# ubc-vision/RefTR

Hardware: AMD Instinct MI355X
Metric: images/sec training step, RefCOCO R50 640x640 bs=8/GPU (higher is better)
Workload: dtype bf16; 1 GPU; RefCOCO-shaped REC train step, ResNet-50 + BERT-base + VL transformer 6+6, 640x640, batch 8/GPU, L=40, aux loss, dropout on, clip 0.1, AdamW (configs[1]); global_batch=8, batch_per_gpu=8, image_size=640, parallelism=dp1, launch=hipgraph

## Files before the change

include/reftr_hip.h:

```cpp
#ifndef REFTR_HIP_H
#define REFTR_HIP_H
#include <stdint.h>

#ifdef __cplusplus
extern "C" {
#endif

typedef void* rt_stream_t;

enum { RT_OK = 0, RT_ERR_BADARG = -1, RT_ERR_UNSUPPORTED = -2, RT_ERR_COMM = -3 };
enum { RT_ACT_NONE = 0, RT_ACT_RELU = 1, RT_ACT_GELU = 2, RT_ACT_TANH = 3 };

int rt_abi_version(void);
int rt_device_arch(int dev, char* buf, int buflen);

typedef struct rt_conv_gemm_desc {
    const void*  src;
    const void*  wgt;
    void*        out_bf16;
    float*       out_f32;
    const float* bias;
    const float* res_f32;
    const void*  res_bf16;
    const void*  gate;
    const void*  preact;
    int32_t B, SH, SW, SC;
    int32_t DH, DW, N;
    int32_t KH, KW, stride, pad;
    int32_t transposed;
    int32_t act;
    float    gate_scale;
    float    drop_p;
    uint32_t drop_seed;
    int32_t  tile_hint;
    void*    out_preact;
    const void* dtanh;
    int32_t  res_first;
    const uint32_t* seed_dev;
    int32_t drop_shift;
    float* acc2_f32;
    int32_t dil;
} rt_conv_gemm_desc;
int rt_conv_gemm(const rt_conv_gemm_desc* d, rt_stream_t stream);
int rt_conv_gemm_grouped(const rt_conv_gemm_desc* descs, int n, rt_stream_t stream);

typedef struct rt_conv_wgrad_desc {
    const void*  dy;
    const void*  x;
    float*       dw;
    const float* scale;
    int32_t B, SH, SW, SC;
    int32_t DH, DW, N;
    int32_t KH, KW, stride, pad;
    int32_t msplit;
    float*  dbias;
    int32_t variant;
    float*  workspace;
    int64_t workspace_bytes;
    int32_t overwrite;
    int32_t dil;
    float*  sqacc;
    void*   g16;
} rt_conv_wgrad_desc;
int rt_conv_wgrad(const rt_conv_wgrad_desc* d, rt_stream_t stream);

typedef struct rt_small_wgrad_job {
    const void* dy; const void* x; float* dw; float* dbias;
    int32_t M, N, K, overwrite;
    float* sqacc;
    void*  g16;
} rt_small_wgrad_job;
int rt_small_wgrad_grouped(const rt_small_wgrad_job* jobs, int njobs, rt_stream_t stream);

int rt_conv_wgrad_grouped(const rt_conv_wgrad_desc* descs, int n, float* workspace, int64_t workspace_bytes, rt_stream_t stream);

int rt_gconv(const rt_conv_gemm_desc* d, int groups, rt_stream_t stream);
int rt_gconv_wgrad(const rt_conv_wgrad_desc* d, int groups, rt_stream_t stream);

typedef struct rt_layernorm_desc {
    const float* x;
    const float* gamma;
    const float* beta;
    float*       y_f32;
    void*        y_bf16;
    const float* pos;
    void*        ypos_bf16;
    float*       mean;
    float*       rstd;
    int32_t M, D;
    float   eps;
    int32_t act;
    float    drop_p;
    uint32_t drop_seed;
    int32_t grp_rows, grp_stride, grp_off;
    const uint32_t* seed_dev;
} rt_layernorm_desc;
int rt_layernorm_fwd(const rt_layernorm_desc* d, rt_stream_t stream);

typedef struct rt_layernorm_bwd_desc {
    const float* dy;
    const float* dy2;
    const float* x;
    const float* gamma;
    const float* beta;
    const float* mean;
    const float* rstd;
    float*       dx_f32;
    void*        dx_bf16;
    float*       dgamma;
    float*       dbeta;
    int32_t M, D;
    int32_t act;
    float    drop_p;  uint32_t drop_seed;
    float    drop2_p; uint32_t drop2_seed;
    int32_t grp_rows, grp_stride, grp_off;
    const uint32_t* seed_dev;
    float*   partials;
    int32_t* n_blocks_out;
} rt_layernorm_bwd_desc;
int rt_layernorm_bwd(const rt_layernorm_bwd_desc* d, rt_stream_t stream);

typedef struct rt_ln_pg_job {
    const float* partials; float* dgamma; float* dbeta;
    int32_t n_blocks, D;
} rt_ln_pg_job;
int rt_ln_param_grad_grouped(const rt_ln_pg_job* jobs, int n, rt_stream_t stream);

typedef struct rt_groupnorm_desc {
    const float* x;
    const float* gamma; const float* beta;
    float*       stats;
    float*       y_f32; void* y_bf16;
    const float* pos; void* ypos_bf16;
    int32_t B, HW, C, G;
    float   eps;
    int32_t out_rows_per_img, out_row_off;
    float*  partials;
    int32_t chunks;
} rt_groupnorm_desc;
int rt_groupnorm_fwd(const rt_groupnorm_desc* d, rt_stream_t stream);

typedef struct rt_groupnorm_bwd_desc {
    const float* dy; const float* dy2;
    const float* x; const float* gamma;
    const float* stats;
    float*       bstats;
    float*       dx_f32; void* dx_bf16;
    float*       dgamma; float* dbeta;
    int32_t B, HW, C, G;
    float   eps;
    int32_t out_rows_per_img, out_row_off;
} rt_groupnorm_bwd_desc;
int rt_groupnorm_bwd(const rt_groupnorm_bwd_desc* d, rt_stream_t stream);

typedef struct rt_gn_nhwc_desc {
    const float* x; const float* gamma; const float* beta;
    float* stats; void* y_bf16;
    int32_t B, HW, C, G, ldx, ldy, act;
    float eps;
    float* partials; int32_t partial_blocks;
} rt_gn_nhwc_desc;
int rt_gn_nhwc_fwd(const rt_gn_nhwc_desc* d, rt_stream_t stream);

typedef struct rt_gn_nhwc_bwd_desc {
    const float* dy; const float* x; const float* gamma; const float* beta;
    const float* stats; float* bstats;
    void* dx_bf16; float* dgamma; float* dbeta;
    int32_t B, HW, C, G, ldx, lddy, lddx, act;
    float eps;
} rt_gn_nhwc_bwd_desc;
int rt_gn_nhwc_bwd(const rt_gn_nhwc_bwd_desc* d, rt_stream_t stream);

typedef struct rt_upsample_add_desc {
    const float* fpn; const void* a_bf16; void* out_bf16;
    int32_t B, H, W, h, w, C, ldf, lda, ldo;
} rt_upsample_add_desc;
int rt_upsample_add(const rt_upsample_add_desc* d, rt_stream_t stream);

typedef struct rt_upsample_add_bwd_desc {
    const float* dy; float* da; void* dy_bf16;
    int32_t B, H, W, h, w, C, lddy, ldda, lddyb;
} rt_upsample_add_bwd_desc;
int rt_upsample_add_bwd(const rt_upsample_add_bwd_desc* d, rt_stream_t stream);

typedef struct rt_attn_map_desc {
    const float* q; const float* k; const uint8_t* mask;
    float* P; void* concat_bf16;
    int32_t B, HW, E, nh, ldk, k_rows_per_img, k_row_off, ld_concat, concat_col;
    float norm;
} rt_attn_map_desc;
int rt_attn_map_fwd(const rt_attn_map_desc* d, rt_stream_t stream);

typedef struct rt_attn_map_bwd_desc {
    const float* q; const float* k; const float* P; const float* dconcat;
    float* dq; float* dk;
    int32_t B, HW, E, nh, ldk, k_rows_per_img, k_row_off, ld_dconcat, concat_col;
    float norm;
} rt_attn_map_bwd_desc;
int rt_attn_map_bwd(const rt_attn_map_bwd_desc* d, rt_stream_t stream);

typedef struct rt_seg_concat_desc {
    const float* src; const float* mem; void* out_bf16;
    int32_t B, HW, E, nh, ldo, mem_rows_per_img, mem_row_off, src_rows_per_img, src_row_off;
} rt_seg_concat_desc;
int rt_seg_concat(const rt_seg_concat_desc* d, rt_stream_t stream);

typedef struct rt_mask_loss_desc {
    const float* pred; const uint8_t* target;
    float* sums; float* losses;
    float* dpred; const float* g_focal; const float* g_dice;
    int32_t B, h, w, Ht, Wt, ldp, lddp;
    float inv_norm;
    float* gbuf;
} rt_mask_loss_desc;
#define RT_MASK_LOSS_PARTIALS 1024
int rt_mask_loss(const rt_mask_loss_desc* d, rt_stream_t stream);

typedef struct rt_attn_desc {
    const void* q; const void* k; const void* v;
    void*  out;
    float* lse;
    const uint8_t* kpm;
    int32_t B, H, Sq, Sk, dh;
    int32_t ldq, ldk, ldv, ldo;
    float    scale;
    float    drop_p; uint32_t drop_seed;
    const uint32_t* seed_dev;
} rt_attn_desc;
int rt_attn_fwd(const rt_attn_desc* d, rt_stream_t stream);

typedef struct rt_attn_bwd_desc {
    const void* q; const void* k; const void* v; const void* out; const void* dout;
    const float* lse;
    float* delta;
    const uint8_t* kpm;
    void* dq; void* dk; void* dv;
    int32_t B, H, Sq, Sk, dh;
    int32_t ldq, ldk, ldv, ldo, lddq, lddk, lddv;
    float    scale;
    float    drop_p; uint32_t drop_seed;
    const uint32_t* seed_dev;
} rt_attn_bwd_desc;
int rt_attn_bwd(const rt_attn_bwd_desc* d, rt_stream_t stream);

int rt_img_pack(const float* img, void* out, int B, int H, int W, int Hp, int Wp, rt_stream_t stream);
int rt_stem_conv(const void* xp, const void* w, const float* bias, void* out,
                 int B, int Hp, int Wp, int Ho, int Wo, rt_stream_t stream);
int rt_maxpool3x3s2(const void* x, void* y, int B, int H, int W, int C, int Ho, int Wo, rt_stream_t stream);
int rt_stem_pool(const void* xp, const void* w, const float* bias, void* out,
                 int B, int Hp, int Wp, int Ho, int Wo, rt_stream_t stream);
int rt_weight_prep(const float* src, const float* scale, void* dst, void* dst_t, int N, int T, int C, rt_stream_t stream);

typedef struct rt_bottleneck_desc {
    const void*  x;
    const void*  w1;
    const void*  w2;
    const void*  w3;
    const void*  wd;
    const float* b1;
    const float* b2;
    const float* b3;
    const float* bd;
    void*        out;
    int32_t B, H, W, cin, planes;
    int32_t form;
} rt_bottleneck_desc;
int rt_bottleneck_fwd(const rt_bottleneck_desc* d, rt_stream_t stream);
int rt_weight_prep_batched(const int64_t* table, int njobs, int total_tiles, rt_stream_t stream);
int rt_stem_weight_prep(const float* src, const float* scale, void* dst, rt_stream_t stream);
int rt_bn_fold(const float* w, const float* b, const float* rm, const float* rv, float eps,
               float* scale, float* shift, int n, rt_stream_t stream);

typedef struct rt_mask_posenc_desc {
    const uint8_t* mask;
    uint8_t* kpm_out;
    float*   pos_out;
    const float* add_vec;
    int32_t B, H, W, h, w, C;
    int32_t kpm_stride, kpm_off;
    int32_t pos_rows_per_img, pos_row_off;
} rt_mask_posenc_desc;
int rt_mask_posenc(const rt_mask_posenc_desc* d, rt_stream_t stream);

int rt_colsum(const void* dy, int is_bf16, float* db, int M, int N, rt_stream_t stream);

typedef struct rt_rows_add_desc {
    const float* a_f32; const void* a_bf16; const float* b_f32;
    float* out_f32; void* out_bf16;
    int32_t rows, D;
    float   alpha;
    int32_t accumulate;
    int32_t a_grp_rows, a_grp_stride, a_grp_off;
    int32_t b_grp_rows, b_grp_stride, b_grp_off;
    int32_t o_grp_rows, o_grp_stride, o_grp_off;
} rt_rows_add_desc;
int rt_rows_add(const rt_rows_add_desc* d, rt_stream_t stream);

int rt_bert_embed_fwd(const int64_t* ids, const float* word, const float* pos, const float* type0,
                      float* out, int rows, int L, int D, const int32_t* pos_ids, rt_stream_t stream);
int rt_bert_embed_bwd(const int64_t* ids, const float* de, float* dword, float* dpos, float* dtype0,
                      int rows, int L, int D, const int32_t* pos_ids, rt_stream_t stream);
int rt_roberta_pos_ids(const int64_t* ids, int32_t* pos_ids, int B, int L, int pad_idx, rt_stream_t stream);
int rt_context_mask(const uint8_t* smask, const uint8_t* phrase_mask, const int64_t* pos_l, const int64_t* pos_r,
                    uint8_t* ctx, uint8_t* qmask, int B, int L, int P, int Lp, rt_stream_t stream);
int rt_qenc_attn_fwd(const float* k, const float* qs, const float* vs, const uint8_t* ctx, float* w, float* c,
                     int B, int P, int L, int E, rt_stream_t stream);
int rt_qenc_attn_bwd(const float* k, const float* qs, const float* vs, const float* w, const float* dc,
                     float* dk, float* dqs, float* dvs, int B, int P, int L, int E, rt_stream_t stream);

typedef struct rt_box_loss_desc {
    const float*   logits;
    const uint8_t* valid;
    const float*   targets;
    const int32_t* tgt_off;
    const float*   num_boxes;
    float* losses; float* total; float* dlogits;
    int32_t NL, B, P, K;
    float   w_bbox, w_giou;
    const float* weights;
} rt_box_loss_desc;
int rt_box_loss(const rt_box_loss_desc* d, rt_stream_t stream);

int rt_small_dgrad(const float* dy, const float* w, const void* gate, void* dx, int M, int N, int K, rt_stream_t stream);
int rt_pos_grad(const float* dpos, float* d_lang_pos, float* d_type, float* d_level, int B, int S, int L, int E,
                rt_stream_t stream);

int rt_sqnorm(const float* g, int64_t n, float* out, rt_stream_t stream);
int rt_sqnorm_bf16(const void* g16, int64_t n, float* out, rt_stream_t stream);

typedef struct rt_adamw_desc {
    float* p; const float* g; float* m; float* v;
    int64_t n;
    const float* gnorm_sq;
    float* gnorm_out;
    float grad_scale, max_norm, beta1, beta2, eps;
    int32_t step, n_ranges;
    int64_t range_begin[8], range_end[8];
    float   range_lr[8], range_wd[8];
    const int32_t* step_dev;
    const int32_t* active;
    const float*   lr_dev;
    int64_t span_begin, span_end;
    const void* g16;
} rt_adamw_desc;
int rt_adamw_flat(const rt_adamw_desc* d, rt_stream_t stream);
int rt_sgd_flat(const rt_adamw_desc* d, rt_stream_t stream);
enum { RT_ACCUM_FIRST = 0, RT_ACCUM_ADD = 1, RT_ACCUM_FINISH = 2 };
// ... 327 lines not shown
```

reftr_amd/csrc/rt_gemm.hip:

```cpp
#include "rt_gemm_dma.h"
#include <stdio.h>

namespace {

#ifdef RT_LAB
template <int BM, int BN, int MODE>
__global__ __launch_bounds__(256, 2) void conv_gemm_kernel(const bf16_t* __restrict__ src,
                                                        const bf16_t* __restrict__ wgt, const GemmArgs p) {
    typedef WaveTile<BM, BN, 2> WT;
    constexpr int TM = WT::TM, TN = WT::TN;
    constexpr int AJ = BN / 32, BJ = BM / 32;
    constexpr int A_BYTES = WT::A_BYTES, BUF_BYTES = WT::BUF_BYTES;
    extern __shared__ __attribute__((aligned(16))) unsigned char smem[];

    const int t = threadIdx.x;
    const int lane = t & 63, wave = t >> 6;
    const int wn = wave & 1, wm = wave >> 1;
    const WT wt{wn, wm, lane & 15, lane >> 4};

    const int n_tiles = (p.N + BN - 1) / BN;
    const int tile_n = blockIdx.x % n_tiles, tile_m = blockIdx.x / n_tiles;
    const int n0 = tile_n * BN, m0 = tile_m * BM;

    const int chunk = t & 7, srow = t >> 3;

    int a_off[AJ]; bool a_ok[AJ];
#pragma unroll
    for (int j = 0; j < AJ; ++j) {
        const int n = n0 + srow + 32 * j;
        a_ok[j] = n < p.N;
        a_off[j] = a_ok[j] ? n * p.K + chunk * 8 : 0;
    }
    int b_off[BJ], b_y[BJ], b_x[BJ]; bool b_ok[BJ];
#pragma unroll
    for (int j = 0; j < BJ; ++j) {
        const int m = m0 + srow + 32 * j;
        b_ok[j] = m < p.M;
        const int mm = b_ok[j] ? m : 0;
        if (MODE == 0) {
            b_off[j] = mm * p.SC + chunk * 8; b_y[j] = 0; b_x[j] = 0;
        } else {
            const int dx = mm % p.DW;
            const int tmp = mm / p.DW;
            const int dy = tmp % p.DH;
            const int b = tmp / p.DH;
            if (MODE == 1) { b_y[j] = dy * p.stride - p.pad; b_x[j] = dx * p.stride - p.pad; }
            else           { b_y[j] = dy + p.pad;            b_x[j] = dx + p.pad; }
            b_off[j] = b * p.SH * p.SW * p.SC + chunk * 8;
        }
    }

    f32x4 acc[TN][TM];
#pragma unroll
    for (int a = 0; a < TN; ++a)
#pragma unroll
        for (int b = 0; b < TM; ++b) acc[a][b] = f32x4{0.f, 0.f, 0.f, 0.f};

    const int nk = p.K >> 6;
    int lk = 0, c0 = 0, kw = 0, kh = 0;

    uint4 ra0[AJ], rb0[BJ], ra1[AJ], rb1[BJ];

    const __amdgpu_buffer_rsrc_t rs_w = __builtin_amdgcn_make_buffer_rsrc(const_cast<bf16_t*>(wgt), 0, p.wgt_bytes, 0x00020000);
    const __amdgpu_buffer_rsrc_t rs_x = __builtin_amdgcn_make_buffer_rsrc(const_cast<bf16_t*>(src), 0, p.src_bytes, 0x00020000);
    constexpr int OOB = 0x7fffffff;
    auto load_tiles = [&](uint4 (&ra)[AJ], uint4 (&rb)[BJ]) __attribute__((always_inline)) {
        const int k0b = lk << 7;
#pragma unroll
        for (int j = 0; j < AJ; ++j) {
            const auto v = __builtin_amdgcn_raw_buffer_load_b128(rs_w, a_ok[j] ? a_off[j] * 2 : OOB, k0b, 0);
            ra[j] = make_uint4(v[0], v[1], v[2], v[3]);
        }
#pragma unroll
        for (int j = 0; j < BJ; ++j) {
            if (MODE == 0) {
                const auto v = __builtin_amdgcn_raw_buffer_load_b128(rs_x, b_ok[j] ? b_off[j] * 2 : OOB, k0b, 0);
                rb[j] = make_uint4(v[0], v[1], v[2], v[3]);
            } else {
                bool ok = b_ok[j];
                int sy, sx;
                if (MODE == 1) { sy = b_y[j] + kh; sx = b_x[j] + kw; }
                else {
                    const int ny = b_y[j] - kh, nx = b_x[j] - kw;
                    const int msk = p.stride - 1;
                    ok = ok && ((ny | nx) >= 0) && (((ny | nx) & msk) == 0);
                    sy = ny >> p.sshift; sx = nx >> p.sshift;
                }
                ok = ok && (unsigned)sy < (unsigned)p.SH && (unsigned)sx < (unsigned)p.SW;
                const int off = (b_off[j] + (sy * p.SW + sx) * p.SC) * 2;
                const auto v = __builtin_amdgcn_raw_buffer_load_b128(rs_x, ok ? off : OOB, c0 * 2, 0);
                rb[j] = make_uint4(v[0], v[1], v[2], v[3]);
            }
        }
        if (lk + 1 < nk) {
            ++lk;
            if (MODE != 0) {
                c0 += 64;
                if (c0 >= p.SC) { c0 = 0; ++kw; if (kw >= p.KW) { kw = 0; ++kh; } }
            }
        }
    };
    auto store_tiles = [&](int buf, const uint4 (&ra)[AJ], const uint4 (&rb)[BJ]) __attribute__((always_inline)) {
        unsigned char* bA = smem + buf * BUF_BYTES;
        unsigned char* bB = bA + A_BYTES;
#pragma unroll
        for (int j = 0; j < AJ; ++j) {
            const int row = srow + 32 * j;
            *reinterpret_cast<uint4*>(bA + row * 128 + ((chunk ^ (row & 7)) << 4)) = ra[j];
        }
#pragma unroll
        for (int j = 0; j < BJ; ++j) {
            const int row = srow + 32 * j;
            *reinterpret_cast<uint4*>(bB + row * 128 + ((chunk ^ (row & 7)) << 4)) = rb[j];
        }
    };
    auto compute = [&](int buf) __attribute__((always_inline)) { wt.compute(smem + buf * BUF_BYTES, acc); };

    load_tiles(ra0, rb0);
    load_tiles(ra1, rb1);
    store_tiles(0, ra0, rb0);
    __syncthreads();
    for (int kt = 0; kt < nk; kt += 2) {
        load_tiles(ra0, rb0);
        compute(0);
        store_tiles(1, ra1, rb1);
        __syncthreads();
        if (kt + 1 >= nk) break;
        load_tiles(ra1, rb1);
        compute(1);
        store_tiles(0, ra0, rb0);
        __syncthreads();
    }

#pragma unroll
    for (int a = 0; a < TN; ++a) {
        const int n = n0 + wn * (BN / 2) + a * 16 + wt.lg * 4;
        if (n >= p.N) continue;
#pragma unroll
        for (int b = 0; b < TM; ++b) {
            const int m = m0 + wm * (BM / 2) + b * 16 + wt.li;
            if (m >= p.M) continue;
            epilogue<4>(p, m, n, acc[a][b]);
        }
    }
}

#endif

struct GemmGroup { GemmArgs j[12]; int first[13]; int n; };
struct GroupTile { static constexpr int BM = 64, BN = 64, NS = 2, MINB = 4; };
template <int BM, int BN, int NS, int MINB>
__global__ __launch_bounds__(256, MINB) void conv_gemm_dma_grouped_kernel(const GemmGroup g) {
    int lo = 0;
    for (int i = 1; i < g.n; ++i) if (g.first[i] <= (int)blockIdx.x) lo = i;
    lo = __builtin_amdgcn_readfirstlane(lo);
    const int lin = (int)blockIdx.x - g.first[lo];
    const int gx = g.first[lo + 1] - g.first[lo];
    gemm_dma_body<BM, BN, 0, NS>(g.j[lo].src, g.j[lo].wgt, g.j[lo], lin, 0, gx);
}

template <int CH>
__global__ __launch_bounds__(256) void skinny_gemm_kernel(const bf16_t* __restrict__ src, const bf16_t* __restrict__ wgt,
                                                          const GemmArgs p) {
    __shared__ f32x4 red[4][64];
    const int lane = threadIdx.x & 63, wave = threadIdx.x >> 6;
    const int li = lane & 15, lg = lane >> 4;
    const int n0 = blockIdx.x * 16;
    const int nrow = n0 + li;
    const int n = n0 + lg * 4;
    const bool out_ok = wave == 0 && n < p.N && li < p.M;
    EpiPre<4> pre;
    if (out_ok) pre = epi_prefetch<4>(p, (size_t)li * p.N + n, n);
    constexpr int OOB = 0x7fffffff;
    const __amdgpu_buffer_rsrc_t rs_w = __builtin_amdgcn_make_buffer_rsrc(const_cast<bf16_t*>(wgt), 0, p.wgt_bytes, 0x00020000);
    const __amdgpu_buffer_rsrc_t rs_x = __builtin_amdgcn_make_buffer_rsrc(const_cast<bf16_t*>(src), 0, p.src_bytes, 0x00020000);
    const int w_off = nrow < p.N ? (nrow * p.K + lg * 8) * 2 : OOB;
    const int x_off = li < p.M ? (li * p.K + lg * 8) * 2 : OOB;
    const int ksteps = p.K >> 5;
    const int per = (ksteps + 3) >> 2;
    const int k_begin = wave * per, k_end = min(k_begin + per, ksteps);
    f32x4 acc = {0.f, 0.f, 0.f, 0.f};
    typedef __attribute__((ext_vector_type(4))) unsigned u32x4;
    for (int ks = k_begin; ks < k_end; ks += CH) {
        u32x4 wv[CH], xv[CH];
#pragma unroll
        for (int j = 0; j < CH; ++j) {
            const bool in = ks + j < k_end;
            wv[j] = __builtin_amdgcn_raw_buffer_load_b128(rs_w, in ? w_off : OOB, (ks + j) << 6, 0);
            xv[j] = __builtin_amdgcn_raw_buffer_load_b128(rs_x, in ? x_off : OOB, (ks + j) << 6, 0);
        }
#pragma unroll
        for (int j = 0; j < CH; ++j)
            acc = __builtin_amdgcn_mfma_f32_16x16x32_bf16(*reinterpret_cast<bf16x8*>(&wv[j]), *reinterpret_cast<bf16x8*>(&xv[j]), acc, 0, 0, 0);
    }
    red[wave][lane] = acc;
    __syncthreads();
    if (wave != 0) return;
    acc = red[0][lane] + red[1][lane] + red[2][lane] + red[3][lane];
    if (out_ok) epilogue<4, true>(p, li, n, acc, &pre);
}

#ifdef RT_LAB
__global__ __launch_bounds__(256) void skinny_gemm_kernel_v1(const bf16_t* __restrict__ src, const bf16_t* __restrict__ wgt,
                                                             const GemmArgs p) {
    __shared__ f32x4 red[4][64];
    const int lane = threadIdx.x & 63, wave = threadIdx.x >> 6;
    const int li = lane & 15, lg = lane >> 4;
    const int n0 = blockIdx.x * 16;
    const int nrow = n0 + li;
    const bool n_ok = nrow < p.N, m_ok = li < p.M;
    const bf16_t* wp = wgt + (size_t)(n_ok ? nrow : 0) * p.K + lg * 8;
    const bf16_t* xp = src + (size_t)(m_ok ? li : 0) * p.K + lg * 8;
    const int ksteps = p.K >> 5;
    const int per = (ksteps + 3) >> 2;
    const int k_begin = wave * per, k_end = min(k_begin + per, ksteps);
    f32x4 acc = {0.f, 0.f, 0.f, 0.f};
    const uint4 z = make_uint4(0, 0, 0, 0);
#pragma unroll 4
    for (int ks = k_begin; ks < k_end; ++ks) {
        uint4 wv = *reinterpret_cast<const uint4*>(wp + ks * 32);
        uint4 xv = *reinterpret_cast<const uint4*>(xp + ks * 32);
        if (!n_ok) wv = z;
        if (!m_ok) xv = z;
        acc = __builtin_amdgcn_mfma_f32_16x16x32_bf16(*reinterpret_cast<bf16x8*>(&wv), *reinterpret_cast<bf16x8*>(&xv), acc, 0, 0, 0);
    }
    red[wave][lane] = acc;
    __syncthreads();
    if (wave != 0) return;
    acc = red[0][lane] + red[1][lane] + red[2][lane] + red[3][lane];
    const int n = n0 + lg * 4;
    if (n < p.N && li < p.M) epilogue<4>(p, li, n, acc);
}

template <int BM, int BN>
int launch_gemm(const GemmArgs& a, hipStream_t s) {
    const int mt = (a.M + BM - 1) / BM, nt = (a.N + BN - 1) / BN;
    const size_t smem = 2 * (size_t)(BM + BN) * 128;
    const dim3 grid((unsigned)(mt * nt)), block(256);
    if (gemm_dense(a))
        hipLaunchKernelGGL((conv_gemm_kernel<BM, BN, 0>), grid, block, smem, s, a.src, a.wgt, a);
    else if (!a.transposed)
        hipLaunchKernelGGL((conv_gemm_kernel<BM, BN, 1>), grid, block, smem, s, a.src, a.wgt, a);
    else
        hipLaunchKernelGGL((conv_gemm_kernel<BM, BN, 2>), grid, block, smem, s, a.src, a.wgt, a);
    RT_CHECK_LAUNCH();
    return RT_OK;
}

#endif

}

static int fill_gemm_args(const rt_conv_gemm_desc* d, GemmArgs& a) {
    if (!d || !d->src || !d->wgt || (!d->out_bf16 && !d->out_f32)) return RT_ERR_BADARG;
    if (d->SC <= 0 || (d->SC & 63) || (d->N & 3) || d->N <= 0) return RT_ERR_UNSUPPORTED;
    if (d->stride != 1 && d->stride != 2) return RT_ERR_UNSUPPORTED;
    if (d->KH <= 0 || d->KW <= 0 || d->B <= 0 || d->DH <= 0 || d->DW <= 0) return RT_ERR_BADARG;
    a.src = (const bf16_t*)d->src; a.wgt = (const bf16_t*)d->wgt;
    a.out_bf16 = (bf16_t*)d->out_bf16; a.out_f32 = d->out_f32; a.out_preact = (bf16_t*)d->out_preact;
    a.bias = d->bias; a.res_f32 = d->res_f32; a.res_bf16 = (const bf16_t*)d->res_bf16;
    a.gate = (const bf16_t*)d->gate; a.preact = (const bf16_t*)d->preact; a.dtanh = (const bf16_t*)d->dtanh;
    a.B = d->B; a.SH = d->SH; a.SW = d->SW; a.SC = d->SC; a.DH = d->DH; a.DW = d->DW; a.N = d->N;
    a.KH = d->KH; a.KW = d->KW; a.stride = d->stride; a.pad = d->pad; a.transposed = d->transposed;
    a.act = d->act; a.res_first = d->res_first; a.gate_scale = d->gate_scale; a.drop_p = d->drop_p; a.drop_seed = d->drop_seed; a.seed_dev = d->seed_dev;
    a.drop_shift = d->drop_shift;
    a.acc2_f32 = d->acc2_f32;
    a.dil = d->dil > 1 ? d->dil : 1;
    if (a.dil > 1 && d->stride != 1) return RT_ERR_UNSUPPORTED;
    if (a.drop_shift < 0 || a.drop_shift > 16) return RT_ERR_BADARG;
    const long long M = (long long)d->B * d->DH * d->DW;
    if (M > 0x7fffffffLL / 4) return RT_ERR_UNSUPPORTED;
    if ((long long)d->B * d->SH * d->SW * d->SC >= 0x3fffffffLL || (long long)d->N * d->KH * d->KW * d->SC >= 0x3fffffffLL) return RT_ERR_UNSUPPORTED;
    a.M = (int)M; a.K = d->KH * d->KW * d->SC; a.sshift = d->stride == 2 ? 1 : 0;
    static const int xcd_env = RT_TUNE("REFTR_XCD", 1);
    a.xcd = xcd_env;
    static const int early_env = RT_TUNE("REFTR_EARLY", 3);
    a.early = early_env & 1;
    static const int epi_env = RT_TUNE("REFTR_EPI", 3);
    a.epi_lds = epi_env & 1;
#ifdef RT_LAB
    static const int abl_env = RT_TUNE("REFTR_GEMM_ABL", 0);
    a.abl = abl_env;
#else
    a.abl = 0;
#endif
    static const int pre_env = RT_TUNE("REFTR_EPI_PREFETCH", 1);
    a.prefetch = pre_env;
    a.mfast = 0;
    a.src_bytes = (unsigned)((long long)d->B * d->SH * d->SW * d->SC * 2);
    a.wgt_bytes = (unsigned)((long long)d->N * d->KH * d->KW * d->SC * 2);
    return RT_OK;
}

static bool gemm_skinny(const GemmArgs& a) { return gemm_dense(a) && a.M <= 16; }
enum { GEMM_ROUTE_SKINNY = -1 };

static int gemm_route(const GemmArgs& a, int tile_hint) {
    if (tile_hint != 0) return tile_hint;
    if (gemm_skinny(a)) return GEMM_ROUTE_SKINNY;
    const bool dense = gemm_dense(a);
    int hint;
    const long long t128 = (long long)((a.M + 127) / 128) * ((a.N + 127) / 128);
    const long long t12864 = (long long)((a.M + 127) / 128) * ((a.N + 63) / 64);
    static const int smallt = RT_TUNE("REFTR_SMALLT", 1);
    static const int pipe = RT_TUNE("REFTR_PIPE", 3);
    const long long t64 = (long long)((a.M + 63) / 64) * ((a.N + 63) / 64);
    const long long t256 = (long long)((a.M + 255) / 256) * ((a.N + 127) / 128);
    static const int deep = RT_TUNE("REFTR_DEEP", 1);
    static const int k1024 = RT_TUNE("REFTR_K1024", 1);
    if (dense && smallt && a.M <= 1024 && t64 < 256 && (a.N & 7) == 0) hint = t64 <= 96 ? ((deep && a.K >= 512) ? 285 : 281) : 33;
    else if (a.K < 1024) hint = (a.N >= 128 && t128 >= 384 && t128 <= 512) ? 51 : 31;
    else if (dense && a.K >= 2048 && a.N >= 128 && t256 >= 512) hint = 262;
    else if (a.N > 64 && (t128 >= 384 || (a.K >= 2048 && t128 >= 192))) hint = (!dense && (pipe & 1) && a.K >= 2048 && t128 <= 256) ? 252 : 51;
    else if (k1024 && dense && a.N > 64 && a.K >= 1024 && t128 >= 192) hint = 51;
    else if (t12864 >= 256) hint = 21;
    else hint = (!dense && (pipe & 2)) ? 233 : 33;
#ifdef RT_LAB
    static const int pp = RT_TUNE("REFTR_PP", 0);
    if ((a.N & 7) == 0 && a.epi_lds && a.N >= 128) {
        if ((pp & 1) && hint == 252) hint = (pp & 4) ? 351 : 352;
        else if ((pp & 2) && dense && a.K >= 1024 && t128 >= 128 && t128 <= 256) hint = (pp & 4) ? 351 : 352;
    }
    static const int astat = RT_TUNE("REFTR_ASTAT", 0);
    if (astat && rt_gemm_astat_ok(a) && a.M >= 1024 && a.N >= 2 * a.K && a.N >= 256) hint = 501;
    {
        const char* ov = getenv("REFTR_HINT_OVERRIDE");
        while (ov && *ov) {
            int t_, kh_, s_, m_, k_, n_, h_, used = 0;
            if (sscanf(ov, "%d,%d,%d,%d,%d,%d=%d%n", &t_, &kh_, &s_, &m_, &k_, &n_, &h_, &used) == 7) {
                if (t_ == (a.transposed ? 1 : 0) && kh_ == a.KH && s_ == a.stride && m_ == a.M && k_ == a.K && n_ == a.N) { hint = h_; break; }
                ov += used;
            }
            while (*ov && *ov != ';') ++ov;
            if (*ov == ';') ++ov;
        }
    }
#endif
    return hint;
}

static int launch_skinny(const GemmArgs& a, hipStream_t s) {
    const dim3 grid((unsigned)((a.N + 15) / 16));
    const int per = ((a.K >> 5) + 3) >> 2;
#ifdef RT_LAB
    static const int skinny_v = RT_TUNE("REFTR_SKINNY_V", 2);
    if (skinny_v == 1) { hipLaunchKernelGGL(skinny_gemm_kernel_v1, grid, dim3(256), 0, s, a.src, a.wgt, a); RT_CHECK_LAUNCH(); return RT_OK; }
#endif
    if (per <= 2) hipLaunchKernelGGL(skinny_gemm_kernel<2>, grid, dim3(256), 0, s, a.src, a.wgt, a);
    else if (per <= 4) hipLaunchKernelGGL(skinny_gemm_kernel<4>, grid, dim3(256), 0, s, a.src, a.wgt, a);
    else hipLaunchKernelGGL(skinny_gemm_kernel<8>, grid, dim3(256), 0, s, a.src, a.wgt, a);
    RT_CHECK_LAUNCH();
    return RT_OK;
}

extern "C" int rt_conv_gemm(const rt_conv_gemm_desc* d, rt_stream_t stream) {
    GemmArgs a;
    const int frc = fill_gemm_args(d, a);
    if (frc != RT_OK) return frc;
    hipStream_t s = (hipStream_t)stream;
    const int hint = gemm_route(a, d->tile_hint);
    if (a.dil > 1 && hint >= 1 && hint <= 3) return RT_ERR_UNSUPPORTED;
    switch (hint) {
        case GEMM_ROUTE_SKINNY: return launch_skinny(a, s);
        case 21: return launch_gemm_dma<128, 64, 2, 2>(a, s);
        case 31: return launch_gemm_dma<GroupTile::BM, GroupTile::BN, GroupTile::NS, GroupTile::MINB>(a, s);
        case 33: return launch_gemm_dma<64, 64, 3, 3>(a, s);
        case 51: return launch_gemm_dma<128, 128, 2, 2, 8>(a, s);
        case 233: case 252: case 262: case 281: case 285: return rt_launch_gemm_pipe(a, hint, s);
#ifdef RT_LAB
        case 501: return rt_launch_gemm_astat(a, s);
        case 1: return launch_gemm<128, 128>(a, s);
        case 2: return launch_gemm<128, 64>(a, s);
        case 3: return launch_gemm<64, 64>(a, s);
        case 11: return launch_gemm_dma<128, 128, 2, 2>(a, s);
        case 12: return launch_gemm_dma<128, 128, 3, 2>(a, s);
        case 13: return launch_gemm_dma<128, 128, 4, 2>(a, s);
        case 22: return launch_gemm_dma<128, 64, 3, 2>(a, s);
        case 32: return launch_gemm_dma<64, 64, 4, 2>(a, s);
        case 52: return launch_gemm_dma<128, 128, 3, 1, 8>(a, s);
        case 53: return launch_gemm_dma<128, 64, 2, 2, 8>(a, s);
        case 54: return launch_gemm_dma<128, 64, 3, 2, 8>(a, s);
        case 61: return launch_gemm_dma<256, 128, 2, 1, 8>(a, s);
        case 62: return launch_gemm_dma<256, 128, 3, 1, 8>(a, s);
        case 63: return launch_gemm_dma<128, 256, 2, 1, 8>(a, s);
        case 211: case 221: case 231: case 251: case 261:
        case 81: case 282: case 283: case 284: case 286: case 287: case 288: case 234: case 236: return rt_launch_gemm_pipe(a, hint, s);
        case 351: case 321: case 323: case 331: case 352: case 322: case 332: return rt_launch_gemm_pp(a, hint, s);
#endif
        default: return RT_ERR_BADARG;
    }
}

extern "C" int rt_conv_gemm_grouped(const rt_conv_gemm_desc* descs, int n, rt_stream_t stream) {
    if (!descs || n <= 0) return RT_ERR_BADARG;
    hipStream_t s = (hipStream_t)stream;
    static const int grp_env = RT_TUNE("REFTR_GEMM_GROUP", 1);
    bool ok = grp_env && n >= 2 && n <= 12;
    GemmGroup g;
    int blocks = 0;
    for (int i = 0; i < n && ok; ++i) {
        const rt_conv_gemm_desc& d = descs[i];
        GemmArgs a;
        const int rc = fill_gemm_args(&d, a);
        if (rc != RT_OK) return rc;
        if (d.tile_hint != 0 || !gemm_dense(a) || gemm_skinny(a) || a.K >= 1024) { ok = false; break; }
        g.j[i] = a; g.first[i] = blocks;
        blocks += ((a.M + GroupTile::BM - 1) / GroupTile::BM) * ((a.N + GroupTile::BN - 1) / GroupTile::BN);
    }
    if (!ok) {
        for (int i = 0; i < n; ++i) { const int rc = rt_conv_gemm(descs + i, stream); if (rc != RT_OK) return rc; }
        return RT_OK;
    }
    g.first[n] = blocks; g.n = n;
    for (int i = n + 1; i < 13; ++i) g.first[i] = blocks;
    hipLaunchKernelGGL((conv_gemm_dma_grouped_kernel<GroupTile::BM, GroupTile::BN, GroupTile::NS, GroupTile::MINB>), dim3((unsigned)blocks), dim3(256),
                       gemm_dma_lds_bytes(GroupTile::BM, GroupTile::BN, GroupTile::NS), s, g);
    RT_CHECK_LAUNCH();
    return RT_OK;
}

extern "C" int rt_abi_version(void) { return 39; }

extern "C" int rt_device_arch(int dev, char* buf, int buflen) {
    hipDeviceProp_t prop;
    hipError_t e = hipGetDeviceProperties(&prop, dev);
    if (e != hipSuccess) return (int)e;
    if (!buf || buflen <= 0) return RT_ERR_BADARG;
    int i = 0;
    for (; i < buflen - 1 && prop.gcnArchName[i]; ++i) buf[i] = prop.gcnArchName[i];
    buf[i] = 0;
    return RT_OK;
}
```

reftr_amd/hip.py:

```python
import contextlib
import ctypes
import os
from ctypes import POINTER, Structure, c_char_p, c_float, c_int, c_int32, c_int64, c_uint32, c_void_p

import torch

_HERE = os.path.dirname(os.path.abspath(__file__))
LIB_PATH = os.path.join(_HERE, "libreftr_hip_lab.so" if os.environ.get("REFTR_LAB", "0") == "1" else "libreftr_hip.so")
ABI_VERSION = 39

CONSTANTS = {
    "RT_ACT_NONE": 0, "RT_ACT_RELU": 1, "RT_ACT_GELU": 2, "RT_ACT_TANH": 3,
    "RT_ACCUM_FIRST": 0, "RT_ACCUM_ADD": 1, "RT_ACCUM_FINISH": 2, "RT_GRAD_ACCUM_SLOTS": 2048,
    "RT_SQ_SLOTS": 256, "RT_SQ_STRIDE": 32,
    "RT_MASK_LOSS_PARTIALS": 1024, "RT_STATS_MAX": 40,
    "RT_BATCH_STAGE_MAX_B": 64,
    "RT_RAW_STAGE_MAX_SCALE": 4, "RT_RAW_STAGE_TILE_H": 32, "RT_RAW_STAGE_TILE_W": 64,
    "RT_EVAL_DET_N": 0, "RT_EVAL_DET_HIT": 1, "RT_EVAL_SEG_N": 6, "RT_EVAL_SEG_HIT": 7, "RT_EVAL_SEG_I": 12, "RT_EVAL_SEG_U": 13,
    "RT_EVAL_DET_SUM": 14, "RT_EVAL_SEG_SUM": 15, "RT_EVAL_SLOTS": 16, "RT_EVAL_CHUNK": 16384,
    "RT_EVAL_ORIG_N": 0, "RT_EVAL_ORIG_HIT": 1, "RT_EVAL_ORIG_I": 6, "RT_EVAL_ORIG_U": 7, "RT_EVAL_ORIG_SUM": 8, "RT_EVAL_ORIG_SLOTS": 9,
    "RT_PREDICT_FACTS_WORDS": 8,
    "RT_DEC_MAX_LAYERS": 8, "RT_DEC_HANDOFF_BYTES": 256 + 16 * 256 * 36 + 16 * 2048 * 4,
}
globals().update({name[3:]: value for name, value in CONSTANTS.items()})

STRUCTS = {}


class _Abi(Structure):

    def __init_subclass__(cls, c):
        cls.C_NAME = c
        STRUCTS[c] = cls


class ConvGemmDesc(_Abi, c="rt_conv_gemm_desc"):
    _fields_ = [("src", c_void_p), ("wgt", c_void_p), ("out_bf16", c_void_p), ("out_f32", c_void_p),
                ("bias", c_void_p), ("res_f32", c_void_p), ("res_bf16", c_void_p), ("gate", c_void_p),
                ("preact", c_void_p),
                ("B", c_int32), ("SH", c_int32), ("SW", c_int32), ("SC", c_int32),
                ("DH", c_int32), ("DW", c_int32), ("N", c_int32),
                ("KH", c_int32), ("KW", c_int32), ("stride", c_int32), ("pad", c_int32),
                ("transposed", c_int32), ("act", c_int32),
                ("gate_scale", c_float), ("drop_p", c_float), ("drop_seed", c_uint32), ("tile_hint", c_int32),
                ("out_preact", c_void_p), ("dtanh", c_void_p), ("res_first", c_int32), ("seed_dev", c_void_p),
                ("drop_shift", c_int32), ("acc2_f32", c_void_p), ("dil", c_int32)]


class ConvWgradDesc(_Abi, c="rt_conv_wgrad_desc"):
    _fields_ = [("dy", c_void_p), ("x", c_void_p), ("dw", c_void_p), ("scale", c_void_p),
                ("B", c_int32), ("SH", c_int32), ("SW", c_int32), ("SC", c_int32),
                ("DH", c_int32), ("DW", c_int32), ("N", c_int32),
                ("KH", c_int32), ("KW", c_int32), ("stride", c_int32), ("pad", c_int32),
                ("msplit", c_int32), ("dbias", c_void_p), ("variant", c_int32),
                ("workspace", c_void_p), ("workspace_bytes", c_int64), ("overwrite", c_int32), ("dil", c_int32),
                ("sqacc", c_void_p), ("g16", c_void_p)]


class LayerNormDesc(_Abi, c="rt_layernorm_desc"):
    _fields_ = [("x", c_void_p), ("gamma", c_void_p), ("beta", c_void_p), ("y_f32", c_void_p), ("y_bf16", c_void_p),
                ("pos", c_void_p), ("ypos_bf16", c_void_p), ("mean", c_void_p), ("rstd", c_void_p),
                ("M", c_int32), ("D", c_int32), ("eps", c_float), ("act", c_int32),
                ("drop_p", c_float), ("drop_seed", c_uint32),
                ("grp_rows", c_int32), ("grp_stride", c_int32), ("grp_off", c_int32), ("seed_dev", c_void_p)]


class LayerNormBwdDesc(_Abi, c="rt_layernorm_bwd_desc"):
    _fields_ = [("dy", c_void_p), ("dy2", c_void_p), ("x", c_void_p), ("gamma", c_void_p), ("beta", c_void_p),
                ("mean", c_void_p), ("rstd", c_void_p), ("dx_f32", c_void_p), ("dx_bf16", c_void_p),
                ("dgamma", c_void_p), ("dbeta", c_void_p),
                ("M", c_int32), ("D", c_int32), ("act", c_int32),
                ("drop_p", c_float), ("drop_seed", c_uint32), ("drop2_p", c_float), ("drop2_seed", c_uint32),
                ("grp_rows", c_int32), ("grp_stride", c_int32), ("grp_off", c_int32), ("seed_dev", c_void_p),
                ("partials", c_void_p), ("n_blocks_out", POINTER(c_int32))]


class LnPgJob(_Abi, c="rt_ln_pg_job"):
    _fields_ = [("partials", c_void_p), ("dgamma", c_void_p), ("dbeta", c_void_p), ("n_blocks", c_int32), ("D", c_int32)]


class GroupNormDesc(_Abi, c="rt_groupnorm_desc"):
    _fields_ = [("x", c_void_p), ("gamma", c_void_p), ("beta", c_void_p), ("stats", c_void_p),
                ("y_f32", c_void_p), ("y_bf16", c_void_p), ("pos", c_void_p), ("ypos_bf16", c_void_p),
                ("B", c_int32), ("HW", c_int32), ("C", c_int32), ("G", c_int32), ("eps", c_float),
                ("out_rows_per_img", c_int32), ("out_row_off", c_int32), ("partials", c_void_p), ("chunks", c_int32)]


class GroupNormBwdDesc(_Abi, c="rt_groupnorm_bwd_desc"):
    _fields_ = [("dy", c_void_p), ("dy2", c_void_p), ("x", c_void_p), ("gamma", c_void_p), ("stats", c_void_p),
                ("bstats", c_void_p), ("dx_f32", c_void_p), ("dx_bf16", c_void_p), ("dgamma", c_void_p), ("dbeta", c_void_p),
                ("B", c_int32), ("HW", c_int32), ("C", c_int32), ("G", c_int32), ("eps", c_float),
                ("out_rows_per_img", c_int32), ("out_row_off", c_int32)]


class AttnDesc(_Abi, c="rt_attn_desc"):
    _fields_ = [("q", c_void_p), ("k", c_void_p), ("v", c_void_p), ("out", c_void_p), ("lse", c_void_p), ("kpm", c_void_p),
                ("B", c_int32), ("H", c_int32), ("Sq", c_int32), ("Sk", c_int32), ("dh", c_int32),
                ("ldq", c_int32), ("ldk", c_int32), ("ldv", c_int32), ("ldo", c_int32),
                ("scale", c_float), ("drop_p", c_float), ("drop_seed", c_uint32), ("seed_dev", c_void_p)]


class AttnBwdDesc(_Abi, c="rt_attn_bwd_desc"):
    _fields_ = [("q", c_void_p), ("k", c_void_p), ("v", c_void_p), ("out", c_void_p), ("dout", c_void_p),
                ("lse", c_void_p), ("delta", c_void_p), ("kpm", c_void_p), ("dq", c_void_p), ("dk", c_void_p), ("dv", c_void_p),
                ("B", c_int32), ("H", c_int32), ("Sq", c_int32), ("Sk", c_int32), ("dh", c_int32),
                ("ldq", c_int32), ("ldk", c_int32), ("ldv", c_int32), ("ldo", c_int32),
                ("lddq", c_int32), ("lddk", c_int32), ("lddv", c_int32),
                ("scale", c_float), ("drop_p", c_float), ("drop_seed", c_uint32), ("seed_dev", c_void_p)]


class MaskPosencDesc(_Abi, c="rt_mask_posenc_desc"):
    _fields_ = [("mask", c_void_p), ("kpm_out", c_void_p), ("pos_out", c_void_p), ("add_vec", c_void_p),
                ("B", c_int32), ("H", c_int32), ("W", c_int32), ("h", c_int32), ("w", c_int32), ("C", c_int32),
                ("kpm_stride", c_int32), ("kpm_off", c_int32), ("pos_rows_per_img", c_int32), ("pos_row_off", c_int32)]


class BottleneckDesc(_Abi, c="rt_bottleneck_desc"):
    _fields_ = [("x", c_void_p), ("w1", c_void_p), ("w2", c_void_p), ("w3", c_void_p), ("wd", c_void_p),
                ("b1", c_void_p), ("b2", c_void_p), ("b3", c_void_p), ("bd", c_void_p), ("out", c_void_p),
                ("B", c_int32), ("H", c_int32), ("W", c_int32), ("cin", c_int32), ("planes", c_int32), ("form", c_int32)]


class RowsAddDesc(_Abi, c="rt_rows_add_desc"):
    _fields_ = [("a_f32", c_void_p), ("a_bf16", c_void_p), ("b_f32", c_void_p), ("out_f32", c_void_p), ("out_bf16", c_void_p),
                ("rows", c_int32), ("D", c_int32), ("alpha", c_float), ("accumulate", c_int32),
                ("a_grp_rows", c_int32), ("a_grp_stride", c_int32), ("a_grp_off", c_int32),
                ("b_grp_rows", c_int32), ("b_grp_stride", c_int32), ("b_grp_off", c_int32),
                ("o_grp_rows", c_int32), ("o_grp_stride", c_int32), ("o_grp_off", c_int32)]


class BoxLossDesc(_Abi, c="rt_box_loss_desc"):
    _fields_ = [("logits", c_void_p), ("valid", c_void_p), ("targets", c_void_p), ("tgt_off", c_void_p),
                ("num_boxes", c_void_p), ("losses", c_void_p), ("total", c_void_p), ("dlogits", c_void_p),
                ("NL", c_int32), ("B", c_int32), ("P", c_int32), ("K", c_int32), ("w_bbox", c_float), ("w_giou", c_float),
                ("weights", c_void_p)]


class MaskPostDesc(_Abi, c="rt_mask_post_desc"):
    _fields_ = [("pred", c_void_p), ("sizes", c_void_p), ("orig", c_void_p), ("origin_off", c_void_p),
                ("masks", c_void_p), ("masks_origin", c_void_p),
                ("B", c_int32), ("Q", c_int32), ("h", c_int32), ("w", c_int32), ("max_h", c_int32), ("max_w", c_int32),
                ("max_origin", c_int64), ("threshold", c_float)]


class BoxPostDesc(_Abi, c="rt_box_post_desc"):
    _fields_ = [("boxes", c_void_p), ("valid", c_void_p), ("sizes", c_void_p), ("out", c_void_p), ("counts", c_void_p),
                ("B", c_int32), ("P", c_int32), ("K", c_int32)]


class CemDesc(_Abi, c="rt_cem_desc"):
    _fields_ = [("hs", c_void_p), ("w3", c_void_p), ("b3", c_void_p), ("res", c_void_p), ("w2", c_void_p), ("b2", c_void_p),
                ("u", c_void_p), ("energy", c_void_p), ("stats", c_void_p), ("loss", c_void_p), ("g", c_void_p),
                ("dres", c_void_p), ("dhs", c_void_p), ("dw3", c_void_p), ("db3", c_void_p), ("dw2", c_void_p),
                ("B", c_int32), ("HW", c_int32), ("ld", c_int32), ("lddr", c_int32), ("E", c_int32), ("reserved", c_int32)]


class AdamWDesc(_Abi, c="rt_adamw_desc"):
    _fields_ = [("p", c_void_p), ("g", c_void_p), ("m", c_void_p), ("v", c_void_p), ("n", c_int64),
                ("gnorm_sq", c_void_p), ("gnorm_out", c_void_p),
                ("grad_scale", c_float), ("max_norm", c_float), ("beta1", c_float), ("beta2", c_float), ("eps", c_float),
                ("step", c_int32), ("n_ranges", c_int32),
                ("range_begin", c_int64 * 8), ("range_end", c_int64 * 8), ("range_lr", c_float * 8), ("range_wd", c_float * 8),
                ("step_dev", c_void_p), ("active", c_void_p), ("lr_dev", c_void_p), ("span_begin", c_int64), ("span_end", c_int64),
                ("g16", c_void_p)]


class FinishDesc(_Abi, c="rt_finish_desc"):
    _fields_ = [("step", c_void_p), ("active", c_void_p), ("cond", c_void_p), ("loss", c_void_p),
                ("sq", c_void_p), ("norm_scale", c_float), ("grad_norm", c_void_p),
                ("src", c_void_p * STATS_MAX), ("n_src", c_int), ("cond_in_stats", c_int), ("stats", c_void_p)]


class SmallWgradJob(_Abi, c="rt_small_wgrad_job"):
    _fields_ = [("dy", c_void_p), ("x", c_void_p), ("dw", c_void_p), ("dbias", c_void_p),
                ("M", c_int32), ("N", c_int32), ("K", c_int32), ("overwrite", c_int32), ("sqacc", c_void_p), ("g16", c_void_p)]


class GnNhwcDesc(_Abi, c="rt_gn_nhwc_desc"):
    _fields_ = [("x", c_void_p), ("gamma", c_void_p), ("beta", c_void_p), ("stats", c_void_p), ("y_bf16", c_void_p),
                ("B", c_int32), ("HW", c_int32), ("C", c_int32), ("G", c_int32), ("ldx", c_int32), ("ldy", c_int32),
                ("act", c_int32), ("eps", c_float), ("partials", c_void_p), ("partial_blocks", c_int32)]


class GnNhwcBwdDesc(_Abi, c="rt_gn_nhwc_bwd_desc"):
    _fields_ = [("dy", c_void_p), ("x", c_void_p), ("gamma", c_void_p), ("beta", c_void_p), ("stats", c_void_p),
                ("bstats", c_void_p), ("dx_bf16", c_void_p), ("dgamma", c_void_p), ("dbeta", c_void_p),
                ("B", c_int32), ("HW", c_int32), ("C", c_int32), ("G", c_int32), ("ldx", c_int32), ("lddy", c_int32),
                ("lddx", c_int32), ("act", c_int32), ("eps", c_float)]


class UpsampleAddDesc(_Abi, c="rt_upsample_add_desc"):
    _fields_ = [("fpn", c_void_p), ("a_bf16", c_void_p), ("out_bf16", c_void_p),
                ("B", c_int32), ("H", c_int32), ("W", c_int32), ("h", c_int32), ("w", c_int32), ("C", c_int32),
                ("ldf", c_int32), ("lda", c_int32), ("ldo", c_int32)]


class UpsampleAddBwdDesc(_Abi, c="rt_upsample_add_bwd_desc"):
    _fields_ = [("dy", c_void_p), ("da", c_void_p), ("dy_bf16", c_void_p),
                ("B", c_int32), ("H", c_int32), ("W", c_int32), ("h", c_int32), ("w", c_int32), ("C", c_int32),
                ("lddy", c_int32), ("ldda", c_int32), ("lddyb", c_int32)]


class AttnMapDesc(_Abi, c="rt_attn_map_desc"):
    _fields_ = [("q", c_void_p), ("k", c_void_p), ("mask", c_void_p), ("P", c_void_p), ("concat_bf16", c_void_p),
                ("B", c_int32), ("HW", c_int32), ("E", c_int32), ("nh", c_int32), ("ldk", c_int32),
                ("k_rows_per_img", c_int32), ("k_row_off", c_int32), ("ld_concat", c_int32), ("concat_col", c_int32),
                ("norm", c_float)]


class AttnMapBwdDesc(_Abi, c="rt_attn_map_bwd_desc"):
    _fields_ = [("q", c_void_p), ("k", c_void_p), ("P", c_void_p), ("dconcat", c_void_p), ("dq", c_void_p), ("dk", c_void_p),
                ("B", c_int32), ("HW", c_int32), ("E", c_int32), ("nh", c_int32), ("ldk", c_int32),
                ("k_rows_per_img", c_int32), ("k_row_off", c_int32), ("ld_dconcat", c_int32), ("concat_col", c_int32),
                ("norm", c_float)]


class SegConcatDesc(_Abi, c="rt_seg_concat_desc"):
    _fields_ = [("src", c_void_p), ("mem", c_void_p), ("out_bf16", c_void_p),
                ("B", c_int32), ("HW", c_int32), ("E", c_int32), ("nh", c_int32), ("ldo", c_int32),
                ("mem_rows_per_img", c_int32), ("mem_row_off", c_int32), ("src_rows_per_img", c_int32), ("src_row_off", c_int32)]


class MaskLossDesc(_Abi, c="rt_mask_loss_desc"):
    _fields_ = [("pred", c_void_p), ("target", c_void_p), ("sums", c_void_p), ("losses", c_void_p),
                ("dpred", c_void_p), ("g_focal", c_void_p), ("g_dice", c_void_p),
                ("B", c_int32), ("h", c_int32), ("w", c_int32), ("Ht", c_int32), ("Wt", c_int32), ("ldp", c_int32),
                ("lddp", c_int32), ("inv_norm", c_float), ("gbuf", c_void_p)]


class EvalMetricsArgs(_Abi, c="rt_eval_metrics_args"):
    _fields_ = [("pred_boxes", c_void_p), ("valid", c_void_p), ("table", c_void_p), ("masks", c_void_p), ("sizes", c_void_p),
                ("partials", c_void_p), ("iou_det", c_void_p), ("iou_seg", c_void_p), ("iu", c_void_p), ("acc", c_void_p),
                ("B", c_int32), ("P", c_int32), ("K", c_int32), ("Q", c_int32), ("max_h", c_int32), ("max_w", c_int32),
                ("reset", c_int32)]


class EvalCanvasArgs(_Abi, c="rt_eval_canvas_args"):
    _fields_ = [("pred_boxes", c_void_p), ("valid", c_void_p), ("tgt_boxes", c_void_p), ("tgt_off", c_void_p), ("facts", c_void_p),
                ("image_ids", c_void_p), ("pred_masks", c_void_p), ("tgt_masks", c_void_p), ("partials", c_void_p),
                ("iou_det", c_void_p), ("iou_seg", c_void_p), ("iu", c_void_p), ("acc", c_void_p), ("ring_boxes", c_void_p),
                ("ring_counts", c_void_p), ("ring_ids", c_void_p), ("cursor", c_void_p), ("veto", c_void_p),
                ("B", c_int32), ("P", c_int32), ("K", c_int32), ("Q", c_int32), ("h", c_int32), ("w", c_int32), ("Hc", c_int32),
                ("Wc", c_int32), ("tgt_rows", c_int32), ("slots", c_int32), ("threshold", c_float)]


class EvalRawFactsArgs(_Abi, c="rt_eval_raw_facts_args"):
    _N = CONSTANTS["RT_BATCH_STAGE_MAX_B"]
    _fields_ = [("facts", c_void_p), ("image_ids", c_void_p), ("mask_table", c_void_p), ("max_pixels", c_int64),
                ("B", c_int32), ("Hc", c_int32), ("Wc", c_int32), ("has_ids", c_int32),
                ("img_h", c_int32 * _N), ("img_w", c_int32 * _N), ("orig_h", c_int32 * _N), ("orig_w", c_int32 * _N),
                ("image_id", c_int64 * _N), ("tm_ptr", c_void_p * _N)]


class EvalOrigArgs(_Abi, c="rt_eval_orig_args"):
    _fields_ = [("pred_masks", c_void_p), ("facts", c_void_p), ("mask_table", c_void_p), ("partials", c_void_p), ("iou_seg", c_void_p),
                ("iu", c_void_p), ("acc", c_void_p), ("veto", c_void_p), ("max_pixels", c_int64),
                ("B", c_int32), ("Q", c_int32), ("h", c_int32), ("w", c_int32), ("Hc", c_int32), ("Wc", c_int32), ("threshold", c_float)]


class PredictFactsArgs(_Abi, c="rt_predict_facts_args"):
    _N = CONSTANTS["RT_BATCH_STAGE_MAX_B"]
    _fields_ = [("facts", c_void_p), ("capacity", c_int64), ("B", c_int32), ("Q", c_int32), ("Hc", c_int32), ("Wc", c_int32),
                ("img_h", c_int32 * _N), ("img_w", c_int32 * _N), ("orig_h", c_int32 * _N), ("orig_w", c_int32 * _N)]


class PredictCanvasArgs(_Abi, c="rt_predict_canvas_args"):
    _fields_ = [("pred_boxes", c_void_p), ("valid", c_void_p), ("facts", c_void_p), ("pred_masks", c_void_p), ("out_boxes", c_void_p),
                ("out_counts", c_void_p), ("out_masks", c_void_p), ("capacity", c_int64),
                ("B", c_int32), ("P", c_int32), ("K", c_int32), ("Q", c_int32), ("h", c_int32), ("w", c_int32), ("Hc", c_int32),
                ("Wc", c_int32), ("threshold", c_float)]


class RawStageArgs(_Abi, c="rt_raw_stage_args"):
    _N = CONSTANTS["RT_BATCH_STAGE_MAX_B"]
    _fields_ = [("img", c_void_p), ("mask", c_void_p), ("tgt_masks", c_void_p), ("boxes", c_void_p), ("tgt_off", c_void_p),
                ("num_boxes", c_void_p), ("B", c_int32), ("Hc", c_int32), ("Wc", c_int32), ("boxes_per_image", c_int32),
                ("mean", c_float * 3), ("std", c_float * 3),
                ("src", c_void_p * _N), ("box_ptr", c_void_p * _N), ("tm_ptr", c_void_p * _N),
                ("h", c_int32 * _N), ("w", c_int32 * _N), ("oh", c_int32 * _N), ("ow", c_int32 * _N), ("box_n", c_int32 * _N),
                ("rw", c_float * _N), ("rh", c_float * _N)]


class HsvJitterArgs(_Abi, c="rt_hsv_jitter_args"):
    _N = CONSTANTS["RT_BATCH_STAGE_MAX_B"]
    _fields_ = [("B", c_int32), ("src", c_void_p * _N), ("dst", c_void_p * _N), ("h", c_int32 * _N), ("w", c_int32 * _N),
                ("s_gain", c_float * _N), ("v_gain", c_float * _N)]


class DecoderLayerFwd(_Abi, c="rt_decoder_layer_fwd"):
    _PTRS = ("Wv", "Wo", "Wq", "Wo2", "W1", "W2", "bv", "bo", "bq", "bo2", "b1", "b2", "g1", "be1", "g2", "be2", "g3", "be3",
             "k2", "v2", "o", "t1q16", "q2", "o2", "t2_16", "hdn", "t3_16", "u", "u2", "u3",
             "mean1", "rstd1", "mean2", "rstd2", "mean3", "rstd3", "lse2", "t3_f32")
    _SEEDS = ("seed_ad", "seed_d1", "seed_ad2", "seed_d2", "seed_dh", "seed_d3")
    _fields_ = [(n, c_void_p) for n in _PTRS] + [(n, c_uint32) for n in _SEEDS]


class DecoderLayerBwd(_Abi, c="rt_decoder_layer_bwd"):
    _PTRS = ("WT2", "WT1", "WTo2", "WTq", "WTo", "WTv", "g1", "g2", "g3", "u", "u2", "u3",
             "mean1", "rstd1", "mean2", "rstd2", "mean3", "rstd3", "hdn", "q2", "k2", "v2", "o2", "lse2", "dnorm",
             "du3b", "dhdn", "du2b", "dq2", "dub", "dv", "dk2", "dv2", "dk2p", "dv2p", "part1", "part2", "part3")
    _SEEDS = ("seed_ad", "seed_d1", "seed_ad2", "seed_d2", "seed_d3", "reserved")
    _fields_ = [(n, c_void_p) for n in _PTRS] + [(n, c_uint32) for n in _SEEDS]


class DecoderBwdDesc(_Abi, c="rt_decoder_bwd_desc"):
    _fields_ = [("layer", DecoderLayerBwd * DEC_MAX_LAYERS),
                ("dta", c_void_p), ("dqpos", c_void_p), ("kpm", c_void_p), ("handoff", c_void_p), ("seed_dev", c_void_p),
                ("n_layers", c_int32), ("M", c_int32), ("H", c_int32), ("S", c_int32), ("F", c_int32), ("ldkv", c_int32),
                ("drop_p", c_float), ("scale", c_float), ("gate_scale", c_float), ("ldkvp", c_int32)]


class DecoderFwdDesc(_Abi, c="rt_decoder_fwd_desc"):
    _fields_ = [("layer", DecoderLayerFwd * DEC_MAX_LAYERS),
                ("t32", c_void_p), ("t16", c_void_p), ("qpos", c_void_p), ("kpm", c_void_p), ("handoff", c_void_p),
                ("seed_dev", c_void_p),
                ("n_layers", c_int32), ("M", c_int32), ("H", c_int32), ("S", c_int32), ("F", c_int32), ("ldkv", c_int32),
                ("drop_p", c_float), ("eps", c_float), ("scale", c_float)]


class QencFwdDesc(_Abi, c="rt_qenc_fwd_desc"):
    _PTRS = ("mem16", "mem32", "ctx", "W1", "W2", "W3", "Wc", "Wf0", "Wf4", "b1", "b2", "b3", "bc", "bf0", "bf4",
             "gc", "betc", "g1", "bet1", "g5", "bet5", "qembed", "seed_dev",
             "cls16", "lang16", "kq", "qs", "vs", "qw", "c16", "co", "cmean", "crstd", "cat16",
             "t1", "m1", "r1", "a16", "t2", "m2", "r2", "tgt32", "tgt16", "qpos", "tgtq16")
    _fields_ = [(n, c_void_p) for n in _PTRS] + [("B", c_int32), ("S", c_int32), ("L", c_int32), ("P", c_int32), ("nq", c_int32),
                                                 ("E", c_int32), ("eps", c_float), ("drop_p", c_float), ("drop_seed", c_uint32),
                                                 ("reserved", c_int32)]


class HeadLossDesc(_Abi, c="rt_head_loss_desc"):
    _PTRS = ("t3", "gn", "betn", "W0", "W1", "W2", "W0T", "W1T", "b0", "b1", "b2", "w2_f32",
             "valid", "targets", "tgt_off", "num_boxes", "weights",
             "hs16", "y1", "y2", "hmean", "hrstd", "logits", "losses", "dlogits", "dl16", "dy2", "dy1", "dhs", "dnorm", "db2_part", "part_n", "total", "ticket")
    _fields_ = [(n, c_void_p) for n in _PTRS] + [("NL", c_int32), ("B", c_int32), ("P", c_int32), ("K", c_int32), ("E", c_int32),
                                                 ("eps", c_float), ("invert_valid", c_int32), ("reserved", c_int32)]


class QencBwdDesc(_Abi, c="rt_qenc_bwd_desc"):
    _PTRS = ("ga", "gb", "dqpos", "t2", "m2", "r2", "g5", "bet5", "t1", "m1", "r1", "g1", "bet1", "co", "cmean", "crstd", "gc", "betc",
             "kq", "qs", "vs", "qw", "Wf4T", "Wf0T", "WcT", "W1T", "W2T", "W3T", "seed_dev",
             "dt2b", "dt1b", "dcob", "dk16", "dqs16", "dvs16", "da", "dcat", "dc", "dmem", "dqembed", "part5", "part1", "partc")
    _fields_ = [(n, c_void_p) for n in _PTRS] + [("B", c_int32), ("S", c_int32), ("L", c_int32), ("P", c_int32), ("E", c_int32),
                                                 ("drop_p", c_float), ("drop_seed", c_uint32), ("reserved", c_int32)]


_SIGNATURES = {
    "rt_abi_version": (c_int, []),
    "rt_device_arch": (c_int, [c_int, c_char_p, c_int]),
    "rt_conv_gemm": (c_int, [POINTER(ConvGemmDesc), c_void_p]),
    "rt_conv_gemm_grouped": (c_int, [c_void_p, c_int, c_void_p]),
    "rt_conv_wgrad": (c_int, [POINTER(ConvWgradDesc), c_void_p]),
    "rt_gconv": (c_int, [POINTER(ConvGemmDesc), c_int, c_void_p]),
    "rt_gconv_wgrad": (c_int, [POINTER(ConvWgradDesc), c_int, c_void_p]),
    "rt_layernorm_fwd": (c_int, [POINTER(LayerNormDesc), c_void_p]),
    "rt_layernorm_bwd": (c_int, [POINTER(LayerNormBwdDesc), c_void_p]),
    "rt_groupnorm_fwd": (c_int, [POINTER(GroupNormDesc), c_void_p]),
    "rt_groupnorm_bwd": (c_int, [POINTER(GroupNormBwdDesc), c_void_p]),
    "rt_attn_fwd": (c_int, [POINTER(AttnDesc), c_void_p]),
    "rt_attn_bwd": (c_int, [POINTER(AttnBwdDesc), c_void_p]),
    "rt_img_pack": (c_int, [c_void_p, c_void_p, c_int, c_int, c_int, c_int, c_int, c_void_p]),
    "rt_stem_conv": (c_int, [c_void_p, c_void_p, c_void_p, c_void_p, c_int, c_int, c_int, c_int, c_int, c_void_p]),
    "rt_maxpool3x3s2": (c_int, [c_void_p, c_void_p, c_int, c_int, c_int, c_int, c_int, c_int, c_void_p]),
    "rt_stem_pool": (c_int, [c_void_p, c_void_p, c_void_p, c_void_p, c_int, c_int, c_int, c_int, c_int, c_void_p]),
    "rt_bottleneck_fwd": (c_int, [POINTER(BottleneckDesc), c_void_p]),
    "rt_weight_prep": (c_int, [c_void_p, c_void_p, c_void_p, c_void_p, c_int, c_int, c_int, c_void_p]),
    "rt_weight_prep_batched": (c_int, [c_void_p, c_int, c_int, c_void_p]),
    "rt_stem_weight_prep": (c_int, [c_void_p, c_void_p, c_void_p, c_void_p]),
    "rt_bn_fold": (c_int, [c_void_p, c_void_p, c_void_p, c_void_p, c_float, c_void_p, c_void_p, c_int, c_void_p]),
    "rt_mask_posenc": (c_int, [POINTER(MaskPosencDesc), c_void_p]),
    "rt_colsum": (c_int, [c_void_p, c_int, c_void_p, c_int, c_int, c_void_p]),
    "rt_rows_add": (c_int, [POINTER(RowsAddDesc), c_void_p]),
    "rt_bert_embed_fwd": (c_int, [c_void_p, c_void_p, c_void_p, c_void_p, c_void_p, c_int, c_int, c_int, c_void_p, c_void_p]),
    "rt_bert_embed_bwd": (c_int, [c_void_p, c_void_p, c_void_p, c_void_p, c_void_p, c_int, c_int, c_int, c_void_p, c_void_p]),
    "rt_roberta_pos_ids": (c_int, [c_void_p, c_void_p, c_int, c_int, c_int, c_void_p]),
    "rt_context_mask": (c_int, [c_void_p, c_void_p, c_void_p, c_void_p, c_void_p, c_void_p, c_int, c_int, c_int, c_int, c_void_p]),
    "rt_qenc_attn_fwd": (c_int, [c_void_p, c_void_p, c_void_p, c_void_p, c_void_p, c_void_p, c_int, c_int, c_int, c_int, c_void_p]),
    "rt_qenc_attn_bwd": (c_int, [c_void_p, c_void_p, c_void_p, c_void_p, c_void_p, c_void_p, c_void_p, c_void_p, c_int, c_int, c_int, c_int, c_void_p]),
    "rt_box_loss": (c_int, [POINTER(BoxLossDesc), c_void_p]),
    "rt_cem_fwd": (c_int, [POINTER(CemDesc), c_void_p]),
    "rt_cem_bwd": (c_int, [POINTER(CemDesc), c_void_p]),
    "rt_mask_postprocess": (c_int, [POINTER(MaskPostDesc), c_void_p]),
    "rt_box_postprocess": (c_int, [POINTER(BoxPostDesc), c_void_p]),
    "rt_eval_metrics": (c_int, [POINTER(EvalMetricsArgs), c_void_p]),
    "rt_eval_facts": (c_int, [POINTER(c_void_p), POINTER(c_void_p), POINTER(c_void_p), POINTER(c_int32), c_int, c_void_p,
                              c_void_p, c_void_p]),
    "rt_eval_canvas": (c_int, [POINTER(EvalCanvasArgs), c_void_p]),
    "rt_eval_raw_facts": (c_int, [POINTER(EvalRawFactsArgs), c_void_p]),
    "rt_eval_orig": (c_int, [POINTER(EvalOrigArgs), c_void_p]),
    "rt_predict_facts": (c_int, [POINTER(PredictFactsArgs), c_void_p]),
    "rt_predict_canvas": (c_int, [POINTER(PredictCanvasArgs), c_void_p]),
    "rt_small_dgrad": (c_int, [c_void_p, c_void_p, c_void_p, c_void_p, c_int, c_int, c_int, c_void_p]),
    "rt_pos_grad": (c_int, [c_void_p, c_void_p, c_void_p, c_void_p, c_int, c_int, c_int, c_int, c_void_p]),
    "rt_sqnorm": (c_int, [c_void_p, c_int64, c_void_p, c_void_p]),
    "rt_sqnorm_bf16": (c_int, [c_void_p, c_int64, c_void_p, c_void_p]),
    "rt_sqnorm_finish": (c_int, [c_void_p, c_void_p, c_int, c_void_p, c_void_p, c_void_p, c_void_p]),
    "rt_round_chunks": (c_int, [c_void_p, c_void_p, c_void_p, c_int, c_void_p]),
    "rt_adamw_flat": (c_int, [POINTER(AdamWDesc), c_void_p]),
    "rt_sgd_flat": (c_int, [POINTER(AdamWDesc), c_void_p]),
    "rt_grad_accum": (c_int, [c_int, c_void_p, c_void_p, c_int64, c_float, c_void_p, c_void_p, c_void_p, c_void_p]),
    "rt_zero_chunks": (c_int, [c_void_p, c_void_p, c_int, c_void_p]),
    "rt_counter_add": (c_int, [c_void_p, c_int32, c_void_p]),
    "rt_ln_param_grad_grouped": (c_int, [POINTER(LnPgJob), c_int, c_void_p]),
    "rt_conv_wgrad_grouped": (c_int, [POINTER(ConvWgradDesc), c_int, c_void_p, c_int64, c_void_p]),
    "rt_small_wgrad_grouped": (c_int, [POINTER(SmallWgradJob), c_int, c_void_p]),
    "rt_resample_u8": (c_int, [c_void_p, c_void_p, c_void_p, c_void_p, c_int, c_int, c_int, c_int, c_int, c_int, c_void_p]),
    "rt_img_collate_norm": (c_int, [c_void_p, c_void_p, c_void_p, c_int, c_int, c_int, POINTER(c_float), POINTER(c_float), c_void_p]),
    "rt_batch_stage": (c_int, [c_void_p, c_void_p, c_int, c_int, c_int, c_void_p, c_void_p, c_int, c_int, POINTER(c_void_p),
                               POINTER(c_int32), c_int, c_void_p, c_void_p, c_void_p, POINTER(c_void_p), POINTER(c_int32),
                               c_void_p, c_void_p]),
    "rt_raw_stage": (c_int, [POINTER(RawStageArgs), c_void_p]),
    "rt_resample_taps": (c_int, [c_int, c_int, c_void_p, c_void_p, c_int, c_void_p]),
    "rt_hsv_jitter": (c_int, [POINTER(HsvJitterArgs), c_void_p]),
    "rt_gn_nhwc_fwd": (c_int, [POINTER(GnNhwcDesc), c_void_p]),
    "rt_gn_nhwc_bwd": (c_int, [POINTER(GnNhwcBwdDesc), c_void_p]),
    "rt_upsample_add": (c_int, [POINTER(UpsampleAddDesc), c_void_p]),
    "rt_upsample_add_bwd": (c_int, [POINTER(UpsampleAddBwdDesc), c_void_p]),
    "rt_attn_map_fwd": (c_int, [POINTER(AttnMapDesc), c_void_p]),
    "rt_attn_map_bwd": (c_int, [POINTER(AttnMapBwdDesc), c_void_p]),
    "rt_seg_concat": (c_int, [POINTER(SegConcatDesc), c_void_p]),
    "rt_mask_loss": (c_int, [POINTER(MaskLossDesc), c_void_p]),
    "rt_comm_unique_id": (c_int, [c_void_p]),
    "rt_comm_init": (c_int, [c_void_p, c_int, c_int, POINTER(c_void_p)]),
    "rt_comm_allreduce": (c_int, [c_void_p, POINTER(c_void_p), POINTER(c_int64), c_int, c_int, c_void_p]),
    "rt_comm_destroy": (c_int, [c_void_p]),
    "rt_decoder_fwd": (c_int, [POINTER(DecoderFwdDesc), c_void_p]),
    "rt_decoder_bwd": (c_int, [POINTER(DecoderBwdDesc), c_void_p]),
    "rt_decoder_trace": (c_int, [c_void_p]),
    "rt_decoder_supported": (c_int, [c_int]),
    "rt_decoder_set_spin": (c_int, [c_int]),
    "rt_counter_add_if_zero": (c_int, [c_void_p, c_int32, c_void_p, c_int, c_void_p]),
    "rt_stamp": (c_int, [c_void_p, c_int, c_void_p]),
    "rt_finish_step": (c_int, [c_void_p, c_void_p, c_void_p, c_void_p, c_void_p]),
    "rt_finish_stats": (c_int, [c_void_p, c_void_p]),
    "rt_adamw_mat": (c_int, [POINTER(AdamWDesc), c_void_p, c_int, c_int, c_void_p]),
    "rt_adamw_chunks": (c_int, [POINTER(AdamWDesc), c_void_p, c_int, c_void_p]),
    "rt_qenc_fwd": (c_int, [POINTER(QencFwdDesc), c_void_p]),
    "rt_head_loss": (c_int, [POINTER(HeadLossDesc), c_void_p]),
    "rt_qenc_bwd": (c_int, [POINTER(QencBwdDesc), c_void_p]),
    "rt_qregion_trace": (c_int, [c_void_p]),
}

_lib = None
LAB_LIB_PATH = os.path.join(_HERE, "libreftr_hip_lab.so")
PRODUCT_TILE_HINTS = frozenset({0, 21, 31, 33, 51, 233, 252, 262, 281, 285})


def _load(path):
    if not os.path.exists(path):
        raise RuntimeError(
            f"{path} not found: the HIP kernel library is not built. Run "
            "`python -c 'import __graft_entry__ as g; g.build()'` (needs hipcc; no CPU fallback exists).")
    L = ctypes.CDLL(path)
    for name, (res, args) in _SIGNATURES.items():
        fn = getattr(L, name)
        fn.restype = res
        fn.argtypes = args
    v = L.rt_abi_version()
    if v != ABI_VERSION:
        raise RuntimeError(f"{os.path.basename(path)} ABI {v} != binding ABI {ABI_VERSION}; rebuild")
    return L


def lib():
    global _lib
    if _lib is None:
        _lib = _load(LIB_PATH)
    return _lib


_lab_lib = None


@contextlib.contextmanager
def lab_library():
    global _lib, _lab_lib
    if _lab_lib is None:
        _lab_lib = _load(LAB_LIB_PATH)
    prev = lib()
    _lib = _lab_lib
    try:
        yield
    finally:
        _lib = prev


def exported_symbols():
    return sorted(_SIGNATURES)


def _p(t):
    return None if t is None else t.data_ptr()


def _stream():
    return torch.cuda.current_stream().cuda_stream


_PLAIN = frozenset({int, float, bool, type(None), POINTER(c_int32)})


def _val(v):
    if isinstance(v, torch.Tensor):
        return v.data_ptr()
    return tuple(_val(e) for e in v) if isinstance(v, (list, tuple)) else v


def _fill(d, fields, Tensor=torch.Tensor, plain=_PLAIN):
    for k, v in fields.items():
        if v.__class__ is Tensor:
            fields[k] = v.data_ptr()
        elif v.__class__ not in plain:
            fields[k] = _val(v)
    d.__init__(**fields)
    if d.__dict__:
        raise TypeError(f"{type(d).__name__} ({d.C_NAME}): no field {sorted(d.__dict__)}")
    return d


def _set(d, **fields):
    return _fill(d, fields)


def _desc(cls, **fields):
    return _fill(cls(), fields)


def _call(name, *args, stream=True, Tensor=torch.Tensor, plain=_PLAIN, byref=ctypes.byref):
    args = [a if a.__class__ in plain else a.data_ptr() if a.__class__ is Tensor
            else byref(a) if isinstance(a, Structure) else _val(a) for a in args]
    if stream:
        args.append(_stream())
    rc = getattr(lib(), name)(*args)
    if rc != 0:
        raise RuntimeError(f"{name} failed with code {rc} ({'RT_ERR' if rc < 0 else 'hipError'})")


_TIMER = None
_SEED_DEV = None


def set_seed_dev(t):
    global _SEED_DEV
    _SEED_DEV = t


def _seedp(drop_p):
    return _p(_SEED_DEV) if (drop_p > 0 and _SEED_DEV is not None) else None


def set_launch_timer(records):
    global _TIMER
    _TIMER = records


def _algo_bytes(tag):
    kind, B, SH, SW, SC, DH, DW, N, KH, KW = tag[:10]
    M = B * DH * DW
    if kind == "W":
        return 2.0 * (M * N + B * SH * SW * SC) + 4.0 * N * KH * KW * SC
    return 2.0 * (B * SH * SW * SC + N * KH * KW * SC + M * N)


def _timed(kind, flops, fn, tag=None, nbytes=None, epi_bytes=0.0):
    if _TIMER is None:
        return fn()
    e0 = torch.cuda.Event(enable_timing=True); e1 = torch.cuda.Event(enable_timing=True)
    e0.record()
    r = fn()
    e1.record()
    _TIMER.append({"kind": kind, "flops": float(flops), "start": e0, "end": e1, "tag": tag,
                   "bytes": nbytes if nbytes is not None else (_algo_bytes(tag) if tag is not None else 0.0),
                   "epi_bytes": float(epi_bytes)})
    return r


def as_u8(t):
    t = t.contiguous()
    if t.dtype == torch.bool:
        return t.view(torch.uint8)
    return t if t.dtype == torch.uint8 else t.to(torch.uint8)


def _req(t, dtype, name):
    if t is None:
        return
    if not t.is_cuda:
        raise RuntimeError(f"{name}: HIP kernels need a device tensor (got {t.device}); no CPU path exists")
    if t.dtype != dtype:
        raise RuntimeError(f"{name}: expected {dtype}, got {t.dtype}")
    if not t.is_contiguous():
        raise RuntimeError(f"{name}: tensor must be contiguous")


_GEOM = ("B", "SH", "SW", "SC", "DH", "DW", "N", "KH", "KW", "stride", "pad")


def _gemm_desc(src, wgt, geom, **fields):
    fields.update(src=src, wgt=wgt)
    return _fill(ConvGemmDesc(**dict(zip(_GEOM, geom, strict=True))), fields)


def _wgrad_desc(dy, x, dw, geom, **fields):
    fields.update(dy=dy, x=x, dw=dw, sqacc=_sqacc(dw), g16=_g16(dw))
    return _fill(ConvWgradDesc(**dict(zip(_GEOM, geom, strict=True))), fields)


def _out_buffer(o, dtype, name, M, N, dev):
    o = o if torch.is_tensor(o) else (torch.empty((M, N), dtype=dtype, device=dev) if o else None)
    _req(o, dtype, name)
    assert o is None or o.numel() == M * N
    return o


def conv_gemm(src, wgt, *, geom, bias=None, res_f32=None, res_bf16=None, gate=None, gate_scale=1.0,
              preact=None, dtanh=None, res_first=False, act=ACT_NONE, drop_p=0.0, drop_seed=0, transposed=False,
              out_bf16=True, out_f32=False, out_preact=False, tile_hint=0, group=None, drop_shift=0, acc2_f32=None, dil=1):
    B, SH, SW, SC, DH, DW, N, KH, KW, stride, pad = geom
    _req(src, torch.bfloat16, "src"); _req(wgt, torch.bfloat16, "wgt")
    _req(bias, torch.float32, "bias"); _req(res_f32, torch.float32, "res_f32")
    _req(res_bf16, torch.bfloat16, "res_bf16"); _req(gate, torch.bfloat16, "gate")
    _req(preact, torch.bfloat16, "preact")
    assert src.numel() == B * SH * SW * SC, (src.shape, geom)
    assert wgt.numel() == N * KH * KW * SC, (wgt.shape, geom)
    M = B * DH * DW
    _req(dtanh, torch.bfloat16, "dtanh")
    ob = _out_buffer(out_bf16, torch.bfloat16, "out_bf16", M, N, src.device)
    of = _out_buffer(out_f32, torch.float32, "out_f32", M, N, src.device)
    _req(acc2_f32, torch.float32, "acc2_f32")
    assert acc2_f32 is None or acc2_f32.numel() == M * N
    d = _gemm_desc(src, wgt, geom, out_bf16=ob, out_f32=of, bias=bias, res_f32=res_f32, res_bf16=res_bf16, gate=gate, preact=preact,
                   transposed=int(bool(transposed)), act=act, gate_scale=gate_scale, drop_p=drop_p, drop_seed=drop_seed & 0xFFFFFFFF,
                   tile_hint=tile_hint, dtanh=dtanh, res_first=int(bool(res_first)), seed_dev=_seedp(drop_p), drop_shift=drop_shift,
                   acc2_f32=acc2_f32, dil=int(dil))
    op = _out_buffer(out_preact, torch.bfloat16, "out_preact", M, N, src.device)
    if op is not None:
        _set(d, out_preact=op)
    if transposed:
        flops = 2.0 * B * SH * SW * SC * N * KH * KW
    else:
        flops = 2.0 * M * N * KH * KW * SC
    epi = M * N * (2.0 * sum(t is not None for t in (res_bf16, gate, preact, dtanh)) + 4.0 * (res_f32 is not None)
                   + 8.0 * (acc2_f32 is not None) + (4.0 if of is not None else 0.0) + (2.0 if ob is not None else 0.0) - 2.0
                   + (2.0 if op is not None else 0.0))
    if group is not None:
        group.add(d, flops, ("T" if transposed else "F",) + tuple(geom), (src, wgt, ob, of, op, bias, res_f32, res_bf16, gate, preact, dtanh), epi)
    else:
        _timed("conv_gemm", flops, lambda: _call("rt_conv_gemm", d), tag=("T" if transposed else "F",) + tuple(geom), epi_bytes=epi)
    if op is not None:
        return ob, of, op
    return ob, of


class GemmGroup:

    def __init__(self):
        self.descs, self.keep, self.flops, self.nbytes, self.epi = [], [], 0.0, 0.0, 0.0

    def add(self, d, flops, tag, keep, epi=0.0):
        self.descs.append(d); self.keep.append(keep); self.flops += flops; self.nbytes += _algo_bytes(tag); self.epi += epi

    def run(self):
        if not self.descs:
            return
        n = len(self.descs)
        for i in range(0, n, 12):
            chunk = self.descs[i:i + 12]
            arr = (ConvGemmDesc * len(chunk))(*chunk)
            share = len(chunk) / n
            _timed("conv_gemm", self.flops * share, lambda arr=arr, m=len(chunk): _call("rt_conv_gemm_grouped", arr, m),
                   nbytes=self.nbytes * share, epi_bytes=self.epi * share)
        self.descs, self.keep, self.flops, self.nbytes, self.epi = [], [], 0.0, 0.0, 0.0


def linear(x, w, bias=None, **kw):
    M, K = x.shape
    N = w.shape[0]
    return conv_gemm(x, w, geom=(M, 1, 1, K, 1, 1, N, 1, 1, 1, 0), bias=bias, **kw)


_WGRAD_WS = {}
WGRAD_WS_BYTES = 64 << 20


def _wgrad_workspace(dev):
    key = (dev.index, torch.cuda.current_stream().cuda_stream)
    ws = _WGRAD_WS.get(key)
    if ws is None:
        ws = _WGRAD_WS[key] = torch.empty(WGRAD_WS_BYTES // 4, dtype=torch.float32, device=dev)
    return ws


_SQACC_MAP = {}


def _owned(table, dw):
    ent = table.get(dw.data_ptr())
    if ent is None:
        return None
    if ent[0]() is None:
        del table[dw.data_ptr()]
        return None
    return ent[1]


def _sqacc(dw):
    t = _owned(_SQACC_MAP, dw)
    return t.data_ptr() if t is not None else None


_G16_MAP = {}


def _g16(dw):
    return _owned(_G16_MAP, dw)


def round_chunks(base, twin, table, n):
    _req(base, torch.float32, "base"); _req(twin, torch.bfloat16, "twin"); _req(table, torch.int64, "table")
    if n > 0:
        _call("rt_round_chunks", base, twin, table, int(n))


def sqnorm_finish(flat_g, table, nchunks, slots, out, extra=None):
    _req(flat_g, torch.float32, "flat_g"); _req(slots, torch.float32, "slots"); _req(out, torch.float32, "out")
    assert slots.numel() == SQ_SLOTS * SQ_STRIDE
    _call("rt_sqnorm_finish", flat_g, table, int(nchunks), slots, extra, out)


def conv_wgrad(dy, x, dw, *, geom, scale=None, msplit=0, dbias=None, variant=0, workspace=True, overwrite=False, dil=1):
    B, SH, SW, SC, DH, DW, N, KH, KW, stride, pad = geom
    _req(dy, torch.bfloat16, "dy"); _req(x, torch.bfloat16, "x"); _req(dw, torch.float32, "dw")
    _req(scale, torch.float32, "scale")
    assert dy.numel() == B * DH * DW * N and x.numel() == B * SH * SW * SC and dw.numel() == N * KH * KW * SC
    _req(dbias, torch.float32, "dbias")
    ws = _wgrad_workspace(dy.device) if workspace else None
    d = _wgrad_desc(dy, x, dw, geom, scale=scale, msplit=msplit, dbias=dbias, variant=variant, workspace=ws,
                    workspace_bytes=WGRAD_WS_BYTES if ws is not None else 0, overwrite=int(bool(overwrite)), dil=int(dil))
    _timed("conv_wgrad", 2.0 * B * DH * DW * N * KH * KW * SC, lambda: _call("rt_conv_wgrad", d), tag=("W",) + tuple(geom))
    return dw


def gconv(src, wgt, *, geom, groups, bias=None, gate=None, gate_scale=1.0, act=ACT_NONE, transposed=False,
          out_bf16=True, out_f32=False, dil=1, **unsupported):
    B, SH, SW, SC, DH, DW, N, KH, KW, stride, pad = geom
    _req(src, torch.bfloat16, "src"); _req(wgt, torch.bfloat16, "wgt"); _req(bias, torch.float32, "bias"); _req(gate, torch.bfloat16, "gate")
    assert src.numel() == B * SH * SW * SC, (src.shape, geom)
    cg = SC // groups if groups > 0 else 0
    assert wgt.numel() == SC * KH * KW * cg, (wgt.shape, geom, groups)
    M = B * DH * DW
    ob = _out_buffer(out_bf16, torch.bfloat16, "out_bf16", M, N, src.device)
    of = _out_buffer(out_f32, torch.float32, "out_f32", M, N, src.device)
    d = _gemm_desc(src, wgt, geom, out_bf16=ob, out_f32=of, bias=bias, gate=gate, transposed=int(bool(transposed)), act=act,
                   gate_scale=gate_scale, dil=int(dil), **unsupported)
    spatial = B * (SH * SW if transposed else DH * DW)
    flops = 2.0 * spatial * SC * KH * KW * cg
    _timed("gconv", flops, lambda: _call("rt_gconv", d, int(groups)), nbytes=2.0 * (B * SH * SW * SC + M * N) + 2.0 * wgt.numel())
    return ob, of


def gconv_wgrad(dy, x, dw, *, geom, groups, scale=None, msplit=0, overwrite=False, dil=1, dbias=None, variant=0):
    B, SH, SW, SC, DH, DW, N, KH, KW, stride, pad = geom
    _req(dy, torch.bfloat16, "dy"); _req(x, torch.bfloat16, "x"); _req(dw, torch.float32, "dw"); _req(scale, torch.float32, "scale")
    _req(dbias, torch.float32, "dbias")
    cg = SC // groups if groups > 0 else 0
    assert dy.numel() == B * DH * DW * N and x.numel() == B * SH * SW * SC and dw.numel() == N * KH * KW * cg
    ws = _wgrad_workspace(dy.device)
    d = _wgrad_desc(dy, x, dw, geom, scale=scale, msplit=msplit, dbias=dbias, variant=variant, workspace=ws,
                    workspace_bytes=WGRAD_WS_BYTES, overwrite=int(bool(overwrite)), dil=int(dil))
    _timed("gconv_wgrad", 2.0 * B * DH * DW * N * KH * KW * cg, lambda: _call("rt_gconv_wgrad", d, int(groups)),
           nbytes=2.0 * (B * DH * DW * N + B * SH * SW * SC) + 4.0 * dw.numel())
    return dw


def linear_wgrad(dy, x, dw, **kw):
    M, N = dy.shape
    K = x.shape[1]
    return conv_wgrad(dy, x, dw, geom=(M, 1, 1, K, 1, 1, N, 1, 1, 1, 0), **kw)


def _new(shape, dtype, like):
    return torch.empty(shape, dtype=dtype, device=like.device)


def layernorm_fwd(x, gamma, beta, eps=1e-5, *, act=ACT_NONE, drop_p=0.0, drop_seed=0, pos=None,
                  y_f32=None, y_bf16=None, ypos_bf16=None, want_f32=True, want_bf16=True,
                  rowmap=(0, 0, 0), save_stats=True):
    M, D = x.shape
    _req(x, torch.float32, "x"); _req(gamma, torch.float32, "gamma"); _req(beta, torch.float32, "beta")
    _req(pos, torch.float32, "pos")
    if y_f32 is None and want_f32:
        y_f32 = _new((M, D), torch.float32, x)
    if y_bf16 is None and want_bf16:
        y_bf16 = _new((M, D), torch.bfloat16, x)
    if pos is not None and ypos_bf16 is None:
        ypos_bf16 = _new((M, D), torch.bfloat16, x)
    mean = _new((M,), torch.float32, x) if save_stats else None
    rstd = _new((M,), torch.float32, x) if save_stats else None
    grp_rows, grp_stride, grp_off = rowmap
    _call("rt_layernorm_fwd", _desc(
        LayerNormDesc, x=x, gamma=gamma, beta=beta, y_f32=y_f32, y_bf16=y_bf16, pos=pos, ypos_bf16=ypos_bf16, mean=mean, rstd=rstd,
        M=M, D=D, eps=eps, act=act, drop_p=drop_p, drop_seed=drop_seed & 0xFFFFFFFF, grp_rows=grp_rows, grp_stride=grp_stride,
        grp_off=grp_off, seed_dev=_seedp(drop_p)))
    return y_f32, y_bf16, ypos_bf16, mean, rstd


class LnGradBatch:

    def __init__(self):
        self.jobs, self.keep = [], []

    def run(self):
        if not self.jobs:
            return
        arr = (LnPgJob * len(self.jobs))(*self.jobs)
        _call("rt_ln_param_grad_grouped", arr, len(self.jobs))
        self.jobs, self.keep = [], []


def layernorm_bwd(dy, x, gamma, beta, mean, rstd, dgamma, dbeta, *, dy2=None, act=ACT_NONE, drop_p=0.0,
                  drop_seed=0, drop2_p=0.0, drop2_seed=0, rowmap=(0, 0, 0), want_f32=True, want_bf16=True, pg_batch=None):
    M, D = x.shape
    _req(dy, torch.float32, "dy"); _req(dy2, torch.float32, "dy2"); _req(x, torch.float32, "x")
    dx_f32 = _new((M, D), torch.float32, x) if want_f32 else None
    dx_bf16 = _new((M, D), torch.bfloat16, x) if want_bf16 else None
    part, nb = None, c_int32(0)
    if pg_batch is not None and (dgamma is not None or dbeta is not None):
        part = _new((min((M + 3) // 4, 1024), 2, D), torch.float32, x)
    grp_rows, grp_stride, grp_off = rowmap
    _call("rt_layernorm_bwd", _desc(
        LayerNormBwdDesc, dy=dy, dy2=dy2, x=x, gamma=gamma, beta=beta, mean=mean, rstd=rstd, dx_f32=dx_f32, dx_bf16=dx_bf16,
        dgamma=dgamma, dbeta=dbeta, M=M, D=D, act=act, drop_p=drop_p, drop_seed=drop_seed & 0xFFFFFFFF, drop2_p=drop2_p,
        drop2_seed=drop2_seed & 0xFFFFFFFF, grp_rows=grp_rows, grp_stride=grp_stride, grp_off=grp_off,
        seed_dev=_seedp(max(drop_p, drop2_p)), partials=part, n_blocks_out=ctypes.pointer(nb)))
    if part is not None:
        pg_batch.jobs.append(_desc(LnPgJob, partials=part, dgamma=dgamma, dbeta=dbeta, n_blocks=nb.value, D=D))
        pg_batch.keep.append(part)
    return dx_f32, dx_bf16


def groupnorm_fwd(x, gamma, beta, G, eps, *, y_f32=None, y_bf16=None, pos=None, ypos_bf16=None,
                  rows_per_img=None, row_off=0):
    B, HW, C = x.shape
    _req(x, torch.float32, "x")
    rows_per_img = HW if rows_per_img is None else rows_per_img
    stats = _new((B, G, 2), torch.float32, x)
    chunks = min(64, (HW + 7) // 8)
    partials = _new((B, chunks, G, 2), torch.float32, x)
    _call("rt_groupnorm_fwd", _desc(
        GroupNormDesc, x=x, gamma=gamma, beta=beta, stats=stats, y_f32=y_f32, y_bf16=y_bf16, pos=pos, ypos_bf16=ypos_bf16,
        B=B, HW=HW, C=C, G=G, eps=eps, out_rows_per_img=rows_per_img, out_row_off=row_off, partials=partials, chunks=chunks))
    return stats


def groupnorm_bwd(dy, x, gamma, stats, dgamma, dbeta, G, eps, *, dy2=None, rows_per_img=None, row_off=0,
                  want_f32=False, want_bf16=True):
    B, HW, C = x.shape
    rows_per_img = HW if rows_per_img is None else rows_per_img
    bstats = _new((B, G, 2), torch.float32, x)
    dx_f32 = _new((B, HW, C), torch.float32, x) if want_f32 else None
    dx_bf16 = _new((B, HW, C), torch.bfloat16, x) if want_bf16 else None
    _call("rt_groupnorm_bwd", _desc(
        GroupNormBwdDesc, dy=dy, dy2=dy2, x=x, gamma=gamma, stats=stats, bstats=bstats, dx_f32=dx_f32, dx_bf16=dx_bf16,
        dgamma=dgamma, dbeta=dbeta, B=B, HW=HW, C=C, G=G, eps=eps, out_rows_per_img=rows_per_img, out_row_off=row_off))
    return dx_f32, dx_bf16


def _ld(t):
    assert t.dim() == 2 and t.stride(1) == 1, "attention operands are 2-D row views with unit inner stride"
    return t.stride(0)


def attn_fwd(q, k, v, kpm, *, B, H, Sq, Sk, dh, scale, drop_p=0.0, drop_seed=0, out=None):
    if out is None:
        out = _new((B * Sq, H * dh), torch.bfloat16, q)
    lse = _new((B, H, Sq), torch.float32, q)
    _call("rt_attn_fwd", _desc(
        AttnDesc, q=q, k=k, v=v, out=out, lse=lse, kpm=kpm, B=B, H=H, Sq=Sq, Sk=Sk, dh=dh, ldq=_ld(q), ldk=_ld(k), ldv=_ld(v),
        ldo=_ld(out), scale=scale, drop_p=drop_p, drop_seed=drop_seed & 0xFFFFFFFF, seed_dev=_seedp(drop_p)))
    return out, lse


def attn_bwd(q, k, v, out, dout, lse, kpm, *, B, H, Sq, Sk, dh, scale, drop_p=0.0, drop_seed=0,
             dq=None, dk=None, dv=None):
    if dq is None:
        dq = _new((B * Sq, H * dh), torch.bfloat16, q)
    if dk is None:
        dk = _new((B * Sk, H * dh), torch.bfloat16, q)
    if dv is None:
        dv = _new((B * Sk, H * dh), torch.bfloat16, q)
    delta = _new((B, H, Sq), torch.float32, q)
    d = _desc(AttnBwdDesc, q=q, k=k, v=v, out=out, dout=dout, lse=lse, delta=delta, kpm=kpm, dq=dq, dk=dk, dv=dv,
              B=B, H=H, Sq=Sq, Sk=Sk, dh=dh, ldq=_ld(q), ldk=_ld(k), ldv=_ld(v), ldo=_ld(out), lddq=_ld(dq), lddk=_ld(dk), lddv=_ld(dv),
              scale=scale, drop_p=drop_p, drop_seed=drop_seed & 0xFFFFFFFF, seed_dev=_seedp(drop_p))
    assert _ld(dout) == _ld(out)
    _call("rt_attn_bwd", d)
    return dq, dk, dv


def decoder_handoff(dev):
    return torch.zeros(DEC_HANDOFF_BYTES // 4, dtype=torch.int32, device=dev)


def decoder_fwd(layers, t32, t16, qpos, kpm, *, H, S, F, drop_p, scale, handoff, eps=1e-5):
    M = t32.shape[0]
    assert 1 <= len(layers) <= DEC_MAX_LAYERS
    d = _desc(DecoderFwdDesc, t32=t32, t16=t16, qpos=qpos, kpm=kpm, handoff=handoff, seed_dev=_seedp(drop_p), n_layers=len(layers),
              M=M, H=H, S=S, F=F, ldkv=_ld(layers[0]["k2"]), drop_p=drop_p, eps=eps, scale=scale)
    for i, lay in enumerate(layers):
        _set(d.layer[i], **{n: lay[n] for n in DecoderLayerFwd._PTRS}, **{n: lay[n] & 0xFFFFFFFF for n in DecoderLayerFwd._SEEDS})
    _call("rt_decoder_fwd", d)
    return handoff[:2]


def decoder_bwd(layers, dta, dqpos, kpm, *, H, S, F, drop_p, scale, gate_scale, handoff, ldkvp=0):
    M = dta.shape[0]
    assert 1 <= len(layers) <= DEC_MAX_LAYERS
    d = _desc(DecoderBwdDesc, dta=dta, dqpos=dqpos, kpm=kpm, handoff=handoff, seed_dev=_seedp(drop_p), n_layers=len(layers),
              M=M, H=H, S=S, F=F, ldkv=_ld(layers[0]["k2"]), drop_p=drop_p, scale=scale, gate_scale=gate_scale, ldkvp=ldkvp)
    for i, lay in enumerate(layers):
        _set(d.layer[i], **{n: lay.get(n) for n in DecoderLayerBwd._PTRS},
             **{n: lay[n] & 0xFFFFFFFF for n in DecoderLayerBwd._SEEDS[:-1]})
    _call("rt_decoder_bwd", d)
    return handoff[:2]


def decoder_trace(readback=True):
    buf = (c_uint32 * 1024)()
    _call("rt_decoder_trace", ctypes.cast(buf, c_void_p) if readback else None, stream=False)
    if not readback:
        return None
    a = list(buf)
    return a[:512], a[512:]


def stem_geometry(H, W):
    Ho, Wo = (H - 1) // 2 + 1, (W - 1) // 2 + 1
    Hp = max(H + 6, 2 * Ho + 5)
    Wp = max(W + 6, 32 * ((Wo + 15) // 16) + 6)
    return Ho, Wo, Hp, Wp


def img_pack(img):
    B, C, H, W = img.shape
    assert C == 3
    _req(img, torch.float32, "img")
    _, _, Hp, Wp = stem_geometry(H, W)
    out = _new((B, Hp, Wp, 4), torch.bfloat16, img)
    _call("rt_img_pack", img, out, B, H, W, Hp, Wp)
    return out


def stem_conv(xp, w, bias, Ho, Wo):
    B, Hp, Wp, _ = xp.shape
    out = _new((B, Ho, Wo, 64), torch.bfloat16, xp)
    _call("rt_stem_conv", xp, w, bias, out, B, Hp, Wp, Ho, Wo)
    return out


def maxpool3x3s2(x):
    B, H, W, C = x.shape
    Ho, Wo = (H - 1) // 2 + 1, (W - 1) // 2 + 1
    y = _new((B, Ho, Wo, C), torch.bfloat16, x)
    _call("rt_maxpool3x3s2", x, y, B, H, W, C, Ho, Wo)
    return y


def stem_pool(xp, w, bias, Ho, Wo):
    B, Hp, Wp, _ = xp.shape
    out = _new((B, (Ho - 1) // 2 + 1, (Wo - 1) // 2 + 1, 64), torch.bfloat16, xp)
    _call("rt_stem_pool", xp, w, bias, out, B, Hp, Wp, Ho, Wo)
    return out


def bottleneck_fwd(x, w1, b1, w2, b2, w3, b3, wd=None, bd=None, out=None, form=0):
    _req(x, torch.bfloat16, "x")
    B, Hh, Ww, cin = x.shape
    if out is None:
        out = _new((B, Hh, Ww, 256), torch.bfloat16, x)
    d = _desc(BottleneckDesc, x=x, w1=w1, w2=w2, w3=w3, wd=wd, b1=b1, b2=b2, b3=b3, bd=bd, out=out, B=B, H=Hh, W=Ww, cin=cin,
              planes=w1.shape[0], form=form)
    M = B * Hh * Ww
    macs = cin * 64 + 576 * 64 + 64 * 256 + (cin * 256 if wd is not None else 0)
    nbytes = 2.0 * (M * (cin + 256) + macs)
    _timed("bottleneck_fwd", 2.0 * M * macs, lambda: _call("rt_bottleneck_fwd", d), tag=("BNK", B, Hh, Ww, cin, Hh, Ww, 256, 3, 3, 1, 1),
           nbytes=nbytes)
    return out


def weight_prep(src, N, T, C, *, scale=None, dst=None, dst_t=None):
    _req(src, torch.float32, "src")
    _call("rt_weight_prep", src, scale, dst, dst_t, N, T, C)


def stem_weight_prep(src, scale, dst):
    _call("rt_stem_weight_prep", src, scale, dst)


def bn_fold(w, b, rm, rv, eps, scale, shift):
    _call("rt_bn_fold", w, b, rm, rv, eps, scale, shift, w.numel())


def mask_posenc(mask_u8, h, w, C, add_vec, kpm_out, kpm_off, pos_out, rows_per_img, row_off):
    B, H, W = mask_u8.shape
    _call("rt_mask_posenc", _desc(
        MaskPosencDesc, mask=mask_u8, kpm_out=kpm_out, pos_out=pos_out, add_vec=add_vec, B=B, H=H, W=W, h=h, w=w, C=C,
        kpm_stride=kpm_out.shape[1], kpm_off=kpm_off, pos_rows_per_img=rows_per_img, pos_row_off=row_off))


def colsum(dy, db):
    M, N = dy.shape
    _call("rt_colsum", dy, 1 if dy.dtype == torch.bfloat16 else 0, db, M, N)


def rows_add(rows, D, *, a_f32=None, a_bf16=None, b_f32=None, out_f32=None, out_bf16=None, alpha=1.0,
             accumulate=False, a_map=(0, 0, 0), b_map=(0, 0, 0), o_map=(0, 0, 0)):
    (a_rows, a_stride, a_off), (b_rows, b_stride, b_off), (o_rows, o_stride, o_off) = a_map, b_map, o_map
    _call("rt_rows_add", _desc(
        RowsAddDesc, a_f32=a_f32, a_bf16=a_bf16, b_f32=b_f32, out_f32=out_f32, out_bf16=out_bf16, rows=rows, D=D, alpha=alpha,
        accumulate=int(accumulate), a_grp_rows=a_rows, a_grp_stride=a_stride, a_grp_off=a_off, b_grp_rows=b_rows, b_grp_stride=b_stride,
        b_grp_off=b_off, o_grp_rows=o_rows, o_grp_stride=o_stride, o_grp_off=o_off))


def roberta_pos_ids(ids, pad_idx):
    B, L = ids.shape
    out = torch.empty((B, L), dtype=torch.int32, device=ids.device)
    _call("rt_roberta_pos_ids", ids, out, B, L, pad_idx)
    return out


def bert_embed_fwd(ids, word, pos, type_emb, L, pos_ids=None):
    rows = ids.numel()
    D = word.shape[1]
    out = _new((rows, D), torch.float32, word)
    _call("rt_bert_embed_fwd", ids, word, pos, type_emb, out, rows, L, D, pos_ids)
    return out


def bert_embed_bwd(ids, de, dword, dpos, dtype_emb, L, pos_ids=None):
    rows, D = de.shape
    _call("rt_bert_embed_bwd", ids, de, dword, dpos, dtype_emb, rows, L, D, pos_ids)


def context_mask(smask_u8, phrase_mask_u8=None, pos_l=None, pos_r=None):
    B, L = smask_u8.shape
    if phrase_mask_u8 is None:
        P, Lp = 1, 0
    else:
        _, P, Lp = phrase_mask_u8.shape
    ctx = _new((B, P, L), torch.uint8, smask_u8)
    qmask = _new((B, P), torch.uint8, smask_u8)
    _call("rt_context_mask", smask_u8, phrase_mask_u8, pos_l, pos_r, ctx, qmask, B, L, P, Lp)
    return ctx, qmask


def qenc_attn_fwd(k, qs, vs, ctx):
    B, L, E = qs.shape
    P = ctx.shape[1]
    w = _new((B, P, L), torch.float32, qs)
    c = _new((B, P, E), torch.float32, qs)
    _call("rt_qenc_attn_fwd", k, qs, vs, ctx, w, c, B, P, L, E)
    return w, c


def qenc_attn_bwd(k, qs, vs, w, dc):
    B, L, E = qs.shape
    P = w.shape[1]
    zz = torch.zeros(B * E + 2 * B * L * E, dtype=torch.float32, device=qs.device)
    dk, dqs, dvs = zz[:B * E].view(B, E), zz[B * E:B * E + B * L * E].view(B, L, E), zz[B * E + B * L * E:].view(B, L, E)
    _call("rt_qenc_attn_bwd", k, qs, vs, w, dc, dk, dqs, dvs, B, P, L, E)
    return dk, dqs, dvs


def qenc_fwd(*, B, S, L, P, nq, E, eps=1e-5, drop_p=0.0, drop_seed=0, **t):
    _call("rt_qenc_fwd", _desc(QencFwdDesc, **dict(t, seed_dev=_SEED_DEV if drop_p > 0 else None), B=B, S=S, L=L, P=P, nq=nq, E=E,
                               eps=eps, drop_p=drop_p, drop_seed=drop_seed & 0xFFFFFFFF))


def head_loss(*, NL, B, P, K, E, eps=1e-5, invert_valid=False, **t):
    _call("rt_head_loss", _desc(HeadLossDesc, **t, NL=NL, B=B, P=P, K=K, E=E, eps=eps, invert_valid=int(bool(invert_valid))))


def qenc_bwd(*, B, S, L, P, E, drop_p=0.0, drop_seed=0, **t):
    _call("rt_qenc_bwd", _desc(QencBwdDesc, **dict(t, seed_dev=_SEED_DEV if drop_p > 0 else None), B=B, S=S, L=L, P=P, E=E,
                               drop_p=drop_p, drop_seed=drop_seed & 0xFFFFFFFF))


def qregion_trace():
    buf = (ctypes.c_uint64 * 72)()
    _call("rt_qregion_trace", ctypes.cast(buf, c_void_p), stream=False)
    return [list(buf[i * 24:(i + 1) * 24]) for i in range(3)]


def box_loss(logits, valid_u8, targets, tgt_off, num_boxes, w_bbox=1.0, w_giou=1.0, want_grad=True, weights=None):
    NL, B, P, K, _ = logits.shape
    buf = _new((NL * 2 + 1,), torch.float32, logits)
    losses, total = buf[:NL * 2].view(NL, 2), buf[NL * 2:]
    dl = _new(tuple(logits.shape), torch.float32, logits) if want_grad else None
    _call("rt_box_loss", _desc(BoxLossDesc, logits=logits, valid=valid_u8, targets=targets, tgt_off=tgt_off, num_boxes=num_boxes,
                               losses=losses, total=total, dlogits=dl, NL=NL, B=B, P=P, K=K, w_bbox=w_bbox, w_giou=w_giou, weights=weights))
    return losses, total, dl


def cem_fwd(hs16, w3, b3, res16, w2, b2, B, HW):
    _req(hs16, torch.bfloat16, "hs"); _req(res16, torch.bfloat16, "res")
    for t, n in ((w3, "w3"), (b3, "b3"), (w2, "w2"), (b2, "b2")):
        _req(t, torch.float32, n)
# ... 684 lines not shown
```

reftr_amd/models/net.py:

```python
import math
import os

import torch

from .. import hip as H

RELU, GELU, TANH, NONE = H.ACT_RELU, H.ACT_GELU, H.ACT_TANH, H.ACT_NONE


class Lin:
    __slots__ = ("w32", "b32", "gw", "gb", "W", "WT", "N", "K")

    def __init__(self, w32, b32, gw, gb, device):
        self.w32, self.b32, self.gw, self.gb = w32, b32, gw, gb
        self.N, self.K = w32.shape
        self.W = torch.empty(self.N, self.K, dtype=torch.bfloat16, device=device)
        self.WT = torch.empty(self.K, self.N, dtype=torch.bfloat16, device=device)

    def refresh(self):
        H.weight_prep(self.w32, self.N, 1, self.K, dst=self.W, dst_t=self.WT)


class Net:
    def __init__(self, store, cfg):
        self.store, self.cfg = store, cfg
        self.lins = {}
        self.training = True
        self._seed_base = 0x1234567
        self._site = 0
        import os
        on = int(os.environ.get("REFTR_STREAMS", "1")) if str(store.device).startswith("cuda") else 0
        self.wg = H.SideStream(bool(on & 2), defer=True)
        self.side = H.SideStream(bool(on & 1))
        self.small_wg = H.SmallWgradBatch()
        self.trivial_sa = True
        self.fold_sa = os.environ.get("REFTR_FOLD_SA", "1") != "0"
        self.dec_coop = os.environ.get("REFTR_DEC_COOP", "1") != "0"
        self.dec_coop_bwd = os.environ.get("REFTR_DEC_COOP_BWD", "1") != "0"
        self.dec_kv_pack = os.environ.get("REFTR_DEC_KV_PACK", "1") != "0"
        self._kv_cat = None
        self._dec_cus = None
        self._dec_handoff = H.decoder_handoff(store.device) if str(store.device).startswith("cuda") else None
        self.ln_batch = H.LnGradBatch() if str(store.device).startswith("cuda") else None
        self.big_wg = H.WgradBatch() if str(store.device).startswith("cuda") else None
        self._build_lins()

    def _lin(self, key, wname, bname, rows=None):
        P, G = self.store.P, self.store.G
        w, gw, b, gb = P[wname], G[wname], P[bname], G[bname]
        if rows is not None:
            a, e = rows
            w, gw, b, gb = w[a:e], gw[a:e], b[a:e], gb[a:e]
        self.lins[key] = Lin(w, b, gw, gb, self.store.device)

    def _build_lins(self):
        cfg, st = self.cfg, self.store
        E = cfg.hidden
        for i in range(cfg.bert.layers):
            lp = f"lang_backbone.encoder.layer.{i}."
            q = lp + "attention.self.query."
            self.lins[lp + "qkv"] = Lin(st.packed(q + "weight", 3), st.packed(q + "bias", 3),
                                        st.packed(q + "weight", 3, grad=True), st.packed(q + "bias", 3, grad=True), st.device)
            for n in ("attention.output.dense.", "intermediate.dense.", "output.dense."):
                self._lin(lp + n, lp + n + "weight", lp + n + "bias")
        self._lin("lang_backbone.pooler.dense.", "lang_backbone.pooler.dense.weight", "lang_backbone.pooler.dense.bias")
        for m in ("map_sentence.", "map_phrase.", "query_encoder.fuse_encoder_query."):
            for j in ("0.", "4."):
                self._lin(m + j, m + j + "weight", m + j + "bias")
        for n in ("linear1.", "linear2.", "linear3.", "context_out.0."):
            self._lin("query_encoder." + n, "query_encoder." + n + "weight", "query_encoder." + n + "bias")
        vt = "vl_transformer."
        for i in range(cfg.enc_layers):
            p = f"{vt}encoder.layers.{i}."
            self._mha(p + "self_attn.", split_qk=False)
            self._lin(p + "linear1.", p + "linear1.weight", p + "linear1.bias")
            self._lin(p + "linear2.", p + "linear2.weight", p + "linear2.bias")
        for i in range(cfg.dec_layers):
            p = f"{vt}decoder.layers.{i}."
            self._mha(p + "self_attn.", split_qk=False)
            self._mha(p + "multihead_attn.", split_qk=True)
            self._lin(p + "linear1.", p + "linear1.weight", p + "linear1.bias")
            self._lin(p + "linear2.", p + "linear2.weight", p + "linear2.bias")
        for i in range(3):
            p = f"bbox_embed.layers.{i}."
            self._lin(p, p + "weight", p + "bias")
        if cfg.masks:
            for n in ("q_linear.", "k_linear."):
                self._lin("bbox_attention." + n, "bbox_attention." + n + "weight", "bbox_attention." + n + "bias")
        w = st.phys("input_proj.0.0.weight").view(E, 2048)
        gw = st.phys("input_proj.0.0.weight", grad=True).view(E, 2048)
        self.lins["input_proj.0.0."] = Lin(w, st.P["input_proj.0.0.bias"], gw, st.G["input_proj.0.0.bias"], st.device)
        for l in self.lins.values():
            st.register_overwritable(l.gw)

    def _mha(self, p, split_qk):
        E = self.cfg.hidden
        wn, bn = p + "in_proj_weight", p + "in_proj_bias"
        if split_qk:
            self._lin(p + "q", wn, bn, rows=(0, E)); self._lin(p + "k", wn, bn, rows=(E, 2 * E))
        else:
            self._lin(p + "qk", wn, bn, rows=(0, 2 * E))
        self._lin(p + "v", wn, bn, rows=(2 * E, 3 * E))
        self._lin(p + "out_proj.", p + "out_proj.weight", p + "out_proj.bias")

    def refresh(self):
        if getattr(self, "_prep", None) is None:
            self._prep = H.WeightPrepBatch(self.store.device)
            for l in self.lins.values():
                self._prep.add(l.w32, l.N, 1, l.K, dst=l.W, dst_t=l.WT)
        self._prep.run()
        self._refresh_kv_cat()

    def begin_step(self, training):
        self.training, self._site = training, 0

    def _drop(self, p):
        self._site += 1
        if not self.training or p <= 0:
            return 0.0, 0
        return float(p), (self._site * 40503 + 977) & 0xFFFFFFFF

    def lin_fwd(self, key, x, **kw):
        l = self.lins[key]
        return H.linear(x, l.W, bias=l.b32, **kw)

    def lin_bwd(self, key, dy, x, need_dx=True, **kw):
        l = self.lins[key]
        ow = self.store.claim(l.gw)
        if self.small_wg is not None and dy.shape[0] <= 16:
            self.small_wg.add(dy, x, l.gw, l.gb, overwrite=ow)
        elif self.big_wg is not None and dy.shape[0] > 16:
            self.big_wg.add(dy, x, l.gw, l.gb, overwrite=ow)
        else:
            self.wg.run(lambda: H.linear_wgrad(dy, x, l.gw, dbias=l.gb, overwrite=ow), dy, x)
        if need_dx:
            return H.linear(dy, l.WT, **kw)
        return None

    def flush_wgrads(self):
        if self.small_wg is not None:
            self.small_wg.run()
        if self.big_wg is not None:
            self.big_wg.run()
        if self.ln_batch is not None:
            self.ln_batch.run()

    def flush_wgrads_side(self):
        if not self.side.enabled:
            return self.flush_wgrads()
        keep = []
        for b in (self.small_wg, self.big_wg, self.ln_batch):
            for tup in getattr(b, "keep", []) if b is not None else []:
                keep.extend(t for t in tup if torch.is_tensor(t))
        if keep:
            self.side.run(self.flush_wgrads, *keep)

    def P(self, name):
        return self.store.P[name]

    def G(self, name):
        return self.store.G[name]

    def ln_fwd(self, x, pfx, eps=1e-5, **kw):
        return H.layernorm_fwd(x, self.P(pfx + "weight"), self.P(pfx + "bias"), eps, **kw)

    def ln_bwd(self, dy, x, pfx, mean, rstd, **kw):
        return H.layernorm_bwd(dy, x, self.P(pfx + "weight"), self.P(pfx + "bias"), mean, rstd,
                               self.G(pfx + "weight"), self.G(pfx + "bias"), pg_batch=self.ln_batch, **kw)

    def bert_fwd(self, ids, mask_u8):
        bc = self.cfg.bert
        B, L = ids.shape
        M, Hd = B * L, bc.hidden
        pfx = "lang_backbone."
        e = pfx + "embeddings."
        kpm = (mask_u8 == 0).view(torch.uint8)
        pos_ids = H.roberta_pos_ids(ids, bc.pad_idx) if bc.pad_idx >= 0 else None
        emb = H.bert_embed_fwd(ids, self.P(e + "word_embeddings.weight"), self.P(e + "position_embeddings.weight"),
                               self.P(e + "token_type_embeddings.weight"), L, pos_ids=pos_ids)
        dp, ds = self._drop(bc.dropout)
        h32, h16, _, mean, rstd = self.ln_fwd(emb, e + "LayerNorm.", bc.eps, drop_p=dp, drop_seed=ds)
        ctx = {"ids": ids, "pos_ids": pos_ids, "kpm": kpm, "B": B, "L": L, "emb": emb, "emb_stats": (mean, rstd, dp, ds), "layers": []}
        dh = Hd // bc.heads
        scale = 1.0 / math.sqrt(dh)
        for i in range(bc.layers):
            lp = f"{pfx}encoder.layer.{i}."
            r = {"h16": h16}
            qkv, _ = self.lin_fwd(lp + "qkv", h16)
            r["qkv"] = qkv
            r["adrop"] = self._drop(bc.dropout)
            o, lse = H.attn_fwd(qkv[:, :Hd], qkv[:, Hd:2 * Hd], qkv[:, 2 * Hd:], kpm, B=B, H=bc.heads, Sq=L, Sk=L, dh=dh,
                                scale=scale, drop_p=r["adrop"][0], drop_seed=r["adrop"][1])
            r["o"], r["lse"] = o, lse
            r["d1"] = self._drop(bc.dropout)
            _, t = self.lin_fwd(lp + "attention.output.dense.", o, drop_p=r["d1"][0], drop_seed=r["d1"][1], res_f32=h32,
                                out_bf16=False, out_f32=True)
            h32, h16, _, m1, r1 = self.ln_fwd(t, lp + "attention.output.LayerNorm.", bc.eps)
            r["t"], r["st1"], r["h1_16"] = t, (m1, r1), h16
            g, _, u = self.lin_fwd(lp + "intermediate.dense.", h16, act=GELU, out_preact=True)
            r["g"], r["u"] = g, u
            r["d2"] = self._drop(bc.dropout)
            _, t2 = self.lin_fwd(lp + "output.dense.", g, drop_p=r["d2"][0], drop_seed=r["d2"][1], res_f32=h32,
                                 out_bf16=False, out_f32=True)
            h32, h16, _, m2, r2 = self.ln_fwd(t2, lp + "output.LayerNorm.", bc.eps)
            r["t2"], r["st2"] = t2, (m2, r2)
            ctx["layers"].append(r)
        cls = torch.empty(B, Hd, dtype=torch.bfloat16, device=h16.device)
        H.rows_add(B, Hd, a_bf16=h16, a_map=(1, L, 0), out_bf16=cls)
        pooled, _ = self.lin_fwd(pfx + "pooler.dense.", cls, act=TANH)
        ctx["cls"], ctx["pooled"] = cls, pooled
        return h16, pooled, ctx

    def bert_bwd(self, ctx, d_seq, d_pooled_bf16):
        for _ in self.bert_bwd_layers(ctx, d_seq, d_pooled_bf16):
            pass

    def bert_bwd_layers(self, ctx, d_seq, d_pooled_bf16, stops=()):
        bc = self.cfg.bert
        B, L, Hd = ctx["B"], ctx["L"], bc.hidden
        pfx = "lang_backbone."
        dev = ctx["emb"].device
        if d_seq is None:
            d_seq = torch.zeros(B * L, Hd, dtype=torch.float32, device=dev)
        if d_pooled_bf16 is not None:
            _, dcls = self.lin_bwd(pfx + "pooler.dense.", d_pooled_bf16, ctx["cls"], out_bf16=False, out_f32=True)
            H.rows_add(B, Hd, a_f32=dcls, out_f32=d_seq, accumulate=True, o_map=(1, L, 0))
        dh = Hd // bc.heads
        scale = 1.0 / math.sqrt(dh)
        dh32 = d_seq
        for i in reversed(range(bc.layers)):
            lp = f"{pfx}encoder.layer.{i}."
            r = ctx["layers"][i]
            dt2, dt2b = self.ln_bwd(dh32, r["t2"], lp + "output.LayerNorm.", *r["st2"], drop2_p=r["d2"][0], drop2_seed=r["d2"][1])
            du, _ = self.lin_bwd(lp + "output.dense.", dt2b, r["g"], preact=r["u"])
            _, dh1 = self.lin_bwd(lp + "intermediate.dense.", du, r["h1_16"], res_f32=dt2, out_bf16=False, out_f32=True)
            dt, dtb = self.ln_bwd(dh1, r["t"], lp + "attention.output.LayerNorm.", *r["st1"], drop2_p=r["d1"][0], drop2_seed=r["d1"][1])
            do, _ = self.lin_bwd(lp + "attention.output.dense.", dtb, r["o"])
            qkv = r["qkv"]
            dqkv = torch.empty_like(qkv)
            H.attn_bwd(qkv[:, :Hd], qkv[:, Hd:2 * Hd], qkv[:, 2 * Hd:], r["o"], do, r["lse"], ctx["kpm"], B=B, H=bc.heads,
                       Sq=L, Sk=L, dh=dh, scale=scale, drop_p=r["adrop"][0], drop_seed=r["adrop"][1],
                       dq=dqkv[:, :Hd], dk=dqkv[:, Hd:2 * Hd], dv=dqkv[:, 2 * Hd:])
            _, dh32 = self.lin_bwd(lp + "qkv", dqkv, r["h16"], res_f32=dt, out_bf16=False, out_f32=True)
            if i in stops:
                self.flush_wgrads()
                yield i
        e = pfx + "embeddings."
        mean, rstd, dp, ds = ctx["emb_stats"]
        de, _ = self.ln_bwd(dh32, ctx["emb"], e + "LayerNorm.", mean, rstd, drop_p=dp, drop_seed=ds, want_bf16=False)
        H.bert_embed_bwd(ctx["ids"], de, self.G(e + "word_embeddings.weight"), self.G(e + "position_embeddings.weight"),
                         self.G(e + "token_type_embeddings.weight"), L, pos_ids=ctx["pos_ids"])
        self.flush_wgrads()

    def mlp_fwd(self, x16, pfx, **out_kw):
        _, t1 = self.lin_fwd(pfx + "0.", x16, out_bf16=False, out_f32=True)
        dp, ds = self._drop(0.1)
        _, a16, _, m1, r1 = self.ln_fwd(t1, pfx + "1.", act=RELU, drop_p=dp, drop_seed=ds, want_f32=False)
        _, t2 = self.lin_fwd(pfx + "4.", a16, out_bf16=False, out_f32=True)
        outs = self.ln_fwd(t2, pfx + "5.", act=RELU, **out_kw)
        ctx = {"x16": x16, "t1": t1, "st1": (m1, r1, dp, ds), "a16": a16, "t2": t2, "st2": (outs[3], outs[4])}
        return outs, ctx

    def mlp_bwd(self, ctx, dy, pfx, dy_rowmap=(0, 0, 0), dy2=None, need_dx=True, dx_f32=True, **dx_kw):
        _, dt2b = self.ln_bwd(dy, ctx["t2"], pfx + "5.", *ctx["st2"], act=RELU, rowmap=dy_rowmap, dy2=dy2, want_f32=False)
        _, da = self.lin_bwd(pfx + "4.", dt2b, ctx["a16"], out_bf16=False, out_f32=True)
        m1, r1, dp, ds = ctx["st1"]
        _, dt1b = self.ln_bwd(da, ctx["t1"], pfx + "1.", m1, r1, act=RELU, drop_p=dp, drop_seed=ds, want_f32=False)
        if not need_dx:
            self.lin_bwd(pfx + "0.", dt1b, ctx["x16"], need_dx=False)
            return None
        ob, of = self.lin_bwd(pfx + "0.", dt1b, ctx["x16"], out_bf16=not dx_f32, out_f32=dx_f32, **dx_kw)
        return of if dx_f32 else ob

    def enc_layer_fwd(self, p, x32, x16, xp16, pos, kpm, B, S, qkv=None, next_p=None):
        cfg = self.cfg
        E, Hh = cfg.hidden, cfg.nheads
        dh = E // Hh
        r = {"x16": x16, "xp16": xp16}
        if qkv is None:
            grp = H.GemmGroup()
            qk, _ = self.lin_fwd(p + "self_attn.qk", xp16, group=grp)
            v, _ = self.lin_fwd(p + "self_attn.v", x16, group=grp)
            grp.run()
        else:
            qk, v = qkv
        r["ad"] = self._drop(cfg.dropout)
        o, lse = H.attn_fwd(qk[:, :E], qk[:, E:], v, kpm, B=B, H=Hh, Sq=S, Sk=S, dh=dh, scale=dh ** -0.5,
                            drop_p=r["ad"][0], drop_seed=r["ad"][1])
        r.update(qk=qk, v=v, o=o, lse=lse)
        r["d1"] = self._drop(cfg.dropout)
        _, t = self.lin_fwd(p + "self_attn.out_proj.", o, drop_p=r["d1"][0], drop_seed=r["d1"][1], res_f32=x32,
                            out_bf16=False, out_f32=True)
        x1_32, x1_16, _, m1, r1 = self.ln_fwd(t, p + "norm1.")
        r.update(t=t, st1=(m1, r1), x1_16=x1_16)
        r["dh"] = self._drop(cfg.dropout)
        hdn, _ = self.lin_fwd(p + "linear1.", x1_16, act=RELU, drop_p=r["dh"][0], drop_seed=r["dh"][1])
        r["hdn"] = hdn
        r["d2"] = self._drop(cfg.dropout)
        _, t2 = self.lin_fwd(p + "linear2.", hdn, drop_p=r["d2"][0], drop_seed=r["d2"][1], res_f32=x1_32,
                             out_bf16=False, out_f32=True)
        x2_32, x2_16, x2p16, m2, r2 = self.ln_fwd(t2, p + "norm2.", pos=pos)
        r.update(t2=t2, st2=(m2, r2))
        return x2_32, x2_16, x2p16, r, None

    def enc_layer_bwd(self, p, r, dx2, dx2b, kpm, B, S, dpos_acc):
        cfg = self.cfg
        E, Hh = cfg.hidden, cfg.nheads
        dh = E // Hh
        M = B * S
        gs = 1.0 / (1.0 - r["dh"][0]) if r["dh"][0] > 0 else 1.0
        if getattr(self, "_dbg_enc", None) is not None:
            self._dbg_enc.append((dx2 if dx2b is None else dx2 + dx2b).detach().clone())
        dt2, dt2b = self.ln_bwd(dx2, r["t2"], p + "norm2.", *r["st2"], dy2=dx2b, drop2_p=r["d2"][0], drop2_seed=r["d2"][1])
        dhdn, _ = self.lin_bwd(p + "linear2.", dt2b, r["hdn"], gate=r["hdn"], gate_scale=gs)
        _, dx1 = self.lin_bwd(p + "linear1.", dhdn, r["x1_16"], res_f32=dt2, out_bf16=False, out_f32=True)
        dt, dtb = self.ln_bwd(dx1, r["t"], p + "norm1.", *r["st1"], drop2_p=r["d1"][0], drop2_seed=r["d1"][1])
        do, _ = self.lin_bwd(p + "self_attn.out_proj.", dtb, r["o"])
        qk, v = r["qk"], r["v"]
        dqk = torch.empty_like(qk)
        _, _, dv = H.attn_bwd(qk[:, :E], qk[:, E:], v, r["o"], do, r["lse"], kpm, B=B, H=Hh, Sq=S, Sk=S, dh=dh,
                              scale=dh ** -0.5, drop_p=r["ad"][0], drop_seed=r["ad"][1], dq=dqk[:, :E], dk=dqk[:, E:])
        grp = H.GemmGroup()
        _, dxa = self.lin_bwd(p + "self_attn.v", dv, r["x16"], res_f32=dt, out_bf16=False, out_f32=True, group=grp)
        _, dxp = self.lin_bwd(p + "self_attn.qk", dqk, r["xp16"], out_bf16=False, out_f32=True, group=grp, acc2_f32=dpos_acc)
        grp.run()
        if getattr(self, "_dbg_enc", None) is not None:
            self._dbg_enc.append((dxa + dxp).detach().clone())
        return dxa, dxp

    def dec_kv_all(self, prefixes, mem16, memp16):
        grp = H.GemmGroup()
        out = []
        for p in prefixes:
            k2, _ = self.lin_fwd(p + "multihead_attn.k", memp16, group=grp)
            v2, _ = self.lin_fwd(p + "multihead_attn.v", mem16, group=grp)
            out.append((k2, v2))
        grp.run()
        return out

    def dec_layer_fwd(self, p, t32, t16, tq16, qpos, mem16, memp16, qmask, kpm, B, T, S, kv=None, t3_out=None, fold_sa=False):
        cfg = self.cfg
        E, Hh = cfg.hidden, cfg.nheads
        dh = E // Hh
        sc = dh ** -0.5
        r = {"t16": t16, "tq16": tq16}
        trivial = T == 1 and self.trivial_sa
        fold = trivial and fold_sa and self.fold_sa and (dh & (dh - 1)) == 0
        r["trivial"], r["fold"] = trivial, fold
        lse = None
        if fold:
            r["ad"] = self._drop(cfg.dropout)
            qk = v = None
            o, _ = self.lin_fwd(p + "self_attn.v", t16, drop_p=r["ad"][0], drop_seed=r["ad"][1], drop_shift=dh.bit_length() - 1)
        else:
            v, _ = self.lin_fwd(p + "self_attn.v", t16)
            r["ad"] = self._drop(cfg.dropout)
            if trivial:
                qk = None
                o, lse = H.attn_fwd(v, v, v, qmask, B=B, H=Hh, Sq=1, Sk=1, dh=dh, scale=sc, drop_p=r["ad"][0], drop_seed=r["ad"][1])
            else:
                qk, _ = self.lin_fwd(p + "self_attn.qk", tq16)
                o, lse = H.attn_fwd(qk[:, :E], qk[:, E:], v, qmask, B=B, H=Hh, Sq=T, Sk=T, dh=dh, scale=sc,
                                    drop_p=r["ad"][0], drop_seed=r["ad"][1])
        r.update(qk=qk, v=v, o=o, lse=lse)
        r["d1"] = self._drop(cfg.dropout)
        _, u = self.lin_fwd(p + "self_attn.out_proj.", o, drop_p=r["d1"][0], drop_seed=r["d1"][1], res_f32=t32,
                            out_bf16=False, out_f32=True)
        t1_32, t1_16, t1q16, m1, r1 = self.ln_fwd(u, p + "norm1.", pos=qpos)
        r.update(u=u, st1=(m1, r1), t1q16=t1q16)
        q2, _ = self.lin_fwd(p + "multihead_attn.q", t1q16)
        if kv is not None:
            k2, v2 = kv
        else:
            k2, _ = self.lin_fwd(p + "multihead_attn.k", memp16)
            v2, _ = self.lin_fwd(p + "multihead_attn.v", mem16)
        r["ad2"] = self._drop(cfg.dropout)
        o2, lse2 = H.attn_fwd(q2, k2, v2, kpm, B=B, H=Hh, Sq=T, Sk=S, dh=dh, scale=sc, drop_p=r["ad2"][0], drop_seed=r["ad2"][1])
        r.update(q2=q2, k2=k2, v2=v2, o2=o2, lse2=lse2)
        r["d2"] = self._drop(cfg.dropout)
        _, u2 = self.lin_fwd(p + "multihead_attn.out_proj.", o2, drop_p=r["d2"][0], drop_seed=r["d2"][1], res_f32=t1_32,
                             out_bf16=False, out_f32=True)
        t2_32, t2_16, _, m2, r2 = self.ln_fwd(u2, p + "norm2.")
        r.update(u2=u2, st2=(m2, r2), t2_16=t2_16)
        r["dh"] = self._drop(cfg.dropout)
        hdn, _ = self.lin_fwd(p + "linear1.", t2_16, act=RELU, drop_p=r["dh"][0], drop_seed=r["dh"][1])
        r["hdn"] = hdn
        r["d3"] = self._drop(cfg.dropout)
        _, u3 = self.lin_fwd(p + "linear2.", hdn, drop_p=r["d3"][0], drop_seed=r["d3"][1], res_f32=t2_32,
                             out_bf16=False, out_f32=True)
        t3_32, t3_16, t3q16, m3, r3 = self.ln_fwd(u3, p + "norm3.", pos=qpos, y_f32=t3_out)
        r.update(u3=u3, st3=(m3, r3))
        return t3_32, t3_16, t3q16, r

    def _dec_handoff_buf(self, dev):
        if self._dec_handoff is None or self._dec_handoff.device != dev:
            self._dec_handoff = H.decoder_handoff(dev)
        return self._dec_handoff

    def dec_stack_coop_ok(self, N, T, S, n_layers, fold_sa):
        cfg = self.cfg
        if self._dec_cus is None:
            dev = self.store.device
            ok = False
            if str(dev).startswith("cuda"):
                with torch.cuda.device(dev):
                    ok = H.decoder_supported(cfg.ffn)
            self._dec_cus = 1 << 20 if ok else 0
        return (self.dec_coop and self._dec_cus >= 160 and T == 1 and fold_sa and self.trivial_sa and self.fold_sa and cfg.hidden == 256 and cfg.nheads == 8
                and cfg.ffn == 2048 and N <= 16 and S <= 768 and 1 <= n_layers <= H.DEC_MAX_LAYERS)

    def dec_stack_fwd_coop(self, prefixes, t32, t16, tq16, qpos, kvs, kpm, B, S, t3_all):
        cfg = self.cfg
        E, F, N = cfg.hidden, cfg.ffn, t32.shape[0]
        dev = t32.device
        bf, f32 = torch.bfloat16, torch.float32
        layers, saved = [], []
        t16_in = t16
        for i, p in enumerate(prefixes):
            r = {"t16": t16_in, "tq16": tq16 if i == 0 else None, "trivial": True, "fold": True, "qk": None, "v": None, "lse": None,
                 "coop": True}
            for k in ("ad", "d1", "ad2", "d2", "dh", "d3"):
                r[k] = self._drop(cfg.dropout)
            sm = torch.empty(6, N, dtype=f32, device=dev)
            act = torch.empty(5, N, E, dtype=bf, device=dev)
            pre = torch.empty(3, N, E, dtype=f32, device=dev)
            t3_16 = torch.empty(N, E, dtype=bf, device=dev)
            hdn = torch.empty(N, F, dtype=bf, device=dev)
            lse2 = torch.empty(B, cfg.nheads, 1, dtype=f32, device=dev)
            k2, v2 = kvs[i]
            r.update(o=act[0], t1q16=act[1], q2=act[2], o2=act[3], t2_16=act[4], u=pre[0], u2=pre[1], u3=pre[2], hdn=hdn,
                     st1=(sm[0], sm[1]), st2=(sm[2], sm[3]), st3=(sm[4], sm[5]), k2=k2, v2=v2, lse2=lse2)
            L = self.lins
            lay = dict(Wv=L[p + "self_attn.v"].W, Wo=L[p + "self_attn.out_proj."].W, Wq=L[p + "multihead_attn.q"].W,
                       Wo2=L[p + "multihead_attn.out_proj."].W, W1=L[p + "linear1."].W, W2=L[p + "linear2."].W,
                       bv=L[p + "self_attn.v"].b32, bo=L[p + "self_attn.out_proj."].b32, bq=L[p + "multihead_attn.q"].b32,
                       bo2=L[p + "multihead_attn.out_proj."].b32, b1=L[p + "linear1."].b32, b2=L[p + "linear2."].b32,
                       g1=self.P(p + "norm1.weight"), be1=self.P(p + "norm1.bias"), g2=self.P(p + "norm2.weight"),
                       be2=self.P(p + "norm2.bias"), g3=self.P(p + "norm3.weight"), be3=self.P(p + "norm3.bias"),
                       k2=k2, v2=v2, o=act[0], t1q16=act[1], q2=act[2], o2=act[3], t2_16=act[4], hdn=hdn, t3_16=t3_16,
                       u=pre[0], u2=pre[1], u3=pre[2], mean1=sm[0], rstd1=sm[1], mean2=sm[2], rstd2=sm[3], mean3=sm[4], rstd3=sm[5],
                       lse2=lse2, t3_f32=t3_all[i * N:(i + 1) * N],
                       seed_ad=r["ad"][1], seed_d1=r["d1"][1], seed_ad2=r["ad2"][1], seed_d2=r["d2"][1], seed_dh=r["dh"][1],
                       seed_d3=r["d3"][1])
            layers.append(lay); saved.append(r)
            t16_in = t3_16
        dh = E // cfg.nheads
        drop_p = saved[0]["ad"][0]
        self.dec_counters = H.decoder_fwd(layers, t32, t16, qpos, kpm, H=cfg.nheads, S=S, F=F, drop_p=drop_p, scale=dh ** -0.5,
                                          handoff=self._dec_handoff_buf(dev))
        return saved

    def _wgrad_only(self, key, dy, x):
        l = self.lins[key]
        ow = self.store.claim(l.gw)
        if self.small_wg is not None and dy.shape[0] <= 16:
            self.small_wg.add(dy, x, l.gw, l.gb, overwrite=ow)
        elif self.big_wg is not None and dy.shape[0] > 16:
            self.big_wg.add(dy, x, l.gw, l.gb, overwrite=ow)
        else:
            self.wg.run(lambda: H.linear_wgrad(dy, x, l.gw, dbias=l.gb, overwrite=ow), dy, x)

    def _dec_kv_wt_cat(self, prefixes):
        if self._kv_cat is None or self._kv_cat[0] != tuple(prefixes):
            E = self.cfg.hidden
            dev = self.store.device
            bufs = {n: torch.empty(E, len(prefixes) * E, dtype=torch.bfloat16, device=dev) for n in ("k", "v")}
            self._kv_cat = (tuple(prefixes), bufs)
            self._refresh_kv_cat()
        return self._kv_cat[1]

    def _refresh_kv_cat(self):
        if self._kv_cat is not None:
            prefixes, bufs = self._kv_cat
            for n in ("k", "v"):
                torch.cat([self.lins[p + "multihead_attn." + n].WT for p in prefixes], dim=1, out=bufs[n])

    def dec_stack_bwd_coop(self, prefixes, saved, dnorm_all, mem16, memp16, kpm, B, S, dmem_acc, dmemp_acc, dqpos_acc):
        cfg = self.cfg
        E, F, N = cfg.hidden, cfg.ffn, B
        dev = dnorm_all.device
        bf, f32 = torch.bfloat16, torch.float32
        nb = (N + 3) // 4
        layers, outs = [], []
        NLd = len(prefixes)
        pack = self.dec_kv_pack and NLd > 1
        dkv_all = torch.empty(2, B * S, NLd * E, dtype=bf, device=dev) if pack else None
        for i, p in enumerate(prefixes):
            r = saved[i]
            d16 = torch.empty(5, N, E, dtype=bf, device=dev)
            dhdn = torch.empty(N, F, dtype=bf, device=dev)
            dkv = torch.empty(2, B * S, E, dtype=bf, device=dev)
            parts = torch.empty(3, nb, 2, E, dtype=f32, device=dev)
            L = self.lins
            lay = dict(WT2=L[p + "linear2."].WT, WT1=L[p + "linear1."].WT, WTo2=L[p + "multihead_attn.out_proj."].WT,
                       WTq=L[p + "multihead_attn.q"].WT, WTo=L[p + "self_attn.out_proj."].WT, WTv=L[p + "self_attn.v"].WT,
                       g1=self.P(p + "norm1.weight"), g2=self.P(p + "norm2.weight"), g3=self.P(p + "norm3.weight"),
                       u=r["u"], u2=r["u2"], u3=r["u3"], mean1=r["st1"][0], rstd1=r["st1"][1], mean2=r["st2"][0], rstd2=r["st2"][1],
                       mean3=r["st3"][0], rstd3=r["st3"][1], hdn=r["hdn"], q2=r["q2"], k2=r["k2"], v2=r["v2"], o2=r["o2"],
                       lse2=r["lse2"], dnorm=dnorm_all[i * N:(i + 1) * N], du3b=d16[0], dhdn=dhdn, du2b=d16[1], dq2=d16[2],
                       dub=d16[3], dv=d16[4], dk2=dkv[0], dv2=dkv[1], part1=parts[0], part2=parts[1], part3=parts[2],
                       seed_ad=r["ad"][1], seed_d1=r["d1"][1], seed_ad2=r["ad2"][1], seed_d2=r["d2"][1], seed_d3=r["d3"][1])
            if pack:
                lay.update(dk2p=dkv_all[0][:, i * E:(i + 1) * E], dv2p=dkv_all[1][:, i * E:(i + 1) * E])
            layers.append(lay); outs.append((d16, dhdn, dkv, parts))
        drop_p = saved[0]["d3"][0]
        p_dh = saved[0]["dh"][0]
        dta = torch.empty(N, E, dtype=f32, device=dev)
        dh = E // cfg.nheads
        self.dec_counters = H.decoder_bwd(layers, dta, dqpos_acc, kpm, H=cfg.nheads, S=S, F=F, drop_p=drop_p, scale=dh ** -0.5,
                                          gate_scale=1.0 / (1.0 - p_dh) if p_dh > 0 else 1.0, ldkvp=NLd * E if pack else 0,
                                          handoff=self._dec_handoff_buf(dev))
        for i in reversed(range(len(prefixes))):
            p, r = prefixes[i], saved[i]
            d16, dhdn, dkv, parts = outs[i]
            self._wgrad_only(p + "linear2.", d16[0], r["hdn"])
            self._wgrad_only(p + "linear1.", dhdn, r["t2_16"])
            self._wgrad_only(p + "multihead_attn.out_proj.", d16[1], r["o2"])
            if pack:
                self._wgrad_only(p + "multihead_attn.v", dkv[1], mem16)
                self._wgrad_only(p + "multihead_attn.k", dkv[0], memp16)
            else:
                grp = H.GemmGroup()
                self.lin_bwd(p + "multihead_attn.v", dkv[1], mem16, res_f32=dmem_acc, out_bf16=False, out_f32=dmem_acc, group=grp)
                self.lin_bwd(p + "multihead_attn.k", dkv[0], memp16, res_f32=dmemp_acc, out_bf16=False, out_f32=dmemp_acc, group=grp)
                grp.run()
            self._wgrad_only(p + "multihead_attn.q", d16[2], r["t1q16"])
            self._wgrad_only(p + "self_attn.out_proj.", d16[3], r["o"])
            self._wgrad_only(p + "self_attn.v", d16[4], r["t16"])
            for j, nm in ((2, "norm3."), (1, "norm2."), (0, "norm1.")):
                self.ln_batch.jobs.append(H._desc(H.LnPgJob, partials=parts[j], dgamma=self.G(p + nm + "weight"),
                                                  dbeta=self.G(p + nm + "bias"), n_blocks=nb, D=E))
                self.ln_batch.keep.append(parts[j])
        if pack:
            cat = self._dec_kv_wt_cat(prefixes)
            grp = H.GemmGroup()
            H.linear(dkv_all[1], cat["v"], res_f32=dmem_acc, out_bf16=False, out_f32=dmem_acc, group=grp)
            H.linear(dkv_all[0], cat["k"], res_f32=dmemp_acc, out_bf16=False, out_f32=dmemp_acc, group=grp)
            grp.run()
        return dta

    def dec_layer_bwd(self, p, r, g_a, g_b, mem16, memp16, qmask, kpm, B, T, S, dmem_acc, dmemp_acc, dqpos_acc):
        cfg = self.cfg
        E, Hh = cfg.hidden, cfg.nheads
        dh = E // Hh
        sc = dh ** -0.5
        N = B * T
        du3, du3b = self.ln_bwd(g_a, r["u3"], p + "norm3.", *r["st3"], dy2=g_b, drop2_p=r["d3"][0], drop2_seed=r["d3"][1])
        gs = 1.0 / (1.0 - r["dh"][0]) if r["dh"][0] > 0 else 1.0
        dhdn, _ = self.lin_bwd(p + "linear2.", du3b, r["hdn"], gate=r["hdn"], gate_scale=gs)
        _, dt2 = self.lin_bwd(p + "linear1.", dhdn, r["t2_16"], res_f32=du3, out_bf16=False, out_f32=True)
        du2, du2b = self.ln_bwd(dt2, r["u2"], p + "norm2.", *r["st2"], drop2_p=r["d2"][0], drop2_seed=r["d2"][1])
        do2, _ = self.lin_bwd(p + "multihead_attn.out_proj.", du2b, r["o2"])
        dq2, dk2, dv2 = H.attn_bwd(r["q2"], r["k2"], r["v2"], r["o2"], do2, r["lse2"], kpm, B=B, H=Hh, Sq=T, Sk=S, dh=dh,
                                   scale=sc, drop_p=r["ad2"][0], drop_seed=r["ad2"][1])
        grp = H.GemmGroup()
        self.lin_bwd(p + "multihead_attn.v", dv2, mem16, res_f32=dmem_acc, out_bf16=False, out_f32=dmem_acc, group=grp)
        self.lin_bwd(p + "multihead_attn.k", dk2, memp16, res_f32=dmemp_acc, out_bf16=False, out_f32=dmemp_acc, group=grp)
        grp.run()
        _, dt1q = self.lin_bwd(p + "multihead_attn.q", dq2, r["t1q16"], out_bf16=False, out_f32=True, acc2_f32=dqpos_acc)
        du, dub = self.ln_bwd(du2, r["u"], p + "norm1.", *r["st1"], dy2=dt1q, drop2_p=r["d1"][0], drop2_seed=r["d1"][1])
        if r["fold"]:
            dv, _ = self.lin_bwd(p + "self_attn.out_proj.", dub, r["o"], drop_p=r["ad"][0], drop_seed=r["ad"][1],
                                 drop_shift=dh.bit_length() - 1)
            _, dta = self.lin_bwd(p + "self_attn.v", dv, r["t16"], res_f32=du, out_bf16=False, out_f32=True)
            return dta, None
        do, _ = self.lin_bwd(p + "self_attn.out_proj.", dub, r["o"])
        qk, v = r["qk"], r["v"]
        if r["trivial"]:
            _, _, dv = H.attn_bwd(v, v, v, r["o"], do, r["lse"], qmask, B=B, H=Hh, Sq=1, Sk=1, dh=dh,
                                  scale=sc, drop_p=r["ad"][0], drop_seed=r["ad"][1])
            _, dta = self.lin_bwd(p + "self_attn.v", dv, r["t16"], res_f32=du, out_bf16=False, out_f32=True)
            return dta, None
        dqk = torch.empty_like(qk)
        _, _, dv = H.attn_bwd(qk[:, :E], qk[:, E:], v, r["o"], do, r["lse"], qmask, B=B, H=Hh, Sq=T, Sk=T, dh=dh,
                              scale=sc, drop_p=r["ad"][0], drop_seed=r["ad"][1], dq=dqk[:, :E], dk=dqk[:, E:])
        _, dta = self.lin_bwd(p + "self_attn.v", dv, r["t16"], res_f32=du, out_bf16=False, out_f32=True)
        _, dtq = self.lin_bwd(p + "self_attn.qk", dqk, r["tq16"], out_bf16=False, out_f32=True, acc2_f32=dqpos_acc)
        return dta, dtq
```

Baseline: 1269 images/s.

## Fuse LayerNorm forward and backward as GEMM prologues in encoder and BERT layers

Adds GEMM kernels that compute LayerNorm (forward) or LayerNorm backward directly into the LDS A-operand tile, with one column-tile writing the side outputs (normalized activations, stats, dgamma/dbeta partials). Encoder and BERT layers use these prologues to feed linear1, qk/v of the next layer, output.dense and out_proj instead of running separate LN kernels. This removes standalone LN launches and a round trip of the normalized activation through global memory. The cost is that every N-tile recomputes the row LN, and the prologue adds register and LDS pressure to the GEMM.

```diff
diff --git a/include/reftr_hip.h b/include/reftr_hip.h
--- a/include/reftr_hip.h
+++ b/include/reftr_hip.h
@@ -43,6 +43,41 @@
 } rt_conv_gemm_desc;
 int rt_conv_gemm(const rt_conv_gemm_desc* d, rt_stream_t stream);
 int rt_conv_gemm_grouped(const rt_conv_gemm_desc* descs, int n, rt_stream_t stream);
+
+typedef struct rt_ln_prologue_desc {
+    const float* x;
+    const float* gamma;
+    const float* beta;
+    const float* pos;
+    float*       y_f32;
+    void*        y_bf16;
+    void*        ypos_bf16;
+    float*       mean;
+    float*       rstd;
+    int32_t M, D;
+    float   eps;
+    int32_t operand_pos;
+    int32_t no_outputs;
+} rt_ln_prologue_desc;
+int rt_conv_gemm_ln(const rt_conv_gemm_desc* d, const rt_ln_prologue_desc* ln, rt_stream_t stream);
+int rt_conv_gemm_ln_grouped(const rt_conv_gemm_desc* descs, const rt_ln_prologue_desc* lns, int n, rt_stream_t stream);
+typedef struct rt_ln_bwd_prologue_desc {
+    const float* dy;
+    const float* dy2;
+    const float* x;
+    const float* gamma;
+    const float* mean;
+    const float* rstd;
+    float*       dx_f32;
+    void*        dx_bf16;
+    float*       partials;
+    int32_t*     n_blocks_out;
+    int32_t M, D;
+    float    drop2_p;
+    uint32_t drop2_seed;
+    const uint32_t* seed_dev;
+} rt_ln_bwd_prologue_desc;
+int rt_conv_gemm_lnbwd(const rt_conv_gemm_desc* d, const rt_ln_bwd_prologue_desc* ln, rt_stream_t stream);
 
 typedef struct rt_conv_wgrad_desc {
     const void*  dy;
diff --git a/reftr_amd/csrc/rt_gemm.hip b/reftr_amd/csrc/rt_gemm.hip
--- a/reftr_amd/csrc/rt_gemm.hip
+++ b/reftr_amd/csrc/rt_gemm.hip
@@ -1,4 +1,5 @@
 #include "rt_gemm_dma.h"
+#include "rt_gemm_ln.h"
 #include <stdio.h>
 
 namespace {
@@ -419,6 +420,83 @@
     return RT_OK;
 }
 
+struct LnTileWide   { static constexpr int BM = 64, BN = 128, NS = 2, V = 1; };
+struct LnTileNarrow { static constexpr int BM = 64, BN = 64,  NS = 2, V = 1; };
+struct LnTileBert   { static constexpr int BM = 32, BN = 64,  NS = 3, V = 3; };
+
+static int fill_ln_args(const rt_conv_gemm_desc* d, const rt_ln_prologue_desc* l, GemmArgs& a, LnPro& q) {
+    if (!l || !l->x || !l->gamma || !l->beta) return RT_ERR_BADARG;
+    const int rc = fill_gemm_args(d, a);
+    if (rc != RT_OK) return rc;
+    if (d->tile_hint != 0) return RT_ERR_BADARG;
+    if ((l->operand_pos || (l->ypos_bf16 && !l->no_outputs)) && !l->pos) return RT_ERR_BADARG;
+    if (!gemm_dense(a) || a.K != l->D || (l->D != 256 && l->D != 768) || l->M != a.M) return RT_ERR_UNSUPPORTED;
+    q.x = l->x; q.gamma = l->gamma; q.beta = l->beta; q.pos = l->pos;
+    q.y_f32 = l->y_f32; q.y_bf16 = (bf16_t*)l->y_bf16; q.ypos_bf16 = (bf16_t*)l->ypos_bf16; q.mean = l->mean; q.rstd = l->rstd;
+    q.eps = l->eps; q.a_pos = l->operand_pos ? 1 : 0; q.write = l->no_outputs ? 0 : 1;
+    return RT_OK;
+}
+
+template <class T, class Pro>
+static int launch_gemm_ln(const GemmArgs& a, const Pro& q, hipStream_t s) {
+    const int mt = (a.M + T::BM - 1) / T::BM, nt = (a.N + T::BN - 1) / T::BN;
+    const size_t smem = gemm_ln_lds_bytes(T::BM, T::BN, T::NS, T::V);
+    const auto kern = conv_gemm_ln_kernel<T::BM, T::BN, T::NS, T::V, Pro>;
+    if (smem > 65536) (void)hipFuncSetAttribute((const void*)kern, hipFuncAttributeMaxDynamicSharedMemorySize, (int)smem);
+    hipLaunchKernelGGL(kern, dim3((unsigned)(mt * nt)), dim3(256), smem, s, a, q);
+    RT_CHECK_LAUNCH();
+    return RT_OK;
+}
+
+extern "C" int rt_conv_gemm_ln(const rt_conv_gemm_desc* d, const rt_ln_prologue_desc* ln, rt_stream_t stream) {
+    GemmArgs a;
+    LnPro q;
+    const int rc = fill_ln_args(d, ln, a, q);
+    if (rc != RT_OK) return rc;
+    hipStream_t s = (hipStream_t)stream;
+    if (ln->D == 768) return launch_gemm_ln<LnTileBert>(a, q, s);
+    return a.N >= 1024 ? launch_gemm_ln<LnTileWide>(a, q, s) : launch_gemm_ln<LnTileNarrow>(a, q, s);
+}
+
+extern "C" int rt_conv_gemm_lnbwd(const rt_conv_gemm_desc* d, const rt_ln_bwd_prologue_desc* l, rt_stream_t stream) {
+    if (!l || !l->dy || !l->x || !l->gamma || !l->mean || !l->rstd) return RT_ERR_BADARG;
+    GemmArgs a;
+    const int rc = fill_gemm_args(d, a);
+    if (rc != RT_OK) return rc;
+    if (d->tile_hint != 0) return RT_ERR_BADARG;
+    if (!gemm_dense(a) || a.K != l->D || (l->D != 256 && l->D != 768) || l->M != a.M) return RT_ERR_UNSUPPORTED;
+    LnBwdPro q;
+    q.dy = l->dy; q.dy2 = l->dy2; q.x = l->x; q.gamma = l->gamma; q.mean = l->mean; q.rstd = l->rstd;
+    q.dx_f32 = l->dx_f32; q.dx_bf16 = (bf16_t*)l->dx_bf16; q.partials = l->partials;
+    q.drop2_p = l->drop2_p; q.drop2_seed = l->drop2_seed; q.seed_dev = l->seed_dev; q.write = 1;
+    hipStream_t s = (hipStream_t)stream;
+    const int bm = l->D == 768 ? LnTileBert::BM : LnTileWide::BM;
+    if (l->n_blocks_out) *l->n_blocks_out = (a.M + bm - 1) / bm;
+    if (l->D == 768) return launch_gemm_ln<LnTileBert>(a, q, s);
+    return a.N >= 1024 ? launch_gemm_ln<LnTileWide>(a, q, s) : launch_gemm_ln<LnTileNarrow>(a, q, s);
+}
+
+extern "C" int rt_conv_gemm_ln_grouped(const rt_conv_gemm_desc* descs, const rt_ln_prologue_desc* lns, int n, rt_stream_t stream) {
+    if (!descs || !lns || n < 2 || n > 4) return RT_ERR_BADARG;
+    typedef LnTileNarrow T;
+    GemmLnGroup g;
+    int blocks = 0;
+    for (int i = 0; i < n; ++i) {
+        const int rc = fill_ln_args(descs + i, lns + i, g.j[i], g.q[i]);
+        if (rc != RT_OK) return rc;
+        if (lns[i].D != 256) return RT_ERR_UNSUPPORTED;
+        g.first[i] = blocks;
+        blocks += ((g.j[i].M + T::BM - 1) / T::BM) * ((g.j[i].N + T::BN - 1) / T::BN);
+    }
+    for (int i = n; i < 5; ++i) g.first[i] = blocks;
+    for (int i = n; i < 4; ++i) { g.j[i] = g.j[0]; g.q[i] = g.q[0]; }
+    g.n = n;
+    hipLaunchKernelGGL((conv_gemm_ln_grouped_kernel<T::BM, T::BN, T::NS, T::V>), dim3((unsigned)blocks), dim3(256),
+                       gemm_ln_lds_bytes(T::BM, T::BN, T::NS, T::V), (hipStream_t)stream, g);
+    RT_CHECK_LAUNCH();
+    return RT_OK;
+}
+
 extern "C" int rt_abi_version(void) { return 39; }
 
 extern "C" int rt_device_arch(int dev, char* buf, int buflen) {
diff --git a/reftr_amd/csrc/rt_gemm_ln.h b/reftr_amd/csrc/rt_gemm_ln.h
--- /dev/null
+++ b/reftr_amd/csrc/rt_gemm_ln.h
@@ -0,0 +1,324 @@
+#pragma once
+#include "rt_gemm_dma.h"
+#include "rt_ln_row.h"
+
+namespace {
+
+template <int BM>
+__device__ __forceinline__ void ln_put(unsigned char* xs, int r, int i, int lane, f32x4 a) {
+    unsigned char* dst = xs + (4 * i + (lane >> 4)) * (BM * 128) + r * 128 + ((((lane & 15) >> 1) ^ (r & 7)) << 4) + ((lane & 1) << 3);
+    *reinterpret_cast<bf16x4*>(dst) = bf16x4{(bf16_t)a[0], (bf16_t)a[1], (bf16_t)a[2], (bf16_t)a[3]};
+}
+
+template <int V>
+__device__ __forceinline__ void ln_row_fwd(const f32x4 (&v)[V], const float eps, const f32x4 (&gam)[V], const f32x4 (&bet)[V],
+                                           float& mean, float& rstd, f32x4 (&y)[V]) {
+    if constexpr (V != 3) {
+        rt_ln_stats<V>(v, eps, mean, rstd);
+#pragma unroll
+        for (int i = 0; i < V; ++i) y[i] = rt_ln_affine(v[i], mean, rstd, gam[i], bet[i], false);
+    } else {
+#pragma clang fp contract(off)
+        constexpr float c = 1.f / 768;
+        float s = 0.f;
+#pragma unroll
+        for (int i = 0; i < 3; ++i) s += (v[i][0] + v[i][1]) + (v[i][2] + v[i][3]);
+        const float S = rt_wave_sum(s);
+        mean = S * c;
+        f32x4 d[3];
+#pragma unroll
+        for (int e = 0; e < 4; ++e) { d[0][e] = __builtin_fmaf(S, -c, v[0][e]); d[1][e] = __builtin_fmaf(S, -c, v[1][e]); d[2][e] = v[2][e] - mean; }
+        float ss = d[0][1] * d[0][1];
+        ss = __builtin_fmaf(d[0][0], d[0][0], ss); ss = __builtin_fmaf(d[0][2], d[0][2], ss); ss = __builtin_fmaf(d[0][3], d[0][3], ss);
+#pragma unroll
+        for (int e = 0; e < 4; ++e) ss = __builtin_fmaf(d[1][e], d[1][e], ss);
+#pragma unroll
+        for (int e = 0; e < 4; ++e) ss = d[2][e] * d[2][e] + ss;
+        rstd = rsqrtf(__builtin_fmaf(rt_wave_sum(ss), c, eps));
+#pragma unroll
+        for (int i = 0; i < 3; ++i)
+#pragma unroll
+            for (int e = 0; e < 4; ++e) y[i][e] = __builtin_fmaf(gam[i][e], d[i][e] * rstd, bet[i][e]);
+    }
+}
+
+struct LnPro {
+    const float* x; const float* gamma; const float* beta; const float* pos;
+    float* y_f32; bf16_t* y_bf16; bf16_t* ypos_bf16; float* mean; float* rstd;
+    float eps;
+    int a_pos;
+    int write;
+    template <int V> struct State {};
+    template <int BM, int V>
+    __device__ __forceinline__ void rows(const int M, const int m0, const bool side, unsigned char* xs, State<V>&) const {
+        constexpr int D = 256 * V, RPW = BM / 4, RB = V == 1 ? 8 : 4;
+        static_assert(RPW % RB == 0, "rows per wave");
+        const int lane = threadIdx.x & 63, wave = threadIdx.x >> 6;
+        f32x4 gam[V], bet[V];
+#pragma unroll
+        for (int i = 0; i < V; ++i) {
+            const int c = (i * 64 + lane) * 4;
+            gam[i] = *reinterpret_cast<const f32x4*>(gamma + c); bet[i] = *reinterpret_cast<const f32x4*>(beta + c);
+        }
+        const bool want_pos = pos && (a_pos || (side && ypos_bf16));
+        for (int r0 = 0; r0 < RPW; r0 += RB) {
+            f32x4 v[RB][V], ps[RB][V];
+#pragma unroll
+            for (int j = 0; j < RB; ++j) {
+                const int m = m0 + (r0 + j) * 4 + wave;
+                const size_t o = (size_t)(m < M ? m : 0) * D;
+#pragma unroll
+                for (int i = 0; i < V; ++i) {
+                    v[j][i] = *reinterpret_cast<const f32x4*>(x + o + (i * 64 + lane) * 4);
+                    ps[j][i] = want_pos ? *reinterpret_cast<const f32x4*>(pos + o + (i * 64 + lane) * 4) : f32x4{0.f, 0.f, 0.f, 0.f};
+                }
+            }
+#pragma unroll
+            for (int j = 0; j < RB; ++j) {
+                const int r = (r0 + j) * 4 + wave, m = m0 + r;
+                const bool ok = m < M;
+                float mu, rs;
+                f32x4 yv[V];
+                ln_row_fwd<V>(v[j], eps, gam, bet, mu, rs, yv);
+                if (side && ok && lane == 0) { if (mean) mean[m] = mu; if (rstd) rstd[m] = rs; }
+#pragma unroll
+                for (int i = 0; i < V; ++i) {
+                    const f32x4 y = yv[i];
+                    const f32x4 yp = y + ps[j][i];
+                    if (side && ok) {
+                        const size_t o = (size_t)m * D + (i * 64 + lane) * 4;
+                        if (y_f32) *reinterpret_cast<f32x4*>(y_f32 + o) = y;
+                        if (y_bf16) rt_store_bf16(y_bf16 + o, y);
+                        if (ypos_bf16) rt_store_bf16(ypos_bf16 + o, yp);
+                    }
+                    ln_put<BM>(xs, r, i, lane, ok ? (a_pos ? yp : y) : f32x4{0.f, 0.f, 0.f, 0.f});
+                }
+            }
+        }
+    }
+    template <int V>
+    __device__ __forceinline__ void finish(bool, int, unsigned char*, const State<V>&) const {}
+};
+
+struct LnBwdPro {
+    const float* dy; const float* dy2; const float* x; const float* gamma; const float* mean; const float* rstd;
+    float* dx_f32; bf16_t* dx_bf16; float* partials;
+    float drop2_p; uint32_t drop2_seed; const uint32_t* seed_dev;
+    int write;
+    template <int V> struct State { f32x4 dg[V], db[V]; };
+    template <int BM, int V>
+    __device__ __forceinline__ void rows(const int M, const int m0, const bool side, unsigned char* xs, State<V>& st) const {
+        constexpr int D = 256 * V, RPW = BM / 4, RB = V == 1 ? 8 : 4;
+        static_assert(RPW % RB == 0, "rows per wave");
+        const int lane = threadIdx.x & 63, wave = threadIdx.x >> 6;
+        const f32x4 zero = {0.f, 0.f, 0.f, 0.f};
+        f32x4 gam[V];
+#pragma unroll
+        for (int i = 0; i < V; ++i) { gam[i] = *reinterpret_cast<const f32x4*>(gamma + (i * 64 + lane) * 4); st.dg[i] = zero; st.db[i] = zero; }
+        const rt_drop drop2 = rt_drop::site(drop2_p, seed_dev, drop2_seed);
+        for (int r0 = 0; r0 < RPW; r0 += RB) {
+            f32x4 d[RB][V], xv[RB][V];
+            float mu[RB], rs[RB];
+#pragma unroll
+            for (int j = 0; j < RB; ++j) {
+                const int m = m0 + (r0 + j) * 4 + wave;
+                const int mm = m < M ? m : 0;
+                const size_t o = (size_t)mm * D;
+                mu[j] = mean[mm]; rs[j] = rstd[mm];
+#pragma unroll
+                for (int i = 0; i < V; ++i) {
+                    d[j][i] = *reinterpret_cast<const f32x4*>(dy + o + (i * 64 + lane) * 4);
+                    if (dy2) d[j][i] += *reinterpret_cast<const f32x4*>(dy2 + o + (i * 64 + lane) * 4);
+                    xv[j][i] = *reinterpret_cast<const f32x4*>(x + o + (i * 64 + lane) * 4);
+                }
+            }
+#pragma unroll
+            for (int j = 0; j < RB; ++j) {
+                const int r = (r0 + j) * 4 + wave, m = m0 + r;
+                if (m >= M) {
+#pragma unroll
+                    for (int i = 0; i < V; ++i) ln_put<BM>(xs, r, i, lane, zero);
+                    continue;
+                }
+                f32x4 xh[V], g[V];
+                float s1 = 0.f, s2 = 0.f;
+#pragma unroll
+                for (int i = 0; i < V; ++i) rt_ln_bwd_group(d[j][i], xv[j][i], mu[j], rs[j], gam[i], zero, false, xh[i], g[i], s1, s2, st.dg[i], st.db[i]);
+                rt_ln_bwd_means<V>(s1, s2);
+#pragma unroll
+                for (int i = 0; i < V; ++i) {
+                    const size_t o = (size_t)m * D + (i * 64 + lane) * 4;
+                    const f32x4 dx = rt_ln_bwd_dx(g[i], xh[i], rs[j], s1, s2);
+                    const f32x4 dxd = drop2.apply(dx, (uint32_t)o);
+                    if (side) {
+                        if (dx_f32) *reinterpret_cast<f32x4*>(dx_f32 + o) = dx;
+                        if (dx_bf16) rt_store_bf16(dx_bf16 + o, dxd);
+                    }
+                    ln_put<BM>(xs, r, i, lane, dxd);
+                }
+            }
+        }
+    }
+    template <int V>
+    __device__ __forceinline__ void finish(const bool side, const int tile_m, unsigned char* smem, const State<V>& st) const {
+        constexpr int D = 256 * V;
+        if (!side || !partials) return;
+        const int lane = threadIdx.x & 63, wave = threadIdx.x >> 6;
+        float* sm_g = reinterpret_cast<float*>(smem);
+        float* sm_b = sm_g + 4 * D;
+        __syncthreads();
+#pragma unroll
+        for (int i = 0; i < V; ++i) {
+            *reinterpret_cast<f32x4*>(sm_g + wave * D + (i * 64 + lane) * 4) = st.dg[i];
+            *reinterpret_cast<f32x4*>(sm_b + wave * D + (i * 64 + lane) * 4) = st.db[i];
+        }
+        __syncthreads();
+        for (int c = threadIdx.x; c < D; c += 256) {
+            partials[((size_t)tile_m * 2) * D + c] = sm_g[c] + sm_g[D + c] + sm_g[2 * D + c] + sm_g[3 * D + c];
+            partials[((size_t)tile_m * 2 + 1) * D + c] = sm_b[c] + sm_b[D + c] + sm_b[2 * D + c] + sm_b[3 * D + c];
+        }
+    }
+};
+
+constexpr size_t gemm_ln_lds_bytes(int BM, int BN, int NS, int V) { return (size_t)BM * 512 * V + (size_t)NS * BN * 128; }
+
+template <int BM, int BN, int NS, int V, class Pro>
+__device__ __forceinline__ void gemm_ln_body(const GemmArgs& p, const Pro& q, const int bx, const int gx) {
+    constexpr int NT = 256, WM = 2, RPP = 32, AJ = BN / RPP, KT = 4 * V;
+    typedef WaveTile<BM, BN, WM> WT;
+    constexpr int TM = WT::TM, TN = WT::TN;
+    constexpr int X_TILE = BM * 128, X_BYTES = KT * X_TILE, W_STAGE = BN * 128;
+    static_assert(AJ >= 1 && TM >= 1 && NS >= 2, "tile too small");
+    static_assert((size_t)8 * 256 * V * 4 <= (size_t)X_BYTES, "the d gamma / d beta rows of four waves fit the block");
+    extern __shared__ __attribute__((aligned(16))) unsigned char smem[];
+    typedef __attribute__((address_space(3))) void* lds_ptr;
+    unsigned char* const xs = smem;
+    const unsigned char* const ws = smem + X_BYTES;
+
+    const int t = threadIdx.x;
+    const int lane = t & 63, wave = t >> 6;
+    const int wn = wave & 1, wm = wave >> 1;
+    const int li = lane & 15, lg = lane >> 4;
+    const WT wt{wn, wm, li, lg};
+
+    const int n_tiles = (p.N + BN - 1) / BN;
+    const int bid = rt_xcd_remap(bx, gx, p.xcd);
+    const int tile_n = bid % n_tiles, tile_m = bid / n_tiles;
+    const int n0 = tile_n * BN, m0 = tile_m * BM;
+
+    const int srow = t >> 3, chunk = (t & 7) ^ (srow & 7);
+    constexpr int OOB = 0x7fffffff;
+    int a_off[AJ];
+#pragma unroll
+    for (int j = 0; j < AJ; ++j) {
+        const int n = n0 + srow + RPP * j;
+        a_off[j] = n < p.N ? (n * p.K + chunk * 8) * 2 : OOB;
+    }
+    const i32x4 rs_w = rt_make_rsrc(p.wgt, p.wgt_bytes);
+    const unsigned lds_w = (unsigned)(uintptr_t)(lds_ptr)smem + (unsigned)X_BYTES + (unsigned)__builtin_amdgcn_readfirstlane(wave) * 1024u;
+    int lk = 0;
+    auto issue_tile = [&](int buf) __attribute__((always_inline)) {
+#pragma unroll
+        for (int j = 0; j < AJ; ++j) rt_dma16(rs_w, lds_w + buf * W_STAGE + j * (RPP * 128), a_off[j], lk << 7);
+        if (lk + 1 < KT) ++lk;
+    };
+#pragma unroll
+    for (int s = 0; s < NS - 1; ++s) issue_tile(s);
+
+    const bool side = q.write && tile_n == 0;
+    typename Pro::template State<V> st;
+    q.template rows<BM, V>(p.M, m0, side, xs, st);
+    rt_wait_vmcnt<0>();
+
+    f32x4 acc[TN][TM], tot[TN][TM];
+#pragma unroll
+    for (int a = 0; a < TN; ++a)
+#pragma unroll
+        for (int b = 0; b < TM; ++b) { acc[a][b] = f32x4{0.f, 0.f, 0.f, 0.f}; tot[a][b] = acc[a][b]; }
+    const bool quarters = p.M <= 16;
+    const int per = ((p.K >> 5) + 3) >> 2;
+    int cbuf = 0, lbuf = NS - 1;
+    for (int kt = 0; kt < KT; ++kt) {
+        rt_wait_vmcnt<(NS - 2) * AJ>();
+        __syncthreads();
+        issue_tile(lbuf);
+        const unsigned char* wst = ws + cbuf * W_STAGE;
+        const unsigned char* xst = xs + kt * X_TILE;
+#pragma unroll
+        for (int kk = 0; kk < 2; ++kk) {
+            const int ks = kt * 2 + kk;
+            if (quarters && ks > 0 && ks % per == 0) {
+#pragma unroll
+                for (int a = 0; a < TN; ++a)
+#pragma unroll
+                    for (int b = 0; b < TM; ++b) { tot[a][b] = ks == per ? acc[a][b] : tot[a][b] + acc[a][b]; acc[a][b] = f32x4{0.f, 0.f, 0.f, 0.f}; }
+            }
+            const int slot = rt_frag_slot(kk, li, lg);
+            bf16x8 fa[TN], fb[TM];
+#pragma unroll
+            for (int a = 0; a < TN; ++a) fa[a] = *rt_frag(wst, wn * (BN / 2) + a * 16 + li, slot);
+#pragma unroll
+            for (int b = 0; b < TM; ++b) fb[b] = *rt_frag(xst, wm * (BM / WM) + b * 16 + li, slot);
+            WT::mma_k(fa, fb, acc);
+        }
+        cbuf = cbuf + 1 == NS ? 0 : cbuf + 1;
+        lbuf = lbuf + 1 == NS ? 0 : lbuf + 1;
+    }
+    rt_wait_vmcnt<0>();
+    if (quarters) {
+#pragma unroll
+        for (int a = 0; a < TN; ++a)
+#pragma unroll
+            for (int b = 0; b < TM; ++b) acc[a][b] = tot[a][b] + acc[a][b];
+    }
+    q.template finish<V>(side, tile_m, smem, st);
+
+    constexpr int EP_LD = BN + 4, CPR = BN / 8, PIECES = (BM * CPR + NT - 1) / NT;
+    static_assert((size_t)BM * EP_LD * 4 <= (size_t)X_BYTES + (size_t)NS * W_STAGE, "epilogue tile does not fit");
+    if (p.epi_lds && (p.N & 7) == 0) {
+        float* tile = reinterpret_cast<float*>(smem);
+        __syncthreads();
+#pragma unroll
+        for (int a = 0; a < TN; ++a)
+#pragma unroll
+            for (int b = 0; b < TM; ++b) *wt.acc_at(tile, EP_LD, wm, a, b) = acc[a][b];
+        __syncthreads();
+#pragma unroll
+        for (int i = 0; i < PIECES; ++i) {
+            const int idx = i * NT + t;
+            const int rl = idx / CPR, cl = (idx - rl * CPR) * 8;
+            if (idx >= BM * CPR) continue;
+            const int m = m0 + rl, n = n0 + cl;
+            if (m >= p.M || n >= p.N) continue;
+            epilogue<8>(p, m, n, epi_ld<8>(tile + rl * EP_LD + cl));
+        }
+        return;
+    }
+#pragma unroll
+    for (int a = 0; a < TN; ++a) {
+        const int n = n0 + wn * (BN / 2) + a * 16 + lg * 4;
+        if (n >= p.N) continue;
+#pragma unroll
+        for (int b = 0; b < TM; ++b) {
+            const int m = m0 + wm * (BM / WM) + b * 16 + li;
+            if (m >= p.M) continue;
+            epilogue<4>(p, m, n, acc[a][b]);
+        }
+    }
+}
+
+template <int BM, int BN, int NS, int V, class Pro>
+__global__ __launch_bounds__(256, 2) void conv_gemm_ln_kernel(const GemmArgs p, const Pro q) {
+    gemm_ln_body<BM, BN, NS, V>(p, q, (int)blockIdx.x, (int)gridDim.x);
+}
+
+struct GemmLnGroup { GemmArgs j[4]; LnPro q[4]; int first[5]; int n; };
+template <int BM, int BN, int NS, int V>
+__global__ __launch_bounds__(256, 2) void conv_gemm_ln_grouped_kernel(const GemmLnGroup g) {
+    int lo = 0;
+    for (int i = 1; i < g.n; ++i) if (g.first[i] <= (int)blockIdx.x) lo = i;
+    lo = __builtin_amdgcn_readfirstlane(lo);
+    gemm_ln_body<BM, BN, NS, V>(g.j[lo], g.q[lo], (int)blockIdx.x - g.first[lo], g.first[lo + 1] - g.first[lo]);
+}
+
+}
diff --git a/reftr_amd/hip.py b/reftr_amd/hip.py
--- a/reftr_amd/hip.py
+++ b/reftr_amd/hip.py
@@ -65,6 +65,18 @@
                 ("grp_rows", c_int32), ("grp_stride", c_int32), ("grp_off", c_int32), ("seed_dev", c_void_p)]
 
 
+class LnPrologueDesc(_Abi, c="rt_ln_prologue_desc"):
+    _fields_ = [("x", c_void_p), ("gamma", c_void_p), ("beta", c_void_p), ("pos", c_void_p), ("y_f32", c_void_p),
+                ("y_bf16", c_void_p), ("ypos_bf16", c_void_p), ("mean", c_void_p), ("rstd", c_void_p),
+                ("M", c_int32), ("D", c_int32), ("eps", c_float), ("operand_pos", c_int32), ("no_outputs", c_int32)]
+
+
+class LnBwdPrologueDesc(_Abi, c="rt_ln_bwd_prologue_desc"):
+    _fields_ = [("dy", c_void_p), ("dy2", c_void_p), ("x", c_void_p), ("gamma", c_void_p), ("mean", c_void_p), ("rstd", c_void_p),
+                ("dx_f32", c_void_p), ("dx_bf16", c_void_p), ("partials", c_void_p), ("n_blocks_out", POINTER(c_int32)),
+                ("M", c_int32), ("D", c_int32), ("drop2_p", c_float), ("drop2_seed", c_uint32), ("seed_dev", c_void_p)]
+
+
 class LayerNormBwdDesc(_Abi, c="rt_layernorm_bwd_desc"):
     _fields_ = [("dy", c_void_p), ("dy2", c_void_p), ("x", c_void_p), ("gamma", c_void_p), ("beta", c_void_p),
                 ("mean", c_void_p), ("rstd", c_void_p), ("dx_f32", c_void_p), ("dx_bf16", c_void_p),
@@ -349,6 +361,9 @@
     "rt_device_arch": (c_int, [c_int, c_char_p, c_int]),
     "rt_conv_gemm": (c_int, [POINTER(ConvGemmDesc), c_void_p]),
     "rt_conv_gemm_grouped": (c_int, [c_void_p, c_int, c_void_p]),
+    "rt_conv_gemm_ln": (c_int, [POINTER(ConvGemmDesc), POINTER(LnPrologueDesc), c_void_p]),
+    "rt_conv_gemm_ln_grouped": (c_int, [c_void_p, c_void_p, c_int, c_void_p]),
+    "rt_conv_gemm_lnbwd": (c_int, [POINTER(ConvGemmDesc), POINTER(LnBwdPrologueDesc), c_void_p]),
     "rt_conv_wgrad": (c_int, [POINTER(ConvWgradDesc), c_void_p]),
     "rt_gconv": (c_int, [POINTER(ConvGemmDesc), c_int, c_void_p]),
     "rt_gconv_wgrad": (c_int, [POINTER(ConvWgradDesc), c_int, c_void_p]),
@@ -614,8 +629,11 @@
 
 def conv_gemm(src, wgt, *, geom, bias=None, res_f32=None, res_bf16=None, gate=None, gate_scale=1.0,
               preact=None, dtanh=None, res_first=False, act=ACT_NONE, drop_p=0.0, drop_seed=0, transposed=False,
-              out_bf16=True, out_f32=False, out_preact=False, tile_hint=0, group=None, drop_shift=0, acc2_f32=None, dil=1):
+              out_bf16=True, out_f32=False, out_preact=False, tile_hint=0, group=None, drop_shift=0, acc2_f32=None, dil=1,
+              ln=None, ln_pos=False):
     B, SH, SW, SC, DH, DW, N, KH, KW, stride, pad = geom
+    if ln is not None:
+        src = ln.operand(ln_pos)
     _req(src, torch.bfloat16, "src"); _req(wgt, torch.bfloat16, "wgt")
     _req(bias, torch.float32, "bias"); _req(res_f32, torch.float32, "res_f32")
     _req(res_bf16, torch.bfloat16, "res_bf16"); _req(gate, torch.bfloat16, "gate")
@@ -643,7 +661,10 @@
                    + 8.0 * (acc2_f32 is not None) + (4.0 if of is not None else 0.0) + (2.0 if ob is not None else 0.0) - 2.0
                    + (2.0 if op is not None else 0.0))
     if group is not None:
-        group.add(d, flops, ("T" if transposed else "F",) + tuple(geom), (src, wgt, ob, of, op, bias, res_f32, res_bf16, gate, preact, dtanh), epi)
+        group.add(d, flops, ("T" if transposed else "F",) + tuple(geom), (src, wgt, ob, of, op, bias, res_f32, res_bf16, gate, preact, dtanh), epi,
+                  ln=None if ln is None else ln.desc(ln_pos))
+    elif ln is not None:
+        _timed("conv_gemm", flops, lambda: ln.call(d, ln_pos), tag=("F",) + tuple(geom), epi_bytes=epi)
     else:
         _timed("conv_gemm", flops, lambda: _call("rt_conv_gemm", d), tag=("T" if transposed else "F",) + tuple(geom), epi_bytes=epi)
     if op is not None:
@@ -654,26 +675,33 @@
 class GemmGroup:
 
     def __init__(self):
-        self.descs, self.keep, self.flops, self.nbytes, self.epi = [], [], 0.0, 0.0, 0.0
-
-    def add(self, d, flops, tag, keep, epi=0.0):
+        self.descs, self.keep, self.flops, self.nbytes, self.epi, self.lns = [], [], 0.0, 0.0, 0.0, []
+
+    def add(self, d, flops, tag, keep, epi=0.0, ln=None):
         self.descs.append(d); self.keep.append(keep); self.flops += flops; self.nbytes += _algo_bytes(tag); self.epi += epi
+        self.lns.append(ln)
 
     def run(self):
         if not self.descs:
             return
         n = len(self.descs)
+        if any(l is not None for l in self.lns):
+            assert all(l is not None for l in self.lns) and 2 <= n <= 4
+            arr, larr = (ConvGemmDesc * n)(*self.descs), (LnPrologueDesc * n)(*self.lns)
+            _timed("conv_gemm", self.flops, lambda: _call("rt_conv_gemm_ln_grouped", arr, larr, n), nbytes=self.nbytes, epi_bytes=self.epi)
+            self.__init__()
+            return
         for i in range(0, n, 12):
             chunk = self.descs[i:i + 12]
             arr = (ConvGemmDesc * len(chunk))(*chunk)
             share = len(chunk) / n
             _timed("conv_gemm", self.flops * share, lambda arr=arr, m=len(chunk): _call("rt_conv_gemm_grouped", arr, m),
                    nbytes=self.nbytes * share, epi_bytes=self.epi * share)
-        self.descs, self.keep, self.flops, self.nbytes, self.epi = [], [], 0.0, 0.0, 0.0
+        self.__init__()
 
 
 def linear(x, w, bias=None, **kw):
-    M, K = x.shape
+    M, K = x.shape if x is not None else kw["ln"].x.shape
     N = w.shape[0]
     return conv_gemm(x, w, geom=(M, 1, 1, K, 1, 1, N, 1, 1, 1, 0), bias=bias, **kw)
 
@@ -802,6 +830,56 @@
         M=M, D=D, eps=eps, act=act, drop_p=drop_p, drop_seed=drop_seed & 0xFFFFFFFF, grp_rows=grp_rows, grp_stride=grp_stride,
         grp_off=grp_off, seed_dev=_seedp(drop_p)))
     return y_f32, y_bf16, ypos_bf16, mean, rstd
+
+
+class LnPrologue:
+
+    def __init__(self, x, gamma, beta, eps=1e-5, *, pos=None):
+        M, D = x.shape
+        _req(x, torch.float32, "x"); _req(gamma, torch.float32, "gamma"); _req(beta, torch.float32, "beta"); _req(pos, torch.float32, "pos")
+        self.x, self.gamma, self.beta, self.eps, self.pos = x, gamma, beta, eps, pos
+        self.outs = (_new((M, D), torch.float32, x), _new((M, D), torch.bfloat16, x),
+                     _new((M, D), torch.bfloat16, x) if pos is not None else None, _new((M,), torch.float32, x), _new((M,), torch.float32, x))
+        self.claimed = False
+
+    def operand(self, with_pos):
+        return self.outs[2 if with_pos else 1]
+
+    def desc(self, with_pos):
+        y_f32, y_bf16, ypos_bf16, mean, rstd = self.outs
+        first, self.claimed = not self.claimed, True
+        return _desc(LnPrologueDesc, x=self.x, gamma=self.gamma, beta=self.beta, pos=self.pos, y_f32=y_f32, y_bf16=y_bf16,
+                     ypos_bf16=ypos_bf16, mean=mean, rstd=rstd, M=self.x.shape[0], D=self.x.shape[1], eps=self.eps,
+                     operand_pos=int(bool(with_pos)), no_outputs=int(not first))
+
+    def call(self, d, with_pos):
+        _call("rt_conv_gemm_ln", d, self.desc(with_pos))
+
+
+class LnBwdPrologue:
+
+    def __init__(self, dy, x, gamma, mean, rstd, dgamma, dbeta, *, dy2=None, drop2_p=0.0, drop2_seed=0, pg_batch=None):
+        M, D = x.shape
+        _req(dy, torch.float32, "dy"); _req(dy2, torch.float32, "dy2"); _req(x, torch.float32, "x")
+        assert pg_batch is not None or (dgamma is None and dbeta is None)
+        self.x, self.dgamma, self.dbeta, self.pg_batch = x, dgamma, dbeta, pg_batch
+        self.outs = (_new((M, D), torch.float32, x), _new((M, D), torch.bfloat16, x))
+        self.part = _new(((M + 31) // 32, 2, D), torch.float32, x) if dgamma is not None or dbeta is not None else None
+        self.nb = c_int32(0)
+        self._desc = _desc(LnBwdPrologueDesc, dy=dy, dy2=dy2, x=x, gamma=gamma, mean=mean, rstd=rstd, dx_f32=self.outs[0],
+                           dx_bf16=self.outs[1], partials=self.part, n_blocks_out=ctypes.pointer(self.nb), M=M, D=D, drop2_p=drop2_p,
+                           drop2_seed=drop2_seed & 0xFFFFFFFF, seed_dev=_seedp(drop2_p))
+        self.keep = (dy, dy2, gamma, mean, rstd)
+
+    def operand(self, with_pos):
+        return self.outs[1]
+
+    def call(self, d, with_pos):
+        _call("rt_conv_gemm_lnbwd", d, self._desc)
+        if self.part is not None:
+            self.pg_batch.jobs.append(_desc(LnPgJob, partials=self.part, dgamma=self.dgamma, dbeta=self.dbeta, n_blocks=self.nb.value,
+                                            D=self.x.shape[1]))
+            self.pg_batch.keep.append(self.part)
 
 
 class LnGradBatch:
diff --git a/reftr_amd/models/net.py b/reftr_amd/models/net.py
--- a/reftr_amd/models/net.py
+++ b/reftr_amd/models/net.py
@@ -6,6 +6,8 @@
 from .. import hip as H
 
 RELU, GELU, TANH, NONE = H.ACT_RELU, H.ACT_GELU, H.ACT_TANH, H.ACT_NONE
+LN_PRO_ENC_FWD, LN_PRO_ENC_BWD, LN_PRO_BERT_FWD, LN_PRO_BERT_BWD = 1, 2, 4, 8
+LN_PRO_DEFAULT = 0
 
 
 class Lin:
@@ -38,6 +40,11 @@
         self.dec_coop = os.environ.get("REFTR_DEC_COOP", "1") != "0"
         self.dec_coop_bwd = os.environ.get("REFTR_DEC_COOP_BWD", "1") != "0"
         self.dec_kv_pack = os.environ.get("REFTR_DEC_KV_PACK", "1") != "0"
+        self.ln_pro = int(os.environ.get("REFTR_LN_PROLOGUE", str(LN_PRO_DEFAULT))) if str(store.device).startswith("cuda") else 0
+        if cfg.hidden != 256:
+            self.ln_pro &= ~(LN_PRO_ENC_FWD | LN_PRO_ENC_BWD)
+        if cfg.bert.hidden not in (256, 768):
+            self.ln_pro &= ~(LN_PRO_BERT_FWD | LN_PRO_BERT_BWD)
         self._kv_cat = None
         self._dec_cus = None
         self._dec_handoff = H.decoder_handoff(store.device) if str(store.device).startswith("cuda") else None
@@ -124,8 +131,11 @@
         l = self.lins[key]
         return H.linear(x, l.W, bias=l.b32, **kw)
 
-    def lin_bwd(self, key, dy, x, need_dx=True, **kw):
+    def lin_bwd(self, key, dy, x, need_dx=True, ln=None, **kw):
         l = self.lins[key]
+        if ln is not None:
+            dy, need_dx = ln.operand(False), False
+            out = H.linear(None, l.WT, ln=ln, **kw)
         ow = self.store.claim(l.gw)
         if self.small_wg is not None and dy.shape[0] <= 16:
             self.small_wg.add(dy, x, l.gw, l.gb, overwrite=ow)
@@ -135,7 +145,7 @@
             self.wg.run(lambda: H.linear_wgrad(dy, x, l.gw, dbias=l.gb, overwrite=ow), dy, x)
         if need_dx:
             return H.linear(dy, l.WT, **kw)
-        return None
+        return out if ln is not None else None
 
     def flush_wgrads(self):
         if self.small_wg is not None:
@@ -167,6 +177,13 @@
     def ln_bwd(self, dy, x, pfx, mean, rstd, **kw):
         return H.layernorm_bwd(dy, x, self.P(pfx + "weight"), self.P(pfx + "bias"), mean, rstd,
                                self.G(pfx + "weight"), self.G(pfx + "bias"), pg_batch=self.ln_batch, **kw)
+
+    def ln_pro_fwd(self, x, pfx, eps=1e-5, pos=None):
+        return H.LnPrologue(x, self.P(pfx + "weight"), self.P(pfx + "bias"), eps, pos=pos)
+
+    def ln_pro_bwd(self, dy, x, pfx, mean, rstd, **kw):
+        return H.LnBwdPrologue(dy, x, self.P(pfx + "weight"), mean, rstd, self.G(pfx + "weight"), self.G(pfx + "bias"),
+                               pg_batch=self.ln_batch, **kw)
 
     def bert_fwd(self, ids, mask_u8):
         bc = self.cfg.bert
@@ -183,10 +200,11 @@
         ctx = {"ids": ids, "pos_ids": pos_ids, "kpm": kpm, "B": B, "L": L, "emb": emb, "emb_stats": (mean, rstd, dp, ds), "layers": []}
         dh = Hd // bc.heads
         scale = 1.0 / math.sqrt(dh)
+        pro = None
         for i in range(bc.layers):
             lp = f"{pfx}encoder.layer.{i}."
             r = {"h16": h16}
-            qkv, _ = self.lin_fwd(lp + "qkv", h16)
+            qkv, _ = self.lin_fwd(lp + "qkv", h16 if pro is None else None, ln=pro)
             r["qkv"] = qkv
             r["adrop"] = self._drop(bc.dropout)
             o, lse = H.attn_fwd(qkv[:, :Hd], qkv[:, Hd:2 * Hd], qkv[:, 2 * Hd:], kpm, B=B, H=bc.heads, Sq=L, Sk=L, dh=dh,
@@ -195,14 +213,24 @@
             r["d1"] = self._drop(bc.dropout)
             _, t = self.lin_fwd(lp + "attention.output.dense.", o, drop_p=r["d1"][0], drop_seed=r["d1"][1], res_f32=h32,
                                 out_bf16=False, out_f32=True)
-            h32, h16, _, m1, r1 = self.ln_fwd(t, lp + "attention.output.LayerNorm.", bc.eps)
+            if self.ln_pro & LN_PRO_BERT_FWD:
+                pro = self.ln_pro_fwd(t, lp + "attention.output.LayerNorm.", bc.eps)
+                h32, h16, _, m1, r1 = pro.outs
+                g, _, u = self.lin_fwd(lp + "intermediate.dense.", None, ln=pro, act=GELU, out_preact=True)
+            else:
+                h32, h16, _, m1, r1 = self.ln_fwd(t, lp + "attention.output.LayerNorm.", bc.eps)
+                g, _, u = self.lin_fwd(lp + "intermediate.dense.", h16, act=GELU, out_preact=True)
             r["t"], r["st1"], r["h1_16"] = t, (m1, r1), h16
-            g, _, u = self.lin_fwd(lp + "intermediate.dense.", h16, act=GELU, out_preact=True)
             r["g"], r["u"] = g, u
             r["d2"] = self._drop(bc.dropout)
             _, t2 = self.lin_fwd(lp + "output.dense.", g, drop_p=r["d2"][0], drop_seed=r["d2"][1], res_f32=h32,
                                  out_bf16=False, out_f32=True)
-            h32, h16, _, m2, r2 = self.ln_fwd(t2, lp + "output.LayerNorm.", bc.eps)
+            if self.ln_pro & LN_PRO_BERT_FWD and i + 1 < bc.layers:
+                pro = self.ln_pro_fwd(t2, lp + "output.LayerNorm.", bc.eps)
+                h32, h16, _, m2, r2 = pro.outs
+            else:
+                pro = None
+                h32, h16, _, m2, r2 = self.ln_fwd(t2, lp + "output.LayerNorm.", bc.eps)
             r["t2"], r["st2"] = t2, (m2, r2)
             ctx["layers"].append(r)
         cls = torch.empty(B, Hd, dtype=torch.bfloat16, device=h16.device)
@@ -231,11 +259,21 @@
         for i in reversed(range(bc.layers)):
             lp = f"{pfx}encoder.layer.{i}."
             r = ctx["layers"][i]
-            dt2, dt2b = self.ln_bwd(dh32, r["t2"], lp + "output.LayerNorm.", *r["st2"], drop2_p=r["d2"][0], drop2_seed=r["d2"][1])
-            du, _ = self.lin_bwd(lp + "output.dense.", dt2b, r["g"], preact=r["u"])
+            if self.ln_pro & LN_PRO_BERT_BWD:
+                pro = self.ln_pro_bwd(dh32, r["t2"], lp + "output.LayerNorm.", *r["st2"], drop2_p=r["d2"][0], drop2_seed=r["d2"][1])
+                dt2, dt2b = pro.outs
+                du, _ = self.lin_bwd(lp + "output.dense.", None, r["g"], ln=pro, preact=r["u"])
+            else:
+                dt2, dt2b = self.ln_bwd(dh32, r["t2"], lp + "output.LayerNorm.", *r["st2"], drop2_p=r["d2"][0], drop2_seed=r["d2"][1])
+                du, _ = self.lin_bwd(lp + "output.dense.", dt2b, r["g"], preact=r["u"])
             _, dh1 = self.lin_bwd(lp + "intermediate.dense.", du, r["h1_16"], res_f32=dt2, out_bf16=False, out_f32=True)
-            dt, dtb = self.ln_bwd(dh1, r["t"], lp + "attention.output.LayerNorm.", *r["st1"], drop2_p=r["d1"][0], drop2_seed=r["d1"][1])
-            do, _ = self.lin_bwd(lp + "attention.output.dense.", dtb, r["o"])
+            if self.ln_pro & LN_PRO_BERT_BWD:
+                pro = self.ln_pro_bwd(dh1, r["t"], lp + "attention.output.LayerNorm.", *r["st1"], drop2_p=r["d1"][0], drop2_seed=r["d1"][1])
+                dt, dtb = pro.outs
+                do, _ = self.lin_bwd(lp + "attention.output.dense.", None, r["o"], ln=pro)
+            else:
+                dt, dtb = self.ln_bwd(dh1, r["t"], lp + "attention.output.LayerNorm.", *r["st1"], drop2_p=r["d1"][0], drop2_seed=r["d1"][1])
+                do, _ = self.lin_bwd(lp + "attention.output.dense.", dtb, r["o"])
             qkv = r["qkv"]
             dqkv = torch.empty_like(qkv)
             H.attn_bwd(qkv[:, :Hd], qkv[:, Hd:2 * Hd], qkv[:, 2 * Hd:], r["o"], do, r["lse"], ctx["kpm"], B=B, H=bc.heads,
@@ -291,17 +329,33 @@
         r["d1"] = self._drop(cfg.dropout)
         _, t = self.lin_fwd(p + "self_attn.out_proj.", o, drop_p=r["d1"][0], drop_seed=r["d1"][1], res_f32=x32,
                             out_bf16=False, out_f32=True)
-        x1_32, x1_16, _, m1, r1 = self.ln_fwd(t, p + "norm1.")
+        fused = bool(self.ln_pro & LN_PRO_ENC_FWD)
+        pro = None
+        if fused:
+            pro = self.ln_pro_fwd(t, p + "norm1.")
+            x1_32, x1_16, _, m1, r1 = pro.outs
+        else:
+            x1_32, x1_16, _, m1, r1 = self.ln_fwd(t, p + "norm1.")
         r.update(t=t, st1=(m1, r1), x1_16=x1_16)
         r["dh"] = self._drop(cfg.dropout)
-        hdn, _ = self.lin_fwd(p + "linear1.", x1_16, act=RELU, drop_p=r["dh"][0], drop_seed=r["dh"][1])
+        hdn, _ = self.lin_fwd(p + "linear1.", None if fused else x1_16, ln=pro, act=RELU, drop_p=r["dh"][0], drop_seed=r["dh"][1])
         r["hdn"] = hdn
         r["d2"] = self._drop(cfg.dropout)
         _, t2 = self.lin_fwd(p + "linear2.", hdn, drop_p=r["d2"][0], drop_seed=r["d2"][1], res_f32=x1_32,
                              out_bf16=False, out_f32=True)
-        x2_32, x2_16, x2p16, m2, r2 = self.ln_fwd(t2, p + "norm2.", pos=pos)
+        nxt = None
+        if fused and next_p is not None:
+            pro = self.ln_pro_fwd(t2, p + "norm2.", pos=pos)
+            x2_32, x2_16, x2p16, m2, r2 = pro.outs
+            grp = H.GemmGroup()
+            qk, _ = self.lin_fwd(next_p + "self_attn.qk", None, ln=pro, ln_pos=True, group=grp)
+            v, _ = self.lin_fwd(next_p + "self_attn.v", None, ln=pro, group=grp)
+            grp.run()
+            nxt = (qk, v)
+        else:
+            x2_32, x2_16, x2p16, m2, r2 = self.ln_fwd(t2, p + "norm2.", pos=pos)
         r.update(t2=t2, st2=(m2, r2))
-        return x2_32, x2_16, x2p16, r, None
+        return x2_32, x2_16, x2p16, r, nxt
 
     def enc_layer_bwd(self, p, r, dx2, dx2b, kpm, B, S, dpos_acc):
         cfg = self.cfg
@@ -311,11 +365,22 @@
         gs = 1.0 / (1.0 - r["dh"][0]) if r["dh"][0] > 0 else 1.0
         if getattr(self, "_dbg_enc", None) is not None:
             self._dbg_enc.append((dx2 if dx2b is None else dx2 + dx2b).detach().clone())
-        dt2, dt2b = self.ln_bwd(dx2, r["t2"], p + "norm2.", *r["st2"], dy2=dx2b, drop2_p=r["d2"][0], drop2_seed=r["d2"][1])
-        dhdn, _ = self.lin_bwd(p + "linear2.", dt2b, r["hdn"], gate=r["hdn"], gate_scale=gs)
+        fused = bool(self.ln_pro & LN_PRO_ENC_BWD)
+        if fused:
+            pro = self.ln_pro_bwd(dx2, r["t2"], p + "norm2.", *r["st2"], dy2=dx2b, drop2_p=r["d2"][0], drop2_seed=r["d2"][1])
+            dt2, dt2b = pro.outs
+            dhdn, _ = self.lin_bwd(p + "linear2.", None, r["hdn"], ln=pro, gate=r["hdn"], gate_scale=gs)
+        else:
+            dt2, dt2b = self.ln_bwd(dx2, r["t2"], p + "norm2.", *r["st2"], dy2=dx2b, drop2_p=r["d2"][0], drop2_seed=r["d2"][1])
+            dhdn, _ = self.lin_bwd(p + "linear2.", dt2b, r["hdn"], gate=r["hdn"], gate_scale=gs)
         _, dx1 = self.lin_bwd(p + "linear1.", dhdn, r["x1_16"], res_f32=dt2, out_bf16=False, out_f32=True)
-        dt, dtb = self.ln_bwd(dx1, r["t"], p + "norm1.", *r["st1"], drop2_p=r["d1"][0], drop2_seed=r["d1"][1])
-        do, _ = self.lin_bwd(p + "self_attn.out_proj.", dtb, r["o"])
+        if fused:
+            pro = self.ln_pro_bwd(dx1, r["t"], p + "norm1.", *r["st1"], drop2_p=r["d1"][0], drop2_seed=r["d1"][1])
+            dt, dtb = pro.outs
+            do, _ = self.lin_bwd(p + "self_attn.out_proj.", None, r["o"], ln=pro)
+        else:
+            dt, dtb = self.ln_bwd(dx1, r["t"], p + "norm1.", *r["st1"], drop2_p=r["d1"][0], drop2_seed=r["d1"][1])
+            do, _ = self.lin_bwd(p + "self_attn.out_proj.", dtb, r["o"])
         qk, v = r["qk"], r["v"]
         dqk = torch.empty_like(qk)
         _, _, dv = H.attn_bwd(qk[:, :E], qk[:, E:], v, r["o"], do, r["lse"], kpm, B=B, H=Hh, Sq=S, Sk=S, dh=dh,
```

Result: slower. 1238 images/s (-2.4%).
